# dkogan/libdogleg

Hardware: NVIDIA B200
Metric: dogleg_iterations_per_sec (higher is better)
Workload: dtype f64

## Files before the change

include/dogleg_gpu.h:

```cpp
#pragma once
#include <stddef.h>
#include "dogleg.h"
#ifdef __cplusplus
extern "C" {
#endif

int         dogleg_gpu_device_count(void);
int         dogleg_gpu_set_device(int device);
int         dogleg_gpu_get_device(void);
const char* dogleg_gpu_last_error(void);
const char* dogleg_gpu_version(void);

void        dogleg_gpu_set_permutation(const int* perm, int n, int postorder);

typedef void (dogleg_gpu_callback_sparse_t)(const double* d_p, double* d_x, double* d_Jt_values,
                                            void* stream, void* cookie);
typedef void (dogleg_gpu_callback_dense_t)(const double* d_p, double* d_x, double* d_J,
                                           void* stream, void* cookie);

double dogleg_gpu_optimize_sparse(double* p, unsigned int Nstate, unsigned int Nmeas, unsigned int NJnnz,
                                  const int* Jp, const int* Ji,
                                  dogleg_gpu_callback_sparse_t* f, void* cookie,
                                  const dogleg_parameters2_t* parameters,
                                  dogleg_solverContext_t** returnContext);
double dogleg_gpu_optimize_dense(double* p, unsigned int Nstate, unsigned int Nmeas,
                                 dogleg_gpu_callback_dense_t* f, void* cookie,
                                 const dogleg_parameters2_t* parameters,
                                 dogleg_solverContext_t** returnContext);

typedef void (dogleg_gpu_callback_dense_products_t)(const double* d_p, double* d_norm2x, double* d_Jtx,
                                                     double* d_JtJ, void* stream, void* cookie);
double dogleg_gpu_optimize_dense_products(double* p, unsigned int Nstate,
                                          dogleg_gpu_callback_dense_products_t* f, void* cookie,
                                          const dogleg_parameters2_t* parameters,
                                          dogleg_solverContext_t** returnContext);

int dogleg_gpu_solve(dogleg_solverContext_t* ctx, const double* B, double* X, int nrhs);
int dogleg_gpu_export_factor(dogleg_solverContext_t* ctx);

void dogleg_gpu_host_progress(size_t n_values_final, size_t n_x_final);

int  dogleg_gpu_nccl_get_unique_id(unsigned char id[128]);
int  dogleg_gpu_nccl_init(int rank, int world, const unsigned char id[128]);
void dogleg_gpu_nccl_finalize(void);
int  dogleg_gpu_nccl_world(void);

double dogleg_gpu_optimize_sparse_sharded(double* p, unsigned int Nstate,
                                          unsigned int Nmeas_total, const int* Jp_global, const int* Ji_global,
                                          unsigned int col_begin, unsigned int Nmeas_local,
                                          dogleg_callback_t* f_host, dogleg_gpu_callback_sparse_t* f_device,
                                          void* cookie, const dogleg_parameters2_t* parameters,
                                          dogleg_solverContext_t** returnContext);

double dogleg_gpu_optimize_dense_sharded(double* p, unsigned int Nstate, unsigned int Nmeas_total,
                                         unsigned int row_begin, unsigned int Nmeas_local,
                                         dogleg_callback_dense_t* f_host, dogleg_gpu_callback_dense_t* f_device,
                                         void* cookie, const dogleg_parameters2_t* parameters,
                                         dogleg_solverContext_t** returnContext);

void dogleg_gpu_context_layout(size_t out[6]);

void dogleg_gpu_get_stats(const dogleg_solverContext_t* ctx, double out[8]);
void dogleg_gpu_get_comm_stats(double out[2]);
void dogleg_gpu_get_phase_ms(double out[8]);

typedef void (dogleg_gpu_callback_dense_batched_t)(const double* d_p, double* d_x, double* d_J,
                                                   const int* d_active, int B,
                                                   void* stream, void* cookie);
int dogleg_gpu_optimize_dense_batched(double* p, unsigned int Nstate, unsigned int Nmeas,
                                      unsigned int B,
                                      dogleg_gpu_callback_dense_batched_t* f, void* cookie,
                                      const dogleg_parameters2_t* parameters,
                                      double* norm2x_out, int* iterations_out);

typedef void (dogleg_gpu_callback_dense_products_batched_t)(const double* d_p, double* d_norm2x, double* d_Jtx,
                                                             double* d_JtJ, const int* d_active, int B,
                                                             void* stream, void* cookie);
int dogleg_gpu_optimize_dense_products_batched(double* p, unsigned int Nstate, unsigned int B,
                                               dogleg_gpu_callback_dense_products_batched_t* f, void* cookie,
                                               const dogleg_parameters2_t* parameters,
                                               double* norm2x_out, int* iterations_out);

typedef struct dogleg_gpu_batch dogleg_gpu_batch_t;

int dogleg_gpu_optimize_dense_batched2(double* p, unsigned int Nstate, unsigned int Nmeas, unsigned int B,
                                       dogleg_gpu_callback_dense_batched_t* f, void* cookie,
                                       const dogleg_parameters2_t* parameters,
                                       double* norm2x_out, int* iterations_out, dogleg_gpu_batch_t** returnBatch);
int dogleg_gpu_optimize_dense_products_batched2(double* p, unsigned int Nstate, unsigned int B,
                                                dogleg_gpu_callback_dense_products_batched_t* f, void* cookie,
                                                const dogleg_parameters2_t* parameters,
                                                double* norm2x_out, int* iterations_out,
                                                dogleg_gpu_batch_t** returnBatch);

enum { DOGLEG_GPU_BATCH_UNFINISHED = 0,
       DOGLEG_GPU_BATCH_GRADIENT = 1,
       DOGLEG_GPU_BATCH_STEP = 2,
       DOGLEG_GPU_BATCH_TRUSTREGION = 3,
       DOGLEG_GPU_BATCH_MAX_ITERATIONS = 4 };


int  dogleg_gpu_batch_status(const dogleg_gpu_batch_t* batch, int* status_out, double* lambda_out);
int  dogleg_gpu_batch_solve(dogleg_gpu_batch_t* batch, const double* R, double* X, int nrhs);
int  dogleg_gpu_batch_solve_device(dogleg_gpu_batch_t* batch, const double* d_R, double* d_X, int nrhs, void* stream);
int  dogleg_gpu_batch_covariance(dogleg_gpu_batch_t* batch, double* out, int packed);
int  dogleg_gpu_batch_covariance_device(dogleg_gpu_batch_t* batch, double* d_out, int packed, void* stream);
void dogleg_gpu_batch_free(dogleg_gpu_batch_t** batch);

void dogleg_gpu_batched_stats(double out[8]);
void dogleg_gpu_release_batched_cache(void);

typedef struct dlb_symbolic dlb_symbolic_t;
dlb_symbolic_t* dlb_symbolic_create(int Nstate, int Nmeas, const int* Jp, const int* Ji,
                                    const int* perm_or_null, int postorder);
void            dlb_symbolic_free(dlb_symbolic_t* S);
void            dlb_symbolic_info(const dlb_symbolic_t* S, long long out[8]);
enum { DLB_SYM_PERM = 0, DLB_SYM_PARENT = 1, DLB_SYM_COLCOUNT = 2, DLB_SYM_SN_FIRST = 3,
       DLB_SYM_ROWS_PTR = 4, DLB_SYM_ROWS = 5, DLB_SYM_SN_PARENT = 6, DLB_SYM_CLS_OF_COL = 7,
       DLB_SYM_CLS_FRONT = 8, DLB_SYM_SN_LEVEL = 9, DLB_SYM_REL = 10, DLB_SYM_CHILD_PTR = 11,
       DLB_SYM_CHILD_LIST = 12, DLB_SYM_LEVEL_PTR = 13, DLB_SYM_LEVEL_SN = 14, DLB_SYM_CLS_PTR = 15,
       DLB_SYM_CLS_ROWS = 16, DLB_SYM_CLS_LOC = 17, DLB_SYM_MEM_PTR = 18, DLB_SYM_MEM_COL = 19 };
long long       dlb_symbolic_get(const dlb_symbolic_t* S, int what, int* out, long long cap);
long long       dlb_symbolic_front_off(const dlb_symbolic_t* S, long long* out, long long cap);

typedef struct dlb_gather_plan dlb_gather_plan_t;
dlb_gather_plan_t* dlb_gather_plan_create(const dlb_symbolic_t* S, int small_front_max, int heavy,
                                          int gsplit, int gchunk, int gtile);
void            dlb_gather_plan_free(dlb_gather_plan_t* G);
void            dlb_gather_plan_info(const dlb_gather_plan_t* G, long long out[8]);
enum { DLB_GP_DST = 0, DLB_GP_SRC_PTR = 1, DLB_GP_SRC_BASE = 2, DLB_GP_LD = 3, DLB_GP_H = 4, DLB_GP_W = 5,
       DLB_GP_SRC_LD = 6, DLB_GP_LEVEL_PTR = 7, DLB_GP_TMP_OFF = 8, DLB_GP_LEVEL_TMP = 9, DLB_GP_SG_FLAG = 10 };
long long       dlb_gather_plan_get(const dlb_gather_plan_t* G, int list, int what, long long* out, long long cap);

typedef struct dlb_task_plan dlb_task_plan_t;
dlb_task_plan_t* dlb_task_plan_create(const dlb_symbolic_t* S, const int* Jp, int col_begin, int ncols,
                                      int sm_count, int ranges_enabled);
void            dlb_task_plan_free(dlb_task_plan_t* T);
enum { DLB_TP_TASK_CLS = 0, DLB_TP_TASK_M0 = 1, DLB_TP_TASK_M1 = 2, DLB_TP_CLS_TASK_PTR = 3, DLB_TP_TASK_GOFF = 4,
       DLB_TP_TASK_GGOFF = 5, DLB_TP_MEM_COL = 6, DLB_TP_MEM_POS = 7, DLB_TP_BIG_TASKS = 8, DLB_TP_SMALL_TASKS = 9,
       DLB_TP_GJ_BIG_TASKS = 10, DLB_TP_RANGED = 11, DLB_TP_GP_COUNT = 12, DLB_TP_GP_FIRST = 13, DLB_TP_GINV_PTR = 14,
       DLB_TP_GINV_CLS = 15, DLB_TP_GINV_OFF = 16, DLB_TP_HEAVY = 17, DLB_TP_MEDIUM = 18,
       DLB_TP_SIZES = 19,
       DLB_TP_RANGE_TASKS = 20    };
long long       dlb_task_plan_get(const dlb_task_plan_t* T, int what, long long* out, long long cap);

typedef struct dlb_engine dlb_engine_t;

typedef struct
{
  double norm2_x, norm2_Jtx, maxabs_Jtx;
  double norm2_JJtx, k_cauchy, norm2_cauchy;
  double norm2_gn;
  double norm2_step, k_interp, Jtx_dot_step, maxabs_step, norm2_Jstep, discriminant;
  double step_type, trial_flags;
  long long minor;
} dlb_scalars_t;

enum { DLB_STEP_CAUCHY = 0, DLB_STEP_GAUSSNEWTON = 1, DLB_STEP_INTERPOLATED = 2 };

dlb_engine_t* dlb_engine_create(int solve_type, unsigned int Nstate, unsigned int Nmeas,
                                unsigned int NJnnz, int packed, int upper);
enum { DLB_ENGINE_NO_HOST_INPUTS = 1 };
dlb_engine_t* dlb_engine_create2(int solve_type, unsigned int Nstate, unsigned int Nmeas,
                                 unsigned int NJnnz, int packed, int upper, int flags);
dlb_engine_t* dlb_engine_create3(int solve_type, unsigned int Nstate, unsigned int Nmeas,
                                 unsigned int NJnnz, int packed, int upper, int flags,
                                 unsigned int Nmeas_total, unsigned int col_begin);
void          dlb_engine_comm_stats(const dlb_engine_t* e, double out[2]);
void          dlb_engine_destroy(dlb_engine_t* e);
void          dogleg_gpu_release_cache(void);
void          dogleg_gpu_assume_pattern_unchanged(int on);
int           dlb_engine_pattern_equals(const dlb_engine_t* e, const int* Jp, const int* Ji);

enum { DLB_BUF_P = 0, DLB_BUF_X = 1, DLB_BUF_JTX = 2, DLB_BUF_CAUCHY = 3, DLB_BUF_GN = 4,
       DLB_BUF_STEP = 5, DLB_BUF_JVALUES = 6, DLB_BUF_JP = 7, DLB_BUF_JI = 8,
       DLB_BUF_NORM2X = 9    };
void*         dlb_engine_host_buffer(dlb_engine_t* e, int slot, int which);
void*         dlb_engine_device_buffer(dlb_engine_t* e, int slot, int which);
void*         dlb_engine_stream(dlb_engine_t* e);

int  dlb_engine_set_pattern(dlb_engine_t* e, const int* Jp, const int* Ji,
                            const int* perm_or_null, int postorder);
const dlb_symbolic_t* dlb_engine_symbolic(const dlb_engine_t* e);

int  dlb_engine_evaluate(dlb_engine_t* e, int slot, int from_host, double norm2x_products);
void dlb_engine_begin_host_fill(dlb_engine_t* e, int slot);
int  dlb_engine_cauchy(dlb_engine_t* e, int slot);
int  dlb_engine_factorize(dlb_engine_t* e, int slot, double lambda);
int  dlb_engine_gauss_newton(dlb_engine_t* e, int slot);
int  dlb_engine_step(dlb_engine_t* e, int from, int to, int step_type, double delta);
int  dlb_engine_has_trial(const dlb_engine_t* e);
int  dlb_engine_has_fused_eval(const dlb_engine_t* e);
int  dlb_engine_trial(dlb_engine_t* e, int from, int to, double delta, double lambda);
void dlb_engine_set_lazy_p(dlb_engine_t* e, int on);
int  dlb_engine_download_p(dlb_engine_t* e, int slot);
int  dlb_engine_download(dlb_engine_t* e, int slot);
int  dlb_engine_upload_p(dlb_engine_t* e, int slot);
const dlb_scalars_t* dlb_engine_scalars(const dlb_engine_t* e);

int  dlb_engine_solve(dlb_engine_t* e, const double* B, double* X, int nrhs);
int  dlb_engine_debug_JtJ(dlb_engine_t* e, int slot, double lambda, double* JtJ_out);
int  dlb_engine_dense_factor_to_host(dlb_engine_t* e, double* out);

void dlb_engine_counters(const dlb_engine_t* e, double out[4]);
void dlb_engine_enable_timing(dlb_engine_t* e, int on);
void dlb_engine_phase_ms(const dlb_engine_t* e, double out[8]);

#ifdef __cplusplus
}
#endif
```

libdogleg_b200/csrc/dlb_capi_symbolic.cpp:

```cpp
#include "dlb_symbolic.h"
#include "dlb_gatherplan.h"
#include "dlb_taskplan.h"
#include "dogleg_internal.h"
#include <cstdlib>
#include <cstring>
#include <algorithm>

struct dlb_symbolic { DlbSymbolic S; };

extern "C" dlb_symbolic_t* dlb_symbolic_create(int Nstate, int Nmeas, const int* Jp, const int* Ji,
                                               const int* perm_or_null, int postorder)
{
  dlb_symbolic* h = new dlb_symbolic();
  if(!dlb_symbolic_analyze(h->S, Nstate, Nmeas, Jp, Ji, perm_or_null, postorder != 0))
  {
    delete h;
    dlb_set_error("malformed Jt pattern or permutation");
    return NULL;
  }
  return h;
}
extern "C" void dlb_symbolic_free(dlb_symbolic_t* h) { delete h; }

static const DlbSymbolic& sym(const dlb_symbolic_t* h) { return *reinterpret_cast<const DlbSymbolic*>(h); }

extern "C" void dlb_symbolic_info(const dlb_symbolic_t* h, long long out[8])
{
  const DlbSymbolic& S = sym(h);
  out[0] = S.ncls; out[1] = S.nsuper; out[2] = S.nlevels; out[3] = S.nnzL();
  out[4] = S.max_front_rows; out[5] = S.front_off.empty() ? 0 : S.front_off.back();
  out[6] = (long long)S.flops(); out[7] = (long long)S.rows.size();
}
extern "C" long long dlb_symbolic_get(const dlb_symbolic_t* h, int what, int* out, long long cap)
{
  const DlbSymbolic& S = sym(h);
  const std::vector<int>* v = NULL;
  switch(what)
  {
  case DLB_SYM_PERM: v = &S.perm; break;           case DLB_SYM_PARENT: v = &S.parent; break;
  case DLB_SYM_COLCOUNT: v = &S.colcount; break;   case DLB_SYM_SN_FIRST: v = &S.sn_first; break;
  case DLB_SYM_ROWS_PTR: v = &S.rows_ptr; break;   case DLB_SYM_ROWS: v = &S.rows; break;
  case DLB_SYM_SN_PARENT: v = &S.sn_parent; break; case DLB_SYM_CLS_OF_COL: v = &S.cls_of_col; break;
  case DLB_SYM_CLS_FRONT: v = &S.cls_front; break; case DLB_SYM_SN_LEVEL: v = &S.sn_level; break;
  case DLB_SYM_REL: v = &S.rel; break;             case DLB_SYM_CHILD_PTR: v = &S.child_ptr; break;
  case DLB_SYM_CHILD_LIST: v = &S.child_list; break; case DLB_SYM_LEVEL_PTR: v = &S.level_ptr; break;
  case DLB_SYM_LEVEL_SN: v = &S.level_sn; break;
  case DLB_SYM_CLS_PTR: v = &S.cls_ptr; break;     case DLB_SYM_CLS_ROWS: v = &S.cls_rows; break;
  case DLB_SYM_CLS_LOC: v = &S.cls_loc; break;     case DLB_SYM_MEM_PTR: v = &S.mem_ptr; break;
  case DLB_SYM_MEM_COL: v = &S.mem_col; break;
  default: return -1;
  }
  const long long n = (long long)v->size();
  if(out && cap > 0) std::memcpy(out, v->data(), sizeof(int) * (size_t)std::min(n, cap));
  return n;
}

extern "C" long long dlb_symbolic_front_off(const dlb_symbolic_t* h, long long* out, long long cap)
{
  const DlbSymbolic& S = sym(h);
  const long long n = (long long)S.front_off.size();
  for(long long i = 0; out && i < std::min(n, cap); i++) out[i] = (long long)S.front_off[i];
  return n;
}

struct dlb_gather_plan { DlbGatherPlan P; long long pool_fronts, solve_rows; int nlevels; };

extern "C" dlb_gather_plan_t* dlb_gather_plan_create(const dlb_symbolic_t* h, int small_front_max, int heavy,
                                                     int gsplit, int gchunk, int gtile)
{
  const DlbSymbolic& S = sym(h);
  DlbGatherParams GP;
  if(small_front_max > 0) GP.small_front_max = small_front_max;
  if(heavy >= 0) GP.heavy = heavy;
  if(gsplit > 0) GP.gsplit = gsplit;
  if(gchunk > 0) GP.gchunk = gchunk;
  if(gtile > 0) GP.gtile = gtile;
  dlb_gather_plan* g = new dlb_gather_plan();
  dlb_build_gather_plan(S, GP, g->P);
  g->pool_fronts = S.front_off.empty() ? 0 : (long long)S.front_off.back();
  g->solve_rows = (long long)S.rows.size();
  g->nlevels = S.nlevels;
  return g;
}
extern "C" void dlb_gather_plan_free(dlb_gather_plan_t* g) { delete g; }
extern "C" void dlb_gather_plan_info(const dlb_gather_plan_t* g, long long out[8])
{
  out[0] = g->pool_fronts; out[1] = g->P.pool_tmp; out[2] = g->P.pool_scratch;
  out[3] = g->solve_rows;  out[4] = g->P.solve_scratch;
  out[5] = (long long)g->P.fronts.dst.size(); out[6] = (long long)g->P.solve.dst.size(); out[7] = g->nlevels;
}
template<class T> static long long copy_wide(const std::vector<T>& v, long long* out, long long cap)
{
  const long long n = (long long)v.size();
  for(long long i = 0; out && i < std::min(n, cap); i++) out[i] = (long long)v[i];
  return n;
}
extern "C" long long dlb_gather_plan_get(const dlb_gather_plan_t* g, int list, int what, long long* out, long long cap)
{
  const DlbGatherList& G = list ? g->P.solve : g->P.fronts;
  switch(what)
  {
  case DLB_GP_DST:       return copy_wide(G.dst, out, cap);
  case DLB_GP_SRC_PTR:   return copy_wide(G.src_ptr, out, cap);
  case DLB_GP_SRC_BASE:  return copy_wide(G.gs_base, out, cap);
  case DLB_GP_LD:        return copy_wide(G.ld, out, cap);
  case DLB_GP_H:         return copy_wide(G.h, out, cap);
  case DLB_GP_W:         return copy_wide(G.w, out, cap);
  case DLB_GP_SRC_LD:    return copy_wide(G.gs_ld, out, cap);
  case DLB_GP_LEVEL_PTR: return copy_wide(list ? g->P.level_sg_ptr : g->P.level_gt_ptr, out, cap);
  case DLB_GP_TMP_OFF:   return copy_wide(g->P.heavy_tmp_off, out, cap);
  case DLB_GP_LEVEL_TMP: return copy_wide(g->P.level_tmp_size, out, cap);
  case DLB_GP_SG_FLAG:   return copy_wide(g->P.sg_flag, out, cap);
  default: return -1;
  }
}

struct dlb_task_plan { DlbTaskPlan T; };

extern "C" dlb_task_plan_t* dlb_task_plan_create(const dlb_symbolic_t* h, const int* Jp, int col_begin, int ncols,
                                                 int sm_count, int ranges_enabled)
{
  const DlbSymbolic& S = sym(h);
  if(!Jp || col_begin < 0 || ncols < 0 || col_begin + ncols > S.m) { dlb_set_error("task plan: bad column range"); return NULL; }
  dlb_task_plan* t = new dlb_task_plan();
  dlb_build_task_plan(S, Jp, col_begin, ncols, S.n, sm_count > 0 ? sm_count : 148, ranges_enabled != 0, t->T);
  return t;
}
extern "C" void dlb_task_plan_free(dlb_task_plan_t* t) { delete t; }
extern "C" long long dlb_task_plan_get(const dlb_task_plan_t* t, int what, long long* out, long long cap)
{
  const DlbTaskPlan& T = t->T;
  switch(what)
  {
  case DLB_TP_TASK_CLS:     return copy_wide(T.task_cls, out, cap);
  case DLB_TP_TASK_M0:      return copy_wide(T.task_m0, out, cap);
  case DLB_TP_TASK_M1:      return copy_wide(T.task_m1, out, cap);
  case DLB_TP_CLS_TASK_PTR: return copy_wide(T.cls_task_ptr, out, cap);
  case DLB_TP_TASK_GOFF:    return copy_wide(T.task_goff, out, cap);
  case DLB_TP_TASK_GGOFF:   return copy_wide(T.task_Goff, out, cap);
  case DLB_TP_MEM_COL:      return copy_wide(T.mem_col, out, cap);
  case DLB_TP_MEM_POS:      return copy_wide(T.mem_pos, out, cap);
  case DLB_TP_BIG_TASKS:    return copy_wide(T.big_tasks, out, cap);
  case DLB_TP_SMALL_TASKS:  return copy_wide(T.small_tasks, out, cap);
  case DLB_TP_GJ_BIG_TASKS: return copy_wide(T.gj_big_tasks, out, cap);
  case DLB_TP_RANGED:       return copy_wide(T.ranged, out, cap);
  case DLB_TP_GP_COUNT:     return copy_wide(T.gp_count, out, cap);
  case DLB_TP_GP_FIRST:     return copy_wide(T.gp_first, out, cap);
  case DLB_TP_GINV_PTR:     return copy_wide(T.ginv_ptr, out, cap);
  case DLB_TP_GINV_CLS:     return copy_wide(T.ginv_cls, out, cap);
  case DLB_TP_GINV_OFF:     return copy_wide(T.ginv_off, out, cap);
  case DLB_TP_HEAVY:        return copy_wide(T.heavy_state, out, cap);
  case DLB_TP_MEDIUM:       return copy_wide(T.medium_state, out, cap);
  case DLB_TP_SIZES:
  {
    const long long v[4] = {T.goff, T.Goff, (long long)T.range_kmax, (long long)T.heavy_threshold};
    for(long long i = 0; out && i < std::min<long long>(4, cap); i++) out[i] = v[i];
    return 4;
  }
  case DLB_TP_RANGE_TASKS:
  {
    const long long n = (long long)T.rtasks.size() * 17;
    for(size_t r = 0; out && r < T.rtasks.size() && (long long)(r + 1) * 17 <= cap; r++)
    {
      const DlbRangeTask& R = T.rtasks[r];
      long long* o = out + r * 17;
      o[0] = R.j0; o[1] = R.ncols; o[2] = R.P; o[3] = R.Ktot; o[4] = R.pos0;
      for(int i = 0; i < 4; i++) { o[5 + i] = R.cls[i]; o[9 + i] = R.koff[i]; o[13 + i] = R.goff[i]; }
    }
    return n;
  }
  default: return -1;
  }
}

extern "C" cholmod_factor* dlb_factor_descriptor_new(const dlb_symbolic_t* h, int n)
{
  cholmod_factor* L = (cholmod_factor*)std::calloc(1, sizeof(cholmod_factor));
  if(!L) return NULL;
  L->n = (size_t)n; L->minor = (size_t)n;
  L->is_ll = 1; L->is_super = 1; L->is_monotonic = 1;
  L->itype = CHOLMOD_INT; L->xtype = CHOLMOD_REAL; L->dtype = CHOLMOD_DOUBLE;
  if(!h) return L;
  const DlbSymbolic& S = sym(h);
  auto dup = [](const std::vector<int>& v) {
    int* p = (int*)std::malloc(sizeof(int) * std::max<size_t>(v.size(), 1));
    if(p && !v.empty()) std::memcpy(p, v.data(), sizeof(int) * v.size());
    return p;
  };
  L->Perm = dup(S.perm); L->IPerm = dup(S.iperm); L->ColCount = dup(S.colcount);
  L->nsuper = (size_t)S.nsuper; L->ssize = S.rows.size();
  L->super = dup(S.sn_first); L->pi = dup(S.rows_ptr); L->s = dup(S.rows);
  L->ordering = S.perm_given ? CHOLMOD_GIVEN : CHOLMOD_AMD;
  size_t xs = 0; int maxc = 0;
  std::vector<int> px(S.nsuper + 1, 0);
  for(int s = 0; s < S.nsuper; s++)
  {
    const int r = S.rows_ptr[s+1] - S.rows_ptr[s], c = S.sn_first[s+1] - S.sn_first[s];
    px[s] = (int)xs; xs += (size_t)r * c; maxc = std::max(maxc, c);
  }
  px[S.nsuper] = (int)xs;
  L->px = dup(px); L->xsize = xs; L->maxcsize = (size_t)maxc;
  return L;
}
extern "C" void dlb_factor_descriptor_free(cholmod_factor* L)
{
  if(!L) return;
  std::free(L->Perm); std::free(L->IPerm); std::free(L->ColCount);
  std::free(L->super); std::free(L->pi); std::free(L->px); std::free(L->s); std::free(L->x);
  std::free(L);
}
```

libdogleg_b200/csrc/dlb_device.h:

```cpp
#pragma once
#include <cuda_runtime.h>
#include <cstdint>
#include "dlb_taskplan.h"
#include "dlb_common.cuh"

struct __align__(16) DlbClsInfo { int k, m0, nm, r0; };
struct __align__(16) DlbLeaf { long long off; int c0, nc, r, rp, fcls0, ncls; };
struct __align__(16) DlbSmallTask { int k, m0, nm, r0; long long goff, Goff; };

struct DlbSparseDev
{
  int n, m, ncls, ntasks;
  const int* cls_ptr;
  const int* cls_rows;
  const int* cls_loc;
  const int* cls_front;
  const int* task_cls;
  const int* task_m0;
  const int* task_m1;
  const long long* task_goff;
  const long long* task_Goff;
  const int* mem_col;
  const unsigned int* mem_pos;
  const int* ginv_ptr;
  const int* ginv_cls;
  const long long* ginv_off;
  const int* cls_task_ptr;
  int nbig, nsmall;
  const int* big_tasks;
  const int* small_tasks;
  int nrange, range_kmax, ngj_big;
  const DlbRangeTask* rtasks;
  const int* gj_big_tasks;
  const int* gp_count;
  const DlbSmallTask* small_info;
  const DlbClsInfo* cls_info;
  int small_group;
  int nasm_small;
  const int* asm_small_tasks;
  int nfused;
  const DlbSmallTask* fused_info;
  int nheavy, heavy_threshold;
  const int* heavy_state;
  int nmedium;
  const int* medium_state;
};

struct DlbGather
{
  const long long* dst;
  const int* ld;
  const int* h;
  const int* w;
  const long long* src_ptr;
  const long long* gs_base;
  const int* gs_ld;
};

struct DlbFrontDev
{
  int n, nsuper;
  const int* sn_first;
  const int* rows_ptr;
  const int* rows;
  const int* rel;
  const int* sn_parent;
  const int* child_ptr;
  const int* child_list;
  const long long* front_off;
  const int* fcls_ptr;
  const int* fcls_list;
  const int* cls_task_ptr;
  const int* level_sn;
  const int* perm;
  const DlbLeaf* leaf;
  const unsigned int* leaf_pos; const unsigned int* leaf_kl; const unsigned int* leaf_loc;
  int leaf_ps, leaf_lw;
  int leaf_max_nc;
  long long ytot;
  const long long* heavy_tmp_off;
  double* heavy_tmp;
  DlbGather fg;
  DlbGather sg;
  const char* sg_flag;
};

struct DlbBigFront { long long off; int r, nc, col0, sn; long long inv_off; };

#define DLB_TRIAL_PART 8
#define DLB_TRIAL_PROF_MAX 62
enum { DLB_TRIAL_CAUCHY = 0, DLB_TRIAL_GN = 1, DLB_TRIAL_INTERP = 2 };
struct DlbPublished { DlbScalars sc; unsigned long long seq; };
struct DlbTrial
{
  int nlev; const int* level_ptr; const long long* level_gt; const long long* level_sg; const long long* level_tmp;
  int max_rows, max_cols, any_solve_gather;
  int small_tail;
  const double* Jtx; const double* p_from; const double* Gpart; double* cauchy; double* gn;
  double norm2_Jtx, norm2_cauchy, norm2_gn; int have_cauchy, have_gn;
  double* step; double* p_to; double* h_p_to;
  double* fronts; double* ywork; double* zperm;
  double* part; unsigned int* bar; long long* minor; long long* minor_next;
  DlbScalars* sc; DlbPublished* pub; unsigned long long seq;
  double delta, lambda;
  const int* eg_ptr; const unsigned int* eg_dst; const int* eg_sptr; const int* eg_src;
  unsigned long long* prof;
};
size_t dlb_trial_smem_bytes(int max_rows);
int  dlb_trial_threads(int max_rows);
int  dlb_trial_max_grid(int max_rows, int sm_count);
int  dlb_launch_trial(const DlbSparseDev& S, const DlbFrontDev& F, const DlbTrial& T, int grid, cudaStream_t st);

void dlb_launch_sparse_grad(const DlbSparseDev& S, const double* Jx, const double* x, double* gpart,
                            double* n2part, double* Jtx, double* part, unsigned int* counter,
                            DlbScalars* sc, int sm_count, cudaStream_t st);
int  dlb_sparse_n2part_size(const DlbSparseDev& S, int sm_count);
struct DlbPublished;
int  dlb_launch_sparse_eval_pass(const DlbSparseDev& S, const double* Jx, const double* x, double* Gpart, double* gpart,
                                 double* n2part, int sm_count, cudaStream_t st);
void dlb_launch_sparse_eval_reduce(const DlbSparseDev& S, const double* gpart, const double* n2part, int n2count, double* Jtx,
                                   double* part, unsigned int* counter, DlbScalars* sc, DlbPublished* pub, unsigned long long seq,
                                   int n2_behind_Jtx, int sm_count, cudaStream_t st);
void dlb_launch_sparse_jv(const DlbSparseDev& S, const double* Jx, const double* v, double* part,
                          unsigned int* counter, double* dst, int sm_count, cudaStream_t st);
void dlb_launch_sparse_jv_quad(const DlbSparseDev& S, const double* Jx, const double* Gpart, const double* v, double* part,
                               unsigned int* counter, double* dst, int sm_count, cudaStream_t st);
void dlb_launch_sparse_assemble(const DlbSparseDev& S, const double* Jx, double* Gpart, int all_small,
                                int sm_count, cudaStream_t st);

void dlb_launch_leaf_fronts(const DlbFrontDev& F, const DlbSparseDev& S, int q0, int q1, const double* Jx,
                            double* fronts, double lambda, long long* minor, int max_rows, int eliminate,
                            int sm_count, cudaStream_t st);
void dlb_launch_leaf_fronts_mma(const DlbFrontDev& F, const DlbSparseDev& S, int q0, int q1, const double* Jx,
                                double* fronts, double lambda, long long* minor, int max_rows, int max_pairs, int eliminate,
                                int sm_count, cudaStream_t st);
void dlb_launch_leaf_solve_fwd(const DlbFrontDev& F, int q0, int q1, const double* fronts, const double* rhs,
                               double* ywork, double* zperm, int nrhs, int sm_count, cudaStream_t st);
void dlb_launch_leaf_solve_bwd(const DlbFrontDev& F, int q0, int q1, const double* fronts, double* zperm,
                               int nrhs, int sm_count, cudaStream_t st);

void dlb_launch_front_level(const DlbFrontDev& F, const DlbSparseDev& S, int l0, int l1,
                            double* fronts, const double* Gpart, double lambda,
                            long long* minor, int max_rows, int skip_elimination, cudaStream_t st);
void dlb_bigfront_factor_batch(const DlbBigFront* d_descs, int nfronts, int max_r, int max_nc, double* fronts, double* inv,
                               int* cnt, long long* minor, cudaStream_t st, double* n_launch);
void dlb_launch_extend_gather(const DlbGather& G, long long t0, long long t1, double* pool, int accumulate, cudaStream_t st);
void dlb_launch_zero_bigfronts(const DlbBigFront* d_descs, int nfronts, int max_r, double* fronts, cudaStream_t st);
void dlb_launch_solve_fwd_level(const DlbFrontDev& F, int l0, int l1, const double* fronts,
                                const double* rhs , double* ywork,
                                double* zperm, int nrhs, int max_rows, int max_cols, cudaStream_t st);
void dlb_launch_solve_bwd_level(const DlbFrontDev& F, int l0, int l1, const double* fronts,
                                double* zperm, int nrhs, int max_rows, int max_cols, cudaStream_t st);
void dlb_launch_fronts_to_dense(const DlbFrontDev& F, const double* fronts, double* out, cudaStream_t st);

void dlb_launch_bigsolve_fwd(const DlbFrontDev& F, const DlbBigFront* d_descs, int nfronts, int max_r, int max_nc,
                             const double* fronts, const double* inv, const double* rhs, double* ywork, double* zperm, int nrhs,
                             cudaStream_t st);
long long dlb_bigsolve_partial_size(int r, int nc);
void dlb_launch_bigsolve_bwd(const DlbFrontDev& F, const DlbBigFront* d_descs, int nfronts, int max_r, int max_nc,
                             const double* fronts, const double* inv, double* zperm, double* partial, const long long* d_part_off,
                             int nrhs, cudaStream_t st);

void dlb_launch_dense_grad(const double* J, const double* x, int M, int N, double* Jtx,
                           double* work, double* part, unsigned int* counter, DlbScalars* sc,
                           int sm_count, cudaStream_t st);
void dlb_launch_dense_jv(const double* J, const double* v, int M, int N, double* work,
                         double* dst, int sm_count, cudaStream_t st);
size_t dlb_dense_syrk_work_size(int M, int N, int sm_count);
void dlb_launch_dense_syrk(const double* J, int M, int N, double* front, double* work,
                           int sm_count, cudaStream_t st);
void dlb_launch_products_to_front(const double* JtJ, int N, int packed, int upper, double* front, cudaStream_t st);
void dlb_launch_products_xAx(const double* JtJ, int N, int packed, int upper, const double* v,
                             double* dst, cudaStream_t st);
void dlb_launch_front_to_reference_layout(const double* front, int N, int packed, int upper, double* out, cudaStream_t st);
void dlb_launch_vec_stats_Jtx(const double* v, int N, double* part, unsigned int* counter, DlbScalars* sc,
                              int sm_count, cudaStream_t st);
void dlb_launch_vec_stats_Jtx_pub(const double* v, int N, double* part, unsigned int* counter, DlbScalars* sc,
                                  DlbPublished* pub, unsigned long long seq, int sm_count, cudaStream_t st);

void dlb_launch_cauchy(const double* Jtx, int N, double* cauchy, DlbScalars* sc, int sm_count, cudaStream_t st);
void dlb_launch_gn_finish(const double* zperm, const int* perm_or_null, int N, double* gn,
                          double* part, unsigned int* counter, DlbScalars* sc, int sm_count, cudaStream_t st);
void dlb_launch_step(int step_type, double delta, const double* p_from, const double* Jtx,
                     const double* cauchy, const double* gn, int N, double* step, double* p_to,
                     double* part, unsigned int* counter, DlbScalars* sc, int sm_count, cudaStream_t st);
```

libdogleg_b200/csrc/dlb_engine.cu:

```cuda
#include "dlb_common.cuh"
#include "dlb_device.h"
#include "dlb_symbolic.h"
#include "dlb_gatherplan.h"
#include "dlb_taskplan.h"
#include "dogleg_gpu.h"
#include <vector>
#include <string>
#include <cstring>
#include <cstdlib>
#include <climits>
#include <algorithm>
#include <type_traits>
#include <mutex>
#include <chrono>
#include <thread>

static_assert(sizeof(DlbScalars) == sizeof(dlb_scalars_t), "scalar block mirrors must agree");
#define DLB_SMALL_FRONT_MAX 158

static thread_local std::string g_last_error;
static int g_device = 0;
extern "C" const char* dogleg_gpu_last_error(void) { return g_last_error.c_str(); }
extern "C" const char* dogleg_gpu_version(void)    { return "libdogleg-b200 0.1 (sm_100a)"; }
extern "C" void dlb_set_error(const char* msg)     { g_last_error = msg ? msg : ""; }
// ... 244 lines not shown
  for(unsigned long spin = 0;; spin++)
  {
    if(*q == e->seq) break;
    if((spin & 0xfff) == 0xfff)
    {
      const cudaError_t rc = cudaStreamQuery(e->st);
      if(rc == cudaSuccess) { if(*q == e->seq) break; g_last_error = "the device finished without publishing its results"; return -1; }
      if(rc != cudaErrorNotReady) { g_last_error = std::string("device error: ") + cudaGetErrorString(rc); return -1; }
    }
  }
  __sync_synchronize();
  e->n_d2h += sizeof(DlbScalars);
  return 0;
}

extern "C" void dlb_trial_dbg_dump();
static std::mutex g_pool_mu;
static std::vector<dlb_engine*> g_pool;
static const size_t POOL_MAX = 2;
static bool cache_enabled()
{
  const char* env = getenv("DOGLEG_GPU_ENGINE_CACHE");
  return !(env && atoi(env) == 0);
}
static void engine_free(dlb_engine* e);
extern "C" void dogleg_gpu_release_batched_cache(void);
extern "C" void dogleg_gpu_release_cache(void)
{
  dogleg_gpu_release_batched_cache();
  std::vector<dlb_engine*> victims;
  { std::lock_guard<std::mutex> lk(g_pool_mu); victims.swap(g_pool); }
  for(dlb_engine* e : victims) engine_free(e);
}

static int allreduce_sum(dlb_engine* e, double* d_buf, size_t count)
{
  if(!e->sharded || g_nccl.world <= 1) return 0;
  if(!g_nccl.comm) { g_last_error = "sharded engine without dogleg_gpu_nccl_init()"; return -1; }
  const int rc = g_nccl.AllReduce(d_buf, d_buf, count,  8,  0, g_nccl.comm, e->st);
  if(rc != 0) { g_last_error = std::string("ncclAllReduce: ") + (g_nccl.GetErrorString ? g_nccl.GetErrorString(rc) : "failed"); return -1; }
  e->n_allreduce += 1; e->allreduce_bytes += 8.0 * count;
  return 0;
}
extern "C" void dlb_engine_comm_stats(const dlb_engine_t* e, double out[2]) { out[0] = e->n_allreduce; out[1] = e->allreduce_bytes; }

extern "C" dlb_engine_t* dlb_engine_create(int solve_type, unsigned int Nstate, unsigned int Nmeas,
                                           unsigned int NJnnz, int packed, int upper)
{
  return dlb_engine_create2(solve_type, Nstate, Nmeas, NJnnz, packed, upper, 0);
}

extern "C" dlb_engine_t* dlb_engine_create2(int solve_type, unsigned int Nstate, unsigned int Nmeas,
                                            unsigned int NJnnz, int packed, int upper, int flags)
{
  return dlb_engine_create3(solve_type, Nstate, Nmeas, NJnnz, packed, upper, flags, 0, 0);
}

static dlb_engine_t* engine_create_impl(int solve_type, unsigned int Nstate, unsigned int Nmeas,
                                        unsigned int NJnnz, int packed, int upper, int flags,
                                        unsigned int Nmeas_total, unsigned int col_begin);
extern "C" dlb_engine_t* dlb_engine_create3(int solve_type, unsigned int Nstate, unsigned int Nmeas,
                                            unsigned int NJnnz, int packed, int upper, int flags,
                                            unsigned int Nmeas_total, unsigned int col_begin)
{
  dlb_engine_t* e = engine_create_impl(solve_type, Nstate, Nmeas, NJnnz, packed, upper, flags, Nmeas_total, col_begin);
  if(!e && g_last_error.find("out of memory") != std::string::npos)
  {
    dogleg_gpu_release_cache();
    cudaGetLastError();
    e = engine_create_impl(solve_type, Nstate, Nmeas, NJnnz, packed, upper, flags, Nmeas_total, col_begin);
  }
  return e;
}
static dlb_engine_t* engine_create_impl(int solve_type, unsigned int Nstate, unsigned int Nmeas,
                                        unsigned int NJnnz, int packed, int upper, int flags,
                                        unsigned int Nmeas_total, unsigned int col_begin)
{
  const bool want_sharded = Nmeas_total > 0;
  if(want_sharded && (solve_type == DOGLEG_DENSE_PRODUCTS || (unsigned long long)col_begin + Nmeas > Nmeas_total))
  { g_last_error = "sharded engine: bad column range or solve type"; return NULL; }
  if(dogleg_gpu_device_count() <= 0)
  {
    g_last_error = "no CUDA device available: libdogleg-b200 has no CPU fallback";
    return NULL;
  }
  if(cudaSetDevice(g_device) != cudaSuccess) { g_last_error = "cudaSetDevice failed"; return NULL; }
  const bool want_host_inputs = !(flags & DLB_ENGINE_NO_HOST_INPUTS);
  if(cache_enabled())
  {
    std::lock_guard<std::mutex> lk(g_pool_mu);
    for(size_t i = 0; i < g_pool.size(); i++)
    {
      dlb_engine* c = g_pool[i];
      if(c->type == solve_type && c->N == (int)Nstate && c->M == (int)Nmeas && c->nnz == NJnnz &&
         c->packed == packed && c->upper == upper && c->device == g_device &&
         (c->host_inputs || !want_host_inputs) && (c->sharded || c->gather) == want_sharded &&
         (!want_sharded || (c->M_total == (int)Nmeas_total && c->col_begin == (int)col_begin)))
      {
        g_pool.erase(g_pool.begin() + i);
        c->factor_slot = -1; c->factor_lambda = 0; c->lazy_p = false;
        for(int sl = 0; sl < 2; sl++) { c->slot[sl].have_G = c->slot[sl].have_cauchy = c->slot[sl].have_gn = false; }
        c->n_launch = c->n_h2d = c->n_d2h = c->n_factor = 0;
        c->timing = false; memset(c->phase_ms, 0, sizeof(c->phase_ms));
        memset(c->h_sc, 0, sizeof(*c->h_sc));
        c->pattern_verified = false;
        c->n_allreduce = c->allreduce_bytes = 0;
        return c;
      }
    }
  }
  dlb_engine* e = new dlb_engine();
  e->host_inputs = want_host_inputs;
  { const char* jp = getenv("DOGLEG_GPU_JV_PASS"); e->jv_quad = !(jp && atoi(jp) != 0); }
  e->sharded = want_sharded; e->M_total = want_sharded ? (int)Nmeas_total : (int)Nmeas; e->col_begin = (int)col_begin;
  {
    const char* sm = getenv("DOGLEG_GPU_SHARD_MODE");
    const bool want_gather = sm ? !strcmp(sm, "gather") : Nstate >= 16384;
    if(want_sharded && solve_type == DOGLEG_SPARSE && want_gather) { e->gather = true; e->sharded = false; }
  }
  e->type = solve_type; e->N = (int)Nstate; e->M = (int)Nmeas; e->nnz = NJnnz;
  e->packed = packed; e->upper = upper; e->device = g_device;
  cudaDeviceProp prop;
  if(cudaGetDeviceProperties(&prop, g_device) == cudaSuccess) e->sm_count = prop.multiProcessorCount;
  const size_t N = e->N, M = e->M;
  if(solve_type == DOGLEG_SPARSE)              e->Jcount = NJnnz;
  else if(solve_type == DOGLEG_DENSE)          e->Jcount = M * N;
  else                                         e->Jcount = packed ? N * (N + 1) / 2 : N * N;

  auto fail = [&](const char* what) { g_last_error = what; engine_free(e); return (dlb_engine_t*)NULL; };
  if(cudaStreamCreateWithFlags(&e->st, cudaStreamNonBlocking) != cudaSuccess) return fail("cudaStreamCreate failed");
  cudaEventCreate(&e->ev0); cudaEventCreate(&e->ev1);
  if(cudaStreamCreateWithFlags(&e->st_copy, cudaStreamNonBlocking) != cudaSuccess) return fail("cudaStreamCreate failed");
  cudaEventCreateWithFlags(&e->ev_copy, cudaEventDisableTiming); cudaEventCreateWithFlags(&e->ev_idle, cudaEventDisableTiming);
  bool ok = true;
  auto hostalloc = [&](size_t count, auto** out) {
    typedef typename std::remove_reference<decltype(**out)>::type T;
    void* p = 0;
    const size_t bytes = std::max<size_t>(count, 1) * sizeof(T);
    if(cudaHostAlloc(&p, bytes, cudaHostAllocDefault) != cudaSuccess) { ok = false; p = 0; }
    else memset(p, 0, bytes);
    *out = static_cast<T*>(p);
  };
  auto devalloc = [&](size_t count, auto** out) {
    typedef typename std::remove_reference<decltype(**out)>::type T;
    void* p = 0;
    if(cudaMalloc(&p, std::max<size_t>(count, 1) * sizeof(T)) != cudaSuccess) { ok = false; p = 0; }
    *out = static_cast<T*>(p);
  };
  for(int s = 0; s < 2; s++)
  {
    Slot& L = e->slot[s];
    hostalloc(N, &L.h_p); hostalloc(N, &L.h_Jtx); hostalloc(N, &L.h_cauchy); hostalloc(N, &L.h_gn); hostalloc(N, &L.h_step);
    devalloc(N, &L.d_p);  devalloc(N + 1, &L.d_Jtx);  devalloc(N, &L.d_cauchy);  devalloc(N, &L.d_gn);  devalloc(N, &L.d_step);
    if(solve_type != DOGLEG_DENSE_PRODUCTS) { if(e->host_inputs) hostalloc(M, &L.h_x); if(!e->gather) devalloc(M, &L.d_x); }
    if(e->host_inputs) hostalloc(e->Jcount, &L.h_J);
    if(!e->gather) devalloc(e->Jcount + 2, &L.d_J);
    if(solve_type == DOGLEG_SPARSE && e->host_inputs) { hostalloc(M + 1, &L.h_Jp); hostalloc(NJnnz, &L.h_Ji); }
  }
  {
    void* hp = 0; void* dpub = 0;
    if(cudaHostAlloc(&hp, sizeof(DlbPublished), cudaHostAllocMapped) != cudaSuccess) ok = false;
    else
    {
      memset(hp, 0, sizeof(DlbPublished));
      e->h_pub = (DlbPublished*)hp; e->h_sc = (dlb_scalars_t*)&e->h_pub->sc;
      if(cudaHostGetDevicePointer(&dpub, hp, 0) != cudaSuccess) ok = false;
      e->d_pub = (DlbPublished*)dpub;
    }
  }
  devalloc(1, &e->d_sc);
  hostalloc(1, &e->h_minor); devalloc(2, &e->d_minor);
  devalloc(5 * (size_t)e->sm_count * 8 + 64, &e->d_part);
  devalloc(4, &e->d_counter);
  if(!ok) return fail("out of memory allocating operating-point buffers");
  cudaMemsetAsync(e->d_counter, 0, 4 * sizeof(unsigned int), e->st);
  cudaMemsetAsync(e->d_sc, 0, sizeof(DlbScalars), e->st);

  if(solve_type != DOGLEG_SPARSE)
  {
    std::vector<int> sn_first{0, e->N}, rows_ptr{0, e->N}, rows(N), rel(N, -1), sn_parent{-1},
                     child_ptr{0, 0}, child_list, fptr{0, 0}, flist, ctask{0}, level_sn{0}, perm(N);
    std::vector<long long> front_off{0, (long long)(N * N)};
    for(size_t i = 0; i < N; i++) { rows[i] = (int)i; perm[i] = (int)i; }
    DlbFrontDev& F = e->F;
    F.n = e->N; F.nsuper = 1; F.ytot = (long long)N;
    int rc = 0;
    rc |= dev_upload(e, sn_first, &F.sn_first);   rc |= dev_upload(e, rows_ptr, &F.rows_ptr);
    rc |= dev_upload(e, rows, &F.rows);           rc |= dev_upload(e, rel, &F.rel);
    rc |= dev_upload(e, sn_parent, &F.sn_parent); rc |= dev_upload(e, child_ptr, &F.child_ptr);
    rc |= dev_upload(e, child_list, &F.child_list); rc |= dev_upload(e, front_off, &F.front_off);
    rc |= dev_upload(e, fptr, &F.fcls_ptr);       rc |= dev_upload(e, flist, &F.fcls_list);
    rc |= dev_upload(e, ctask, &F.cls_task_ptr);  rc |= dev_upload(e, level_sn, &F.level_sn);
    rc |= dev_upload(e, perm, &F.perm);
    e->level_ptr = {0, 1};
    e->max_front_rows = e->N; e->max_front_cols = e->N;
    e->level_big.assign(1, {});
    if(e->N > DLB_SMALL_FRONT_MAX) { e->level_mid = {0}; e->level_big[0].push_back({0, e->N, e->N, 0, 0}); e->max_small_rows = 0; }
    else                           { e->level_mid = {1}; e->max_small_rows = e->N; }
    e->level_small_rows = {e->max_small_rows}; e->level_rows = {e->N}; e->level_cols = {e->N};
    rc |= upload_big_descs(e);
    const int nblk = std::max(1, std::min((e->M + 63) / 64, e->sm_count * 4));
    size_t work = (size_t)nblk * (N + 1) + 16;
    if(solve_type == DOGLEG_DENSE) work = std::max(work, dlb_dense_syrk_work_size(e->M, e->N, e->sm_count));
    rc |= dev_alloc(e, N * N + 128, &e->d_fronts);
    rc |= dev_alloc(e, work, &e->d_work);
    rc |= dev_alloc(e, (size_t)2048, &e->d_xAx);
    rc |= dev_alloc(e, N, &e->d_ywork);
    rc |= dev_alloc(e, N, &e->d_zperm);
    if(rc) return fail("out of memory allocating dense workspace");
    e->pattern_set = true;
  }
  if(cudaStreamSynchronize(e->st) != cudaSuccess) return fail("device initialisation failed");
  return e;
}

extern "C" void dlb_engine_destroy(dlb_engine_t* e)
{
  if(!e) return;
  if(cache_enabled() && e->st && e->pattern_set)
  {
    cudaSetDevice(e->device);
    if(cudaStreamSynchronize(e->st) != cudaSuccess || cudaGetLastError() != cudaSuccess) { engine_free(e); return; }
    dlb_engine* evicted = NULL;
    {
      std::lock_guard<std::mutex> lk(g_pool_mu);
      g_pool.push_back(e);
      if(g_pool.size() > POOL_MAX) { evicted = g_pool.front(); g_pool.erase(g_pool.begin()); }
    }
    if(evicted) engine_free(evicted);
    return;
  }
  engine_free(e);
}

static void engine_free(dlb_engine* e)
{
  if(!e) return;
  cudaSetDevice(e->device);
  if(e->st) cudaStreamSynchronize(e->st);
  for(int s = 0; s < 2; s++)
  {
    Slot& L = e->slot[s];
    void* hs[] = {L.h_p, L.h_x, L.h_Jtx, L.h_cauchy, L.h_gn, L.h_step, L.h_J, L.h_Jp, L.h_Ji};
    void* ds[] = {L.d_p, L.d_x, L.d_Jtx, L.d_cauchy, L.d_gn, L.d_step, L.d_J};
    for(void* p : hs) if(p) cudaFreeHost(p);
    for(void* p : ds) if(p) cudaFree(p);
  }
  if(e->h_pub) cudaFreeHost(e->h_pub);
  if(e->h_minor) cudaFreeHost(e->h_minor);
  void* ds[] = {e->d_sc, e->d_minor, e->d_part, e->d_counter, e->d_rhs};
  for(void* p : ds) if(p) cudaFree(p);
  for(void* p : e->dev_allocs) cudaFree(p);
  if(e->ev0) cudaEventDestroy(e->ev0);
  if(e->ev1) cudaEventDestroy(e->ev1);
  if(e->ev_copy) cudaEventDestroy(e->ev_copy);
  if(e->ev_idle) cudaEventDestroy(e->ev_idle);
  if(e->st_copy) cudaStreamDestroy(e->st_copy);
  if(e->st) cudaStreamDestroy(e->st);
  delete e->sym;
  delete e;
}

extern "C" void* dlb_engine_host_buffer(dlb_engine_t* e, int s, int which)
{
  Slot& L = e->slot[s & 1];
  switch(which)
  {
  case DLB_BUF_P: return L.h_p;       case DLB_BUF_X: return L.h_x;     case DLB_BUF_JTX: return L.h_Jtx;
  case DLB_BUF_CAUCHY: return L.h_cauchy; case DLB_BUF_GN: return L.h_gn; case DLB_BUF_STEP: return L.h_step;
  case DLB_BUF_JVALUES: return L.h_J; case DLB_BUF_JP: return L.h_Jp;   case DLB_BUF_JI: return L.h_Ji;
  }
  return NULL;
}
extern "C" void* dlb_engine_device_buffer(dlb_engine_t* e, int s, int which)
{
  Slot& L = e->slot[s & 1];
  switch(which)
  {
  case DLB_BUF_P: return L.d_p;       case DLB_BUF_JTX: return L.d_Jtx;
  case DLB_BUF_CAUCHY: return L.d_cauchy; case DLB_BUF_GN: return L.d_gn; case DLB_BUF_STEP: return L.d_step;
  case DLB_BUF_X:       return L.d_x ? L.d_x + (e->gather ? e->col_begin : 0) : NULL;
  case DLB_BUF_JVALUES: return L.d_J ? L.d_J + (e->gather ? e->slice_off : 0) : NULL;
  case DLB_BUF_NORM2X:  return e->type == DOGLEG_DENSE_PRODUCTS ? L.d_Jtx + e->N : NULL;
  }
  return NULL;
}
extern "C" int dlb_engine_pattern_equals(const dlb_engine_t* e, const int* Jp, const int* Ji)
{
  if(e->pat_full_p.empty()) return -1;
  const size_t np = e->pat_full_p.size(), ni = e->pat_full_i.size();
  if((size_t)(unsigned int)Jp[np - 1] != ni) return 0;
  return !memcmp(e->pat_full_p.data(), Jp, sizeof(int) * np) && !memcmp(e->pat_full_i.data(), Ji, sizeof(int) * ni) ? 1 : 0;
}
extern "C" void* dlb_engine_stream(dlb_engine_t* e) { return (void*)e->st; }
extern "C" const dlb_scalars_t* dlb_engine_scalars(const dlb_engine_t* e) { return e->h_sc; }
extern "C" const dlb_symbolic_t* dlb_engine_symbolic(const dlb_engine_t* e) { return (const dlb_symbolic_t*)e->sym; }
extern "C" void dlb_engine_counters(const dlb_engine_t* e, double out[4])
{ out[0] = e->n_launch; out[1] = e->n_h2d; out[2] = e->n_d2h; out[3] = e->n_factor; }
extern "C" void dlb_engine_enable_timing(dlb_engine_t* e, int on) { e->timing = on != 0; memset(e->phase_ms, 0, sizeof(e->phase_ms)); }
extern "C" void dlb_engine_phase_ms(const dlb_engine_t* e, double out[8]) { memcpy(out, e->phase_ms, sizeof(e->phase_ms)); }

static inline unsigned long long hash_mix(unsigned long long h, unsigned long long v)
{
  h ^= v + 0x9E3779B97F4A7C15ull + (h << 6) + (h >> 2);
  return h * 0xff51afd7ed558ccdull;
}
static unsigned long long hash_ints(const int* a, size_t n, unsigned long long seed)
{
  unsigned long long h0 = seed, h1 = seed ^ 0x1234567ull, h2 = seed ^ 0x89abcdefull, h3 = seed ^ 0x5555aaaaull;
  size_t i = 0;
  for(; i + 8 <= n; i += 8)
  {
    unsigned long long v[4];
    memcpy(v, a + i, 32);
    h0 = hash_mix(h0, v[0]); h1 = hash_mix(h1, v[1]); h2 = hash_mix(h2, v[2]); h3 = hash_mix(h3, v[3]);
  }
  for(; i < n; i++) h0 = hash_mix(h0, (unsigned long long)(unsigned int)a[i]);
  return hash_mix(hash_mix(h0, h1), hash_mix(h2, h3));
}
static unsigned long long pattern_hash(const int* Jp, size_t np, const int* Ji, size_t ni)
{
  const int NTH = ni > (1u << 22) ? 4 : 1;
  unsigned long long part[4] = {0, 0, 0, 0};
  std::vector<std::thread> th;
  for(int t = 1; t < NTH; t++)
    th.emplace_back([&, t]() { const size_t a = ni * t / NTH, b = ni * (t + 1) / NTH; part[t] = hash_ints(Ji + a, b - a, 0xabcdull + t); });
  part[0] = hash_ints(Ji, ni / NTH, 0xabcdull);
  for(auto& x : th) x.join();
  unsigned long long h = hash_ints(Jp, np, 0x77ull);
  for(int t = 0; t < NTH; t++) h = hash_mix(h, part[t]);
  return hash_mix(h, (unsigned long long)ni);
}
static thread_local int g_trust_pattern = -1;
extern "C" void dogleg_gpu_assume_pattern_unchanged(int on) { g_trust_pattern = on ? 1 : 0; }
static bool trust_pattern()
{
  if(g_trust_pattern >= 0) return g_trust_pattern != 0;
  const char* env = getenv("DOGLEG_GPU_TRUST_PATTERN");
  return env && atoi(env) != 0;
}

extern "C" int dlb_engine_set_pattern(dlb_engine_t* e, const int* Jp, const int* Ji,
                                      const int* perm_or_null, int postorder)
{
  if(e->type != DOGLEG_SPARSE) return 0;
  if(e->pattern_set && e->pattern_verified) return 0;
  cudaSetDevice(e->device);
  if(!Jp) { Jp = e->slot[0].h_Jp; Ji = e->slot[0].h_Ji; }
  if(!Jp || !Ji) { g_last_error = "set_pattern: no pattern given"; return -1; }
  const int Mtot = e->M_total, cb = e->col_begin;
  if((unsigned int)(Jp[cb + e->M] - Jp[cb]) > e->nnz) { g_last_error = "the pattern has more nonzeros than NJnnz"; return -1; }

  const char* env = getenv("DOGLEG_GPU_CHECK_PATTERN");
  const bool full_check = env && atoi(env) != 0;
  std::vector<int> sample;
  {
    auto take = [&](const int* a, size_t len) {
      const size_t stride = std::max<size_t>(1, len / 4096);
      sample.push_back((int)len);
      for(size_t i = 0; i < len; i += stride) sample.push_back(a[i]);
      for(size_t i = 0; i < std::min<size_t>(len, 64); i++) { sample.push_back(a[i]); sample.push_back(a[len - 1 - i]); }
    };
    take(Jp, (size_t)Mtot + 1);
    take(Ji, (size_t)(unsigned int)Jp[Mtot]);
  }
  std::vector<int> perm_req;
  if(perm_or_null) perm_req.assign(perm_or_null, perm_or_null + e->N);
  if(e->pattern_set)
  {
    bool same = sample == e->pat_sample && perm_req == e->perm_used && (perm_req.empty() || postorder == e->postorder_used);
    if(same && !trust_pattern()) same = pattern_hash(Jp, (size_t)Mtot + 1, Ji, (size_t)(unsigned int)Jp[Mtot]) == e->pat_hash;
    if(same && full_check)
      same = e->pat_full_p.size() == (size_t)Mtot + 1 && !memcmp(e->pat_full_p.data(), Jp, sizeof(int) * ((size_t)Mtot + 1)) &&
             !memcmp(e->pat_full_i.data(), Ji, sizeof(int) * e->pat_full_i.size());
    if(same) { e->pattern_verified = true; return 0; }
    CU(cudaStreamSynchronize(e->st));
    for(void* q : e->dev_allocs) cudaFree(q);
    e->dev_allocs.clear();
    delete e->sym; e->sym = 0;
    e->pattern_set = false;
    e->d_gpart = e->d_n2part = e->d_jvpart = e->d_fronts = e->d_ywork = e->d_zperm = 0;
    e->slot[0].d_G = e->slot[1].d_G = 0; e->slot[0].have_G = e->slot[1].have_G = false;
    e->fused_eval = e->fused_trial = false; e->d_trial_part = 0; e->d_bar = 0; e->d_prof = 0;
  }
  e->pat_sample.swap(sample);
  e->pat_hash = pattern_hash(Jp, (size_t)Mtot + 1, Ji, (size_t)(unsigned int)Jp[Mtot]);
  e->perm_used.swap(perm_req); e->postorder_used = postorder;
  if(full_check) { e->pat_full_p.assign(Jp, Jp + Mtot + 1); e->pat_full_i.assign(Ji, Ji + (unsigned int)Jp[Mtot]); }
  else { e->pat_full_p.clear(); e->pat_full_i.clear(); }
  e->sym = new DlbSymbolic();
  const bool verbose = getenv("DOGLEG_GPU_VERBOSE") && atoi(getenv("DOGLEG_GPU_VERBOSE")) != 0;
  const auto t_begin = std::chrono::steady_clock::now();
  if(!dlb_symbolic_analyze(*e->sym, e->N, Mtot, Jp, Ji, perm_or_null, postorder != 0))
  { g_last_error = "malformed Jt pattern (indices must be ascending and in range)"; return -1; }
  const DlbSymbolic& Y = *e->sym;
  const auto t_sym = std::chrono::steady_clock::now();
  if(Y.max_front_rows > 46340) { g_last_error = "a front has more than 46340 rows: not supported"; return -1; }

  const int cbk = e->gather ? 0 : cb, Mk = e->gather ? Mtot : e->M;
  if(e->gather)
  {
    const size_t nnz_full = (size_t)(unsigned int)Jp[Mtot];
    for(int sl = 0; sl < 2; sl++)
    {
      Slot& L = e->slot[sl];
      if(L.d_x) cudaFree(L.d_x);
      if(L.d_J) cudaFree(L.d_J);
      L.d_x = L.d_J = 0;
      CU(cudaMalloc(&L.d_x, sizeof(double) * std::max<size_t>(Mtot, 1)));
      CU(cudaMalloc(&L.d_J, sizeof(double) * (nnz_full + 2)));
    }
    e->slice_off = Jp[cb];
    const int world = g_nccl.comm ? g_nccl.world : 1, rank = g_nccl.comm ? g_nccl.rank : 0;
    std::vector<long long> mine{(long long)cb, (long long)e->M}, all(2 * (size_t)world, 0);
    if(world > 1)
    {
      long long* d_tab = 0;
      CU(cudaMalloc(&d_tab, sizeof(long long) * 2 * (size_t)(world + 1)));
      CU(cudaMemcpyAsync(d_tab, mine.data(), sizeof(long long) * 2, cudaMemcpyHostToDevice, e->st));
      if(g_nccl.AllGather(d_tab, d_tab + 2, 2,  4, g_nccl.comm, e->st) != 0)
      { cudaFree(d_tab); g_last_error = "ncclAllGather of the slice table failed"; return -1; }
      CU(cudaMemcpyAsync(all.data(), d_tab + 2, sizeof(long long) * 2 * world, cudaMemcpyDeviceToHost, e->st));
      CU(cudaStreamSynchronize(e->st));
      cudaFree(d_tab);
    }
    else all = mine;
    (void)rank;
    e->rank_cb.assign(world, 0); e->rank_m.assign(world, 0); e->rank_off.assign(world, 0); e->rank_nnz.assign(world, 0);
    for(int r = 0; r < world; r++)
    {
      e->rank_cb[r] = all[2*r]; e->rank_m[r] = all[2*r+1];
      if(e->rank_cb[r] < 0 || e->rank_cb[r] + e->rank_m[r] > Mtot) { g_last_error = "inconsistent column ranges across the ranks"; return -1; }
      e->rank_off[r] = Jp[e->rank_cb[r]];
      e->rank_nnz[r] = Jp[e->rank_cb[r] + e->rank_m[r]] - Jp[e->rank_cb[r]];
    }
  }
  {
    const char* fe = getenv("DOGLEG_GPU_FUSED");
    e->fused_eval = e->jv_quad && !(fe && atoi(fe) == 0);
    e->G_global = e->sharded && e->fused_eval;
  }
  DlbTaskPlan TP;
  {
    const char* renv = getenv("DOGLEG_GPU_RANGE");
    dlb_build_task_plan(Y, Jp, cbk, Mk, e->N, e->sm_count, !e->fused_eval && !(renv && atoi(renv) == 0), TP, e->G_global);
  }
  const std::vector<int>& task_cls = TP.task_cls; const std::vector<int>& task_m0 = TP.task_m0;
  const std::vector<int>& task_m1 = TP.task_m1;   const std::vector<int>& cls_task_ptr = TP.cls_task_ptr;
  const std::vector<long long>& task_goff = TP.task_goff; const std::vector<long long>& task_Goff = TP.task_Goff;
  const std::vector<int>& lmem_col = TP.mem_col;  const std::vector<unsigned int>& mem_pos = TP.mem_pos;
  const std::vector<int>& big_tasks = TP.big_tasks; const std::vector<int>& small_tasks = TP.small_tasks;
  const std::vector<DlbRangeTask>& rtasks = TP.rtasks; const std::vector<int>& gj_big_tasks = TP.gj_big_tasks;
  const std::vector<int>& gp_count = TP.gp_count;
  const std::vector<int>& ginv_ptr = TP.ginv_ptr; const std::vector<int>& ginv_cls = TP.ginv_cls;
  const std::vector<long long>& ginv_off = TP.ginv_off;
  const std::vector<int>& heavy_state = TP.heavy_state; const std::vector<int>& medium_state = TP.medium_state;
  const int ntasks = (int)task_cls.size(), range_kmax = TP.range_kmax, heavy_threshold = TP.heavy_threshold;
  const long long goff = TP.goff, Goff = TP.Goff;

  DlbSparseDev& S = e->S; DlbFrontDev& F = e->F;
  S.nheavy = (int)heavy_state.size(); S.heavy_threshold = heavy_threshold; S.nmedium = (int)medium_state.size();
  S.n = e->N; S.m = Mk; S.ncls = Y.ncls; S.ntasks = ntasks;
  S.nbig = (int)big_tasks.size(); S.nsmall = (int)small_tasks.size();
  S.nrange = (int)rtasks.size(); S.range_kmax = range_kmax; S.ngj_big = (int)gj_big_tasks.size();
  const std::vector<int>& mem_col_local = lmem_col;
  F.n = e->N; F.nsuper = Y.nsuper; F.ytot = (long long)Y.rows.size();
  int rc = 0;
  rc |= dev_upload(e, Y.cls_ptr, &S.cls_ptr);     rc |= dev_upload(e, Y.cls_rows, &S.cls_rows);
  rc |= dev_upload(e, Y.cls_loc, &S.cls_loc);     rc |= dev_upload(e, Y.cls_front, &S.cls_front);
  rc |= dev_upload(e, task_cls, &S.task_cls);     rc |= dev_upload(e, task_m0, &S.task_m0);
  rc |= dev_upload(e, task_m1, &S.task_m1);       rc |= dev_upload(e, task_goff, &S.task_goff);
  rc |= dev_upload(e, task_Goff, &S.task_Goff);   rc |= dev_upload(e, mem_col_local, &S.mem_col);
  rc |= dev_upload(e, mem_pos, &S.mem_pos);       rc |= dev_upload(e, ginv_ptr, &S.ginv_ptr);
  rc |= dev_upload(e, ginv_cls, &S.ginv_cls);     rc |= dev_upload(e, ginv_off, &S.ginv_off);
  rc |= dev_upload(e, heavy_state, &S.heavy_state); rc |= dev_upload(e, medium_state, &S.medium_state);
  rc |= dev_upload(e, big_tasks, &S.big_tasks);   rc |= dev_upload(e, small_tasks, &S.small_tasks);
  rc |= dev_upload(e, rtasks, &S.rtasks);         rc |= dev_upload(e, gj_big_tasks, &S.gj_big_tasks);
  rc |= dev_upload(e, gp_count, &S.gp_count);
  {
    std::vector<DlbSmallTask> info(small_tasks.size());
    int kmax = 1;
    for(size_t i = 0; i < small_tasks.size(); i++)
    {
      const int t = small_tasks[i], c = task_cls[t];
      info[i] = {Y.cls_ptr[c+1] - Y.cls_ptr[c], task_m0[t], task_m1[t] - task_m0[t], Y.cls_ptr[c], task_goff[t], task_Goff[t]};
      kmax = std::max(kmax, info[i].k);
    }
    S.small_group = kmax <= 8 ? 8 : (kmax <= 16 ? 16 : 32);
    rc |= dev_upload(e, info, &S.small_info);
  }
  rc |= dev_upload(e, Y.sn_first, &F.sn_first);   rc |= dev_upload(e, Y.rows_ptr, &F.rows_ptr);
  rc |= dev_upload(e, Y.rows, &F.rows);           rc |= dev_upload(e, Y.rel, &F.rel);
  rc |= dev_upload(e, Y.sn_parent, &F.sn_parent); rc |= dev_upload(e, Y.child_ptr, &F.child_ptr);
  rc |= dev_upload(e, Y.child_list, &F.child_list);
  { std::vector<long long> fo(Y.front_off.begin(), Y.front_off.end()); rc |= dev_upload(e, fo, &F.front_off); }
  rc |= dev_upload(e, Y.fcls_ptr, &F.fcls_ptr);   rc |= dev_upload(e, Y.fcls_list, &F.fcls_list);
  rc |= dev_upload(e, cls_task_ptr, &F.cls_task_ptr);
  S.cls_task_ptr = F.cls_task_ptr;
  {
    std::vector<int> level_sn(Y.level_sn);
    e->level_mid.assign(Y.nlevels, 0);
    e->level_big.assign(Y.nlevels, {});
    e->max_small_rows = 0;
    e->level_small_rows.assign(Y.nlevels, 0); e->level_rows.assign(Y.nlevels, 0); e->level_cols.assign(Y.nlevels, 0);
    e->nleaf = 0; e->leaf_max_rows = 0; e->leaf_max_pairs = 0;
    std::vector<char> cls_fused(Y.ncls, 0);
    if(!e->sharded && Y.nlevels > 0)
    {
      auto eligible = [&](int sn) {
        const int r = Y.rows_ptr[sn+1] - Y.rows_ptr[sn], nc = Y.sn_first[sn+1] - Y.sn_first[sn];
        if(r > 48 || nc > 8 || Y.child_ptr[sn+1] != Y.child_ptr[sn]) return false;
        if(Y.fcls_ptr[sn+1] - Y.fcls_ptr[sn] > 32) return false;
        int npair = 0, nvals = 0, nlocs = 0;
        for(int ci = Y.fcls_ptr[sn]; ci < Y.fcls_ptr[sn+1]; ci++)
        {
          const int c = Y.fcls_list[ci];
          if(cls_task_ptr[c+1] - cls_task_ptr[c] != 1) return false;
          const int t = cls_task_ptr[c];
          const int nm = task_m1[t] - task_m0[t], k = Y.cls_ptr[c+1] - Y.cls_ptr[c];
          if(k > 32) return false;
          npair += nm; nvals += nm * k; nlocs += k;
        }
        return npair <= 32 && nvals <= 256 && nlocs <= 128;
      };
      auto mid0 = std::stable_partition(level_sn.begin() + Y.level_ptr[0], level_sn.begin() + Y.level_ptr[1], eligible);
      e->nleaf = (int)(mid0 - (level_sn.begin() + Y.level_ptr[0]));
      const char* lm = getenv("DOGLEG_GPU_LEAF_MIN");
      if(e->nleaf < (lm ? atoi(lm) : 1024)) e->nleaf = 0;
      { const char* lm2 = getenv("DOGLEG_GPU_LEAF_MMA"); e->leaf_mma = !(lm2 && atoi(lm2) == 0); }
      for(int q = Y.level_ptr[0]; q < Y.level_ptr[0] + e->nleaf; q++)
      {
        const int sn = level_sn[q];
        e->leaf_max_rows = std::max(e->leaf_max_rows, Y.rows_ptr[sn+1] - Y.rows_ptr[sn]);
        if(Y.sn_first[sn+1] - Y.sn_first[sn] > 4) e->leaf_mma = false;
        int np = 0;
        for(int ci = Y.fcls_ptr[sn]; ci < Y.fcls_ptr[sn+1]; ci++) { const int t = cls_task_ptr[Y.fcls_list[ci]]; np += task_m1[t] - task_m0[t]; }
        e->leaf_max_pairs = std::max(e->leaf_max_pairs, np);
        for(int ci = Y.fcls_ptr[sn]; ci < Y.fcls_ptr[sn+1]; ci++) cls_fused[Y.fcls_list[ci]] = 1;
      }
    }
    {
      std::vector<DlbLeaf> leaf(e->nleaf);
      for(int i = 0; i < e->nleaf; i++)
      {
        const int sn = level_sn[Y.level_ptr[0] + i];
        leaf[i] = {(long long)Y.front_off[sn], Y.sn_first[sn], Y.sn_first[sn+1] - Y.sn_first[sn],
                   Y.rows_ptr[sn+1] - Y.rows_ptr[sn], Y.rows_ptr[sn], Y.fcls_ptr[sn], Y.fcls_ptr[sn+1] - Y.fcls_ptr[sn]};
      }
      rc |= dev_upload(e, leaf, &F.leaf);
      int ps = 1, lw = 1;
      for(int i = 0; i < e->nleaf; i++)
      {
        const int sn = level_sn[Y.level_ptr[0] + i];
        int np = 0, nl = 0;
        for(int ci = Y.fcls_ptr[sn]; ci < Y.fcls_ptr[sn+1]; ci++)
        { const int c = Y.fcls_list[ci], t = cls_task_ptr[c]; np += task_m1[t] - task_m0[t]; nl += Y.cls_ptr[c+1] - Y.cls_ptr[c]; }
        ps = std::max(ps, np); lw = std::max(lw, (nl + 3) / 4);
      }
      F.leaf_ps = ps; F.leaf_lw = lw; F.leaf_max_nc = 0;
      for(int i = 0; i < e->nleaf; i++)
      { const int sn = level_sn[Y.level_ptr[0] + i]; F.leaf_max_nc = std::max(F.leaf_max_nc, Y.sn_first[sn+1] - Y.sn_first[sn]); }
      std::vector<unsigned int> lpos((size_t)e->nleaf * ps, 0u), lkl((size_t)e->nleaf * ps, 0u), lloc((size_t)e->nleaf * lw, 0u);
      for(int i = 0; i < e->nleaf && e->leaf_mma; i++)
      {
        const int sn = level_sn[Y.level_ptr[0] + i];
        int np = 0, nl = 0;
        unsigned char* lb = (unsigned char*)(lloc.data() + (size_t)i * lw);
        for(int ci = Y.fcls_ptr[sn]; ci < Y.fcls_ptr[sn+1]; ci++)
        {
          const int c = Y.fcls_list[ci], t = cls_task_ptr[c], k = Y.cls_ptr[c+1] - Y.cls_ptr[c];
          for(int m = task_m0[t]; m < task_m1[t]; m++, np++)
          { lpos[(size_t)i * ps + np] = mem_pos[m]; lkl[(size_t)i * ps + np] = (unsigned)k | ((unsigned)nl << 8); }
          for(int l = 0; l < k; l++) lb[nl + l] = (unsigned char)Y.cls_loc[Y.cls_ptr[c] + l];
          nl += k;
        }
      }
      if(!e->leaf_mma) { lpos.clear(); lkl.clear(); lloc.clear(); }
      rc |= dev_upload(e, lpos, &F.leaf_pos); rc |= dev_upload(e, lkl, &F.leaf_kl); rc |= dev_upload(e, lloc, &F.leaf_loc);
      std::vector<DlbClsInfo> cinfo(Y.ncls);
      for(int c = 0; c < Y.ncls; c++)
      {
        const int t = cls_task_ptr[c];
        cinfo[c] = {Y.cls_ptr[c+1] - Y.cls_ptr[c], t < ntasks ? task_m0[t] : 0,
                    (t < ntasks && t < cls_task_ptr[c+1]) ? task_m1[t] - task_m0[t] : 0, Y.cls_ptr[c]};
      }
      rc |= dev_upload(e, cinfo, &S.cls_info);
    }
    {
      std::vector<int> asm_small;
      std::vector<DlbSmallTask> fused_info;
      for(int t : small_tasks)
      {
        const int c = task_cls[t];
        if(!cls_fused[c]) asm_small.push_back(t);
        else fused_info.push_back({Y.cls_ptr[c+1] - Y.cls_ptr[c], task_m0[t], task_m1[t] - task_m0[t], Y.cls_ptr[c], task_goff[t], task_Goff[t]});
      }
      S.nasm_small = (int)asm_small.size(); S.nfused = (int)fused_info.size();
      rc |= dev_upload(e, asm_small, &S.asm_small_tasks);
      rc |= dev_upload(e, fused_info, &S.fused_info);
    }
    for(int l = 0; l < Y.nlevels; l++)
    {
      auto rows_of = [&](int sn) { return Y.rows_ptr[sn+1] - Y.rows_ptr[sn]; };
      const int lbeg = Y.level_ptr[l] + (l == 0 ? e->nleaf : 0);
      for(int q = Y.level_ptr[l]; q < Y.level_ptr[l+1]; q++)
      {
        const int sn = level_sn[q];
        if(q < lbeg) continue;
        e->level_rows[l] = std::max(e->level_rows[l], rows_of(sn));
        e->level_cols[l] = std::max(e->level_cols[l], Y.sn_first[sn+1] - Y.sn_first[sn]);
        if(rows_of(sn) <= DLB_SMALL_FRONT_MAX) e->level_small_rows[l] = std::max(e->level_small_rows[l], rows_of(sn));
      }
      std::stable_partition(level_sn.begin() + lbeg, level_sn.begin() + Y.level_ptr[l+1],
                            [&](int sn) { return rows_of(sn) <= DLB_SMALL_FRONT_MAX; });
      int mid = lbeg;
      while(mid < Y.level_ptr[l+1] && rows_of(level_sn[mid]) <= DLB_SMALL_FRONT_MAX)
      { e->max_small_rows = std::max(e->max_small_rows, rows_of(level_sn[mid])); mid++; }
      e->level_mid[l] = mid;
      for(int q = mid; q < Y.level_ptr[l+1]; q++)
      {
        const int sn = level_sn[q];
        e->level_big[l].push_back({(long long)Y.front_off[sn], rows_of(sn), Y.sn_first[sn+1] - Y.sn_first[sn], Y.sn_first[sn], sn});
      }
    }
    rc |= dev_upload(e, level_sn, &F.level_sn);
    rc |= upload_big_descs(e);
  }
  rc |= dev_upload(e, Y.perm, &F.perm);
  long long pool_tmp = 0, pool_scratch = 0;
  long long solve_scratch = 0;
  {
// ... 97 lines not shown
        if(r2) { g_last_error = "out of device memory for the trial kernel's workspace"; return -1; }
        CU(cudaMemsetAsync(e->d_bar, 0, 4 * sizeof(unsigned int), e->st));
        e->fused_trial = true;
      }
    }
  }
  CU(cudaStreamSynchronize(e->st));
  e->pattern_set = true;
  e->pattern_verified = true;
  if(verbose)
  {
    const auto t_end = std::chrono::steady_clock::now();
    size_t fr = 0, tot = 0; cudaMemGetInfo(&fr, &tot);
    fprintf(stderr, "libdogleg-b200: pattern N=%d M=%d: %d classes, %d supernodes, %d levels, nnz(L)=%lld, fronts %.2f GB, "
            "max front %d; symbolic %.2f s, index build + upload %.2f s; device memory in use %.1f GB; fused evaluation %d, trial kernel %d (grid %d)\n",
            e->N, Mtot, Y.ncls, Y.nsuper, Y.nlevels, (long long)Y.nnzL(), 8e-9 * (double)Y.front_off[Y.nsuper], Y.max_front_rows,
            std::chrono::duration<double>(t_sym - t_begin).count(), std::chrono::duration<double>(t_end - t_sym).count(),
            1e-9 * (double)(tot - fr), (int)e->fused_eval, (int)e->fused_trial, e->trial_grid);
  }
  return 0;
}

extern "C" int dlb_engine_upload_p(dlb_engine_t* e, int s)
{
  cudaSetDevice(e->device);
  Slot& L = e->slot[s & 1];
  CU(cudaMemcpyAsync(L.d_p, L.h_p, sizeof(double) * e->N, cudaMemcpyHostToDevice, e->st));
  e->n_h2d += sizeof(double) * e->N;
  return 0;
}

static thread_local struct { dlb_engine* e; int slot; size_t wJ, wx; } g_fill = {0, 0, 0, 0};
#define DLB_FILL_MIN_BYTES (1u << 20)
extern "C" void dlb_engine_begin_host_fill(dlb_engine_t* e, int s)
{
  g_fill.e = 0;
  if(!e->host_inputs || e->type == DOGLEG_DENSE_PRODUCTS) return;
  cudaSetDevice(e->device);
  if(cudaEventRecord(e->ev_idle, e->st) != cudaSuccess || cudaStreamWaitEvent(e->st_copy, e->ev_idle, 0) != cudaSuccess) { cudaGetLastError(); return; }
  g_fill.e = e; g_fill.slot = s & 1; g_fill.wJ = 0; g_fill.wx = 0;
}
static void fill_copy_upto(dlb_engine* e, Slot& L, size_t nJ, size_t nx, bool all)
{
  nJ = std::min(nJ, e->Jcount); nx = std::min(nx, (size_t)e->M);
  if(nx > g_fill.wx && (all || (nx - g_fill.wx) * sizeof(double) >= DLB_FILL_MIN_BYTES))
  {
    cudaMemcpyAsync(L.d_x + (e->gather ? e->col_begin : 0) + g_fill.wx, L.h_x + g_fill.wx, sizeof(double) * (nx - g_fill.wx),
                    cudaMemcpyHostToDevice, e->st_copy);
    g_fill.wx = nx;
  }
  if(nJ > g_fill.wJ && (all || (nJ - g_fill.wJ) * sizeof(double) >= DLB_FILL_MIN_BYTES))
  {
    cudaMemcpyAsync(L.d_J + (e->gather ? e->slice_off : 0) + g_fill.wJ, L.h_J + g_fill.wJ, sizeof(double) * (nJ - g_fill.wJ),
                    cudaMemcpyHostToDevice, e->st_copy);
    g_fill.wJ = nJ;
  }
}
extern "C" void dogleg_gpu_host_progress(size_t n_values_final, size_t n_x_final)
{
  dlb_engine* e = g_fill.e;
  if(!e) return;
  fill_copy_upto(e, e->slot[g_fill.slot], n_values_final, n_x_final, false);
}

extern "C" int dlb_engine_evaluate(dlb_engine_t* e, int s, int from_host, double norm2x_products)
{
  cudaSetDevice(e->device);
  Slot& L = e->slot[s & 1];
  if(e->factor_slot == (s & 1)) e->factor_slot = -1;
  L.have_G = L.have_cauchy = L.have_gn = false;
  if(from_host && !e->host_inputs) { g_last_error = "evaluate(from_host): this engine was created without host mirrors"; return -1; }
  if(from_host)
  {
    PhaseTimer tm(e, 0);
    if(e->type == DOGLEG_DENSE_PRODUCTS)
    {
      CU(cudaMemcpyAsync(L.d_Jtx, L.h_Jtx, sizeof(double) * e->N, cudaMemcpyHostToDevice, e->st));
      CU(cudaMemcpyAsync(L.d_J, L.h_J, sizeof(double) * e->Jcount, cudaMemcpyHostToDevice, e->st));
      e->n_h2d += sizeof(double) * (e->N + e->Jcount);
    }
    else
    {
      size_t cnt = e->Jcount;
      if(e->type == DOGLEG_SPARSE)
      {
        cnt = (size_t)(unsigned int)L.h_Jp[e->M];
        if(cnt > (size_t)e->nnz) { g_fill.e = 0; g_last_error = "the callback wrote more nonzeros (Jt->p[Nmeas]) than NJnnz"; return -1; }
      }
      if(!(g_fill.e == e && g_fill.slot == (s & 1)))
      {
        g_fill.e = e; g_fill.slot = s & 1; g_fill.wJ = 0; g_fill.wx = 0;
        CU(cudaEventRecord(e->ev_idle, e->st));
        CU(cudaStreamWaitEvent(e->st_copy, e->ev_idle, 0));
      }
      if(g_fill.wJ > cnt) g_fill.wJ = cnt;
      {
        const size_t keepJ = e->Jcount; e->Jcount = cnt;
        fill_copy_upto(e, L, cnt, (size_t)e->M, true);
        e->Jcount = keepJ;
      }
      g_fill.e = 0;
      CU(cudaEventRecord(e->ev_copy, e->st_copy));
      CU(cudaStreamWaitEvent(e->st, e->ev_copy, 0));
      CU(cudaGetLastError());
      e->n_h2d += sizeof(double) * (e->M + cnt);
    }
  }
  if(e->gather && g_nccl.comm && g_nccl.world > 1)
  {
    PhaseTimer tm(e, 0);
    bool ok = g_nccl.GroupStart() == 0;
    for(int r = 0; ok && r < g_nccl.world; r++)
    {
      double* px = L.d_x + e->rank_cb[r]; double* pj = L.d_J + e->rank_off[r];
      if(e->rank_m[r] > 0)   ok = ok && g_nccl.Broadcast(px, px, (size_t)e->rank_m[r],  8, r, g_nccl.comm, e->st) == 0;
      if(e->rank_nnz[r] > 0) ok = ok && g_nccl.Broadcast(pj, pj, (size_t)e->rank_nnz[r], 8, r, g_nccl.comm, e->st) == 0;
      e->allreduce_bytes += 8.0 * (double)(e->rank_m[r] + e->rank_nnz[r]);
    }
    ok = (g_nccl.GroupEnd() == 0) && ok;
    if(!ok) { g_last_error = "ncclBroadcast of the Jacobian slices failed"; return -1; }
    e->n_allreduce += 1;
  }
  if(e->type == DOGLEG_SPARSE && e->fused_eval)
  {
    if(!e->pattern_set || !e->pattern_verified) { g_last_error = "dlb_engine_set_pattern() has not been called"; return -1; }
    int n2count = 0;
    {
      PhaseTimer tm(e, 1);
      n2count = dlb_launch_sparse_eval_pass(e->S, L.d_J, L.d_x, L.d_G, e->d_gpart, e->d_n2part, e->sm_count, e->st);
    }
    if(e->G_global && g_nccl.world > 1)
    {
      PhaseTimer tm(e, 3);
      dlb_launch_sparse_eval_reduce(e->S, e->d_gpart, e->d_n2part, n2count, L.d_Jtx, e->d_part, e->d_counter, e->d_sc,
                                    (DlbPublished*)0, 0ull, 1, e->sm_count, e->st);
      if(!g_nccl.comm) { g_last_error = "sharded engine without dogleg_gpu_nccl_init()"; return -1; }
      bool ok = g_nccl.GroupStart() == 0;
      ok = ok && g_nccl.AllReduce(L.d_G, L.d_G, (size_t)e->Goff_total,  8,  0, g_nccl.comm, e->st) == 0;
      ok = ok && g_nccl.AllReduce(L.d_Jtx, L.d_Jtx, (size_t)e->N + 1, 8, 0, g_nccl.comm, e->st) == 0;
      ok = (g_nccl.GroupEnd() == 0) && ok;
      if(!ok) { g_last_error = "ncclAllReduce of the class blocks / gradient failed"; return -1; }
      e->n_allreduce += 1; e->allreduce_bytes += 8.0 * (double)(e->Goff_total + e->N + 1);
      e->seq++;
      dlb_launch_vec_stats_Jtx_pub(L.d_Jtx, e->N, e->d_part, e->d_counter, e->d_sc, e->d_pub, e->seq, e->sm_count, e->st);
      e->n_launch += 1;
    }
    else
    {
      PhaseTimer tm(e, 3);
      e->seq++;
      dlb_launch_sparse_eval_reduce(e->S, e->d_gpart, e->d_n2part, n2count, L.d_Jtx, e->d_part, e->d_counter, e->d_sc, e->d_pub,
                                    e->seq, 0, e->sm_count, e->st);
    }
    e->n_launch += 1 + (e->S.nbig > 0) + (e->S.nasm_small > 0) + (e->S.nfused > 0);
    L.have_G = true;
    if(e->G_shared) e->slot[1 - (s & 1)].have_G = false;
    CU(cudaGetLastError());
  }
  else
  {
    PhaseTimer tm(e, 1);
    if(e->type == DOGLEG_SPARSE)
    {
      if(!e->pattern_set || !e->pattern_verified) { g_last_error = "dlb_engine_set_pattern() has not been called"; return -1; }
      dlb_launch_sparse_grad(e->S, L.d_J, L.d_x, e->d_gpart, e->d_n2part, L.d_Jtx, e->d_part, e->d_counter,
                             e->d_sc, e->sm_count, e->st);
      e->n_launch += 2;
    }
    else if(e->type == DOGLEG_DENSE)
    {
      dlb_launch_dense_grad(L.d_J, L.d_x, e->M, e->N, L.d_Jtx, e->d_work, e->d_part, e->d_counter,
                            e->d_sc, e->sm_count, e->st);
      e->n_launch += 2;
    }
    else
    {
      dlb_launch_vec_stats_Jtx(L.d_Jtx, e->N, e->d_part, e->d_counter, e->d_sc, e->sm_count, e->st);
      e->n_launch += 1;
      if(!from_host) CU(cudaMemcpyAsync(&e->d_sc->norm2_x, L.d_Jtx + e->N, sizeof(double), cudaMemcpyDeviceToDevice, e->st));
    }
    CU(cudaGetLastError());
    if(e->sharded && g_nccl.world > 1)
    {
      CU(cudaMemcpyAsync(L.d_Jtx + e->N, &e->d_sc->norm2_x, sizeof(double), cudaMemcpyDeviceToDevice, e->st));
      if(allreduce_sum(e, L.d_Jtx, (size_t)e->N + 1)) return -1;
      dlb_launch_vec_stats_Jtx(L.d_Jtx, e->N, e->d_part, e->d_counter, e->d_sc, e->sm_count, e->st);
      CU(cudaMemcpyAsync(&e->d_sc->norm2_x, L.d_Jtx + e->N, sizeof(double), cudaMemcpyDeviceToDevice, e->st));
      e->n_launch += 1;
    }
  }
  if(e->type == DOGLEG_SPARSE && e->fused_eval) { if(wait_published(e)) return -1; }
  else if(sync_scalars(e)) return -1;
  if(e->type == DOGLEG_DENSE_PRODUCTS && from_host) e->h_sc->norm2_x = norm2x_products;
  L.norm2_x = e->h_sc->norm2_x;
  L.norm2_Jtx = e->h_sc->norm2_Jtx;
  return 0;
}

static int ensure_G(dlb_engine* e, int s);
static int launch_norm2_Jv(dlb_engine* e, Slot& L, const double* d_v, double* d_dst)
{
  if(e->type == DOGLEG_SPARSE)
  {
    if(e->jv_quad && L.have_G)
      dlb_launch_sparse_jv_quad(e->S, L.d_J, L.d_G, d_v, e->d_part, e->d_counter, d_dst, e->sm_count, e->st);
    else
      dlb_launch_sparse_jv(e->S, L.d_J, d_v, e->d_part, e->d_counter, d_dst, e->sm_count, e->st);
    e->n_launch += 1;
  }
  else if(e->type == DOGLEG_DENSE)
  { dlb_launch_dense_jv(L.d_J, d_v, e->M, e->N, e->d_work, d_dst, e->sm_count, e->st); e->n_launch += 2; }
  else
  {
    if(e->packed && !e->upper)
    { g_last_error = "dense-products: v'JtJ v is only supported for unpacked or packed-upper JtJ (as in the reference)"; return -1; }
    dlb_launch_products_xAx(L.d_J, e->N, e->packed, e->upper, d_v, e->d_xAx, e->st);
    CU(cudaMemcpyAsync(d_dst, e->d_xAx, sizeof(double), cudaMemcpyDeviceToDevice, e->st));
    e->n_launch += 2;
  }
  CU(cudaGetLastError());
  if(!(e->G_global && L.have_G) && allreduce_sum(e, d_dst, 1)) return -1;
  return 0;
}

extern "C" int dlb_engine_cauchy(dlb_engine_t* e, int s)
{
  cudaSetDevice(e->device);
  Slot& L = e->slot[s & 1];
  if(ensure_G(e, s)) return -1;
  {
    PhaseTimer tm(e, 2);
    if(launch_norm2_Jv(e, L, L.d_Jtx, &e->d_sc->norm2_JJtx)) return -1;
    dlb_launch_cauchy(L.d_Jtx, e->N, L.d_cauchy, e->d_sc, e->sm_count, e->st);
    e->n_launch += 1;
    CU(cudaGetLastError());
  }
  if(sync_scalars(e)) return -1;
  L.have_cauchy = true; L.norm2_cauchy = e->h_sc->norm2_cauchy;
  return 0;
}

struct EvProf
{
  bool on; cudaStream_t st; std::vector<std::pair<std::string, cudaEvent_t>> ev;
  EvProf(cudaStream_t s) : st(s) { const char* p = getenv("DOGLEG_GPU_SOLVE_PROF"); on = p && atoi(p) != 0; if(on) mark("start"); }
  void mark(const std::string& name) { if(!on) return; cudaEvent_t x; cudaEventCreate(&x); cudaEventRecord(x, st); ev.push_back({name, x}); }
  void dump(const char* what)
  {
    if(!on) return;
    cudaStreamSynchronize(st);
    fprintf(stderr, "libdogleg-b200: %s (us):", what);
    for(size_t i = 1; i < ev.size(); i++) { float ms = 0; cudaEventElapsedTime(&ms, ev[i-1].second, ev[i].second); fprintf(stderr, " %s %.1f", ev[i].first.c_str(), 1e3 * ms); }
    float tot = 0; if(ev.size() > 1) cudaEventElapsedTime(&tot, ev.front().second, ev.back().second);
    fprintf(stderr, "  total %.1f\n", 1e3 * tot);
    for(auto& x : ev) cudaEventDestroy(x.second);
    ev.clear();
  }
};

static int run_factor_levels(dlb_engine* e, const double* Gpart, double lambda)
{
  const long long big = LLONG_MAX;
  e->minor_dirty = true;
  CU(cudaMemcpyAsync(e->d_minor, &big, sizeof(big), cudaMemcpyHostToDevice, e->st));
  const int nlev = (int)e->level_ptr.size() - 1;
  EvProf prof(e->st);
  for(int l = 0; l < nlev; l++)
  {
    const int nbigl = e->level_big_ptr[l+1] - e->level_big_ptr[l];
    if(nbigl > 0 && Gpart)
    {
      dlb_launch_zero_bigfronts(e->d_big_descs + e->level_big_ptr[l], nbigl, e->level_big_max_r[l], e->d_fronts, e->st);
      e->n_launch += 1;
    }
    if(!e->level_gt_ptr.empty() && e->level_gt_ptr[2*l+2] > e->level_gt_ptr[2*l])
    {
      if(e->level_tmp_size[l] > 0)
        CU(cudaMemsetAsync(e->F.heavy_tmp, 0, sizeof(double) * (size_t)e->level_tmp_size[l], e->st));
      dlb_launch_extend_gather(e->F.fg, e->level_gt_ptr[2*l], e->level_gt_ptr[2*l+1], e->d_fronts, 0, e->st);
      dlb_launch_extend_gather(e->F.fg, e->level_gt_ptr[2*l+1], e->level_gt_ptr[2*l+2], e->d_fronts, 1, e->st);
      e->n_launch += 2;
    }
    prof.mark("g" + std::to_string(l));
    const int lbeg = e->level_ptr[l] + (l == 0 && Gpart ? e->nleaf : 0);
    if(lbeg > e->level_ptr[l])
    {
      if(e->leaf_mma)
        dlb_launch_leaf_fronts_mma(e->F, e->S, e->level_ptr[l], lbeg, e->slot[e->asm_slot].d_J, e->d_fronts, lambda,
                                   e->d_minor, e->leaf_max_rows, e->leaf_max_pairs, 1, e->sm_count, e->st);
      else
        dlb_launch_leaf_fronts(e->F, e->S, e->level_ptr[l], lbeg, e->slot[e->asm_slot].d_J, e->d_fronts, lambda,
                               e->d_minor, e->leaf_max_rows, 1, e->sm_count, e->st);
      e->n_launch += 1;
    }
    if(e->level_mid[l] > lbeg)
    {
      dlb_launch_front_level(e->F, e->S, lbeg, e->level_mid[l], e->d_fronts, Gpart, lambda,
                             e->d_minor, e->level_small_rows[l], 0, e->st);
      e->n_launch += 1;
    }
    if(e->level_ptr[l+1] > e->level_mid[l])
    {
      dlb_launch_front_level(e->F, e->S, e->level_mid[l], e->level_ptr[l+1], e->d_fronts, Gpart, lambda,
                             e->d_minor, e->level_rows[l], 1, e->st);
      e->n_launch += 1;
      dlb_bigfront_factor_batch(e->d_big_descs + e->level_big_ptr[l], e->level_big_ptr[l+1] - e->level_big_ptr[l],
                                e->level_big_max_r[l], e->level_big_max_nc[l], e->d_fronts, e->d_biginv, e->d_big_cnt + e->level_big_ptr[l],
// ... 317 lines not shown
  return rc ? -1 : 0;
}

__global__ void k_pack_panels(DlbFrontDev F, const double* __restrict__ fronts, const int* __restrict__ px, double* __restrict__ out)
{
  const int s = blockIdx.x;
  const int nc = F.sn_first[s+1] - F.sn_first[s], r = F.rows_ptr[s+1] - F.rows_ptr[s];
  const double* A = fronts + F.front_off[s];
  double* o = out + px[s];
  for(int idx = threadIdx.x; idx < r * nc; idx += blockDim.x) o[idx] = A[idx];
}
extern "C" int dlb_engine_export_factor(dlb_engine_t* e, const int* px, long long xsize, double* x_host)
{
  cudaSetDevice(e->device);
  if(e->type != DOGLEG_SPARSE) { g_last_error = "export_factor: sparse engines only (dense factors: dlb_engine_dense_factor_to_host)"; return -1; }
  if(e->factor_slot < 0) { g_last_error = "export_factor: no factorization available"; return -1; }
  int* d_px = 0; double* d_out = 0;
  CU(cudaMalloc(&d_px, sizeof(int) * ((size_t)e->F.nsuper + 1)));
  if(cudaMalloc(&d_out, sizeof(double) * (size_t)std::max<long long>(xsize, 1)) != cudaSuccess)
  { cudaFree(d_px); cudaGetLastError(); g_last_error = "export_factor: out of device memory"; return -1; }
  CU(cudaMemcpyAsync(d_px, px, sizeof(int) * ((size_t)e->F.nsuper + 1), cudaMemcpyHostToDevice, e->st));
  k_pack_panels<<<e->F.nsuper, 256, 0, e->st>>>(e->F, e->d_fronts, d_px, d_out);
  CU(cudaGetLastError());
  CU(cudaMemcpyAsync(x_host, d_out, sizeof(double) * (size_t)xsize, cudaMemcpyDeviceToHost, e->st));
  CU(cudaStreamSynchronize(e->st));
  cudaFree(d_px); cudaFree(d_out);
  e->n_launch += 1; e->n_d2h += sizeof(double) * (double)xsize;
  return 0;
}

extern "C" int dlb_engine_step(dlb_engine_t* e, int from, int to, int step_type, double delta)
{
  cudaSetDevice(e->device);
  Slot& A = e->slot[from & 1]; Slot& B = e->slot[to & 1];
  if(ensure_G(e, from)) return -1;
  {
    PhaseTimer tm(e, 6);
    dlb_launch_step(step_type, delta, A.d_p, A.d_Jtx, A.d_cauchy, A.d_gn, e->N, B.d_step, B.d_p,
                    e->d_part, e->d_counter, e->d_sc, e->sm_count, e->st);
    e->n_launch += step_type == DLB_STEP_INTERPOLATED ? 2 : 1;
    if(launch_norm2_Jv(e, A, B.d_step, &e->d_sc->norm2_Jstep)) return -1;
  }
  if(!e->lazy_p)
  {
    PhaseTimer tm(e, 7);
    CU(cudaMemcpyAsync(B.h_p, B.d_p, sizeof(double) * e->N, cudaMemcpyDeviceToHost, e->st));
    e->n_d2h += sizeof(double) * e->N;
  }
  return sync_scalars(e);
}

extern "C" int dlb_engine_has_trial(const dlb_engine_t* e) { return e->fused_trial ? 1 : 0; }
extern "C" int dlb_engine_has_fused_eval(const dlb_engine_t* e) { return e->fused_eval ? 1 : 0; }
extern "C" int dlb_engine_trial(dlb_engine_t* e, int from, int to, double delta, double lambda)
{
  cudaSetDevice(e->device);
  if(!e->fused_trial) { g_last_error = "dlb_engine_trial: this engine has no fused trial kernel (dlb_engine_has_trial)"; return -1; }
  Slot& A = e->slot[from & 1]; Slot& B = e->slot[to & 1];
  if(!A.have_G) { g_last_error = "dlb_engine_trial: the starting point has not been evaluated"; return -1; }
  if(A.have_gn && (e->factor_slot != (from & 1))) A.have_gn = false;
  if(!A.have_gn) e->factor_slot = -1;
  if(e->minor_dirty)
  {
    static const long long big2[2] = {LLONG_MAX, LLONG_MAX};
    CU(cudaMemcpyAsync(e->d_minor, big2, sizeof(big2), cudaMemcpyHostToDevice, e->st));
    e->minor_dirty = false;
  }
  DlbTrial T;
  memset(&T, 0, sizeof(T));
  T.nlev = (int)e->level_ptr.size() - 1; T.level_ptr = e->d_level_ptr; T.level_gt = e->d_level_gt;
  T.level_sg = e->d_level_sg; T.level_tmp = e->d_level_tmp;
  T.max_rows = e->max_front_rows; T.max_cols = e->max_front_cols; T.any_solve_gather = e->any_solve_gather ? 1 : 0;
  T.small_tail = 2 * (size_t)e->N * sizeof(double) <= dlb_trial_smem_bytes(e->max_front_rows) ? 1 : 0;
  T.Jtx = A.d_Jtx; T.p_from = A.d_p; T.Gpart = A.d_G; T.cauchy = A.d_cauchy; T.gn = A.d_gn;
  T.norm2_Jtx = A.norm2_Jtx; T.norm2_cauchy = A.norm2_cauchy; T.norm2_gn = A.norm2_gn;
  T.have_cauchy = A.have_cauchy ? 1 : 0; T.have_gn = A.have_gn ? 1 : 0;
  T.step = B.d_step; T.p_to = B.d_p; T.h_p_to = e->lazy_p ? NULL : B.h_p;
  T.fronts = e->d_fronts; T.ywork = e->d_ywork; T.zperm = e->d_zperm;
  T.part = e->d_trial_part; T.bar = e->d_bar;
  T.minor = e->d_minor + (e->trial_parity & 1); T.minor_next = e->d_minor + ((e->trial_parity + 1) & 1);
  e->trial_parity++;
  T.sc = e->d_sc; T.pub = e->d_pub; T.seq = ++e->seq;
  T.delta = delta; T.lambda = lambda; T.prof = e->d_prof;
  T.eg_ptr = e->d_eg_ptr; T.eg_dst = e->d_eg_dst; T.eg_sptr = e->d_eg_sptr; T.eg_src = e->d_eg_src;
  {
    PhaseTimer tm(e, 4);
    if(dlb_launch_trial(e->S, e->F, T, e->trial_grid, e->st))
    { g_last_error = std::string("cooperative launch of the trial kernel failed: ") + cudaGetErrorString(cudaGetLastError()); return -1; }
    e->n_launch += 1;
  }
  if(wait_published(e)) return -1;
  if(e->d_prof)
  {
    unsigned long long h[DLB_TRIAL_PROF_MAX + 1];
    CU(cudaStreamSynchronize(e->st));
    CU(cudaMemcpy(h, e->d_prof, sizeof(h), cudaMemcpyDeviceToHost));
    const int n = (int)std::min<unsigned long long>(h[DLB_TRIAL_PROF_MAX], DLB_TRIAL_PROF_MAX);
    fprintf(stderr, "libdogleg-b200: trial kernel phases (us):");
    for(int i = 1; i < n; i++) fprintf(stderr, " %.1f", 1e-3 * (double)(h[i] - h[i-1]));
    fprintf(stderr, "  total %.1f\n", n > 0 ? 1e-3 * (double)(h[n-1] - h[0]) : 0.0);
    dlb_trial_dbg_dump();
  }
  if(!e->lazy_p) e->n_d2h += sizeof(double) * e->N;
  const dlb_scalars_t* sc = e->h_sc;
  if(!A.have_cauchy) { A.have_cauchy = true; A.norm2_cauchy = sc->norm2_cauchy; }
  if(sc->minor >= 0) { if(e->factor_slot == (from & 1)) e->factor_slot = -1; e->n_factor += 1; return 0; }
  if(sc->trial_flags != 0.0)
  {
    A.have_gn = true; A.norm2_gn = sc->norm2_gn;
    e->factor_slot = from & 1; e->factor_lambda = lambda; e->asm_slot = from & 1;
    e->n_factor += 1;
  }
  return 0;
}

extern "C" void dlb_engine_set_lazy_p(dlb_engine_t* e, int on) { e->lazy_p = on != 0; }
extern "C" int dlb_engine_download_p(dlb_engine_t* e, int s)
{
  cudaSetDevice(e->device);
  Slot& L = e->slot[s & 1];
  CU(cudaMemcpyAsync(L.h_p, L.d_p, sizeof(double) * e->N, cudaMemcpyDeviceToHost, e->st));
  CU(cudaStreamSynchronize(e->st));
  e->n_d2h += sizeof(double) * e->N;
  return 0;
}

extern "C" int dlb_engine_download(dlb_engine_t* e, int s)
{
  cudaSetDevice(e->device);
  Slot& L = e->slot[s & 1];
  const size_t nb = sizeof(double) * e->N;
  CU(cudaMemcpyAsync(L.h_p, L.d_p, nb, cudaMemcpyDeviceToHost, e->st));
  CU(cudaMemcpyAsync(L.h_Jtx, L.d_Jtx, nb, cudaMemcpyDeviceToHost, e->st));
  CU(cudaMemcpyAsync(L.h_cauchy, L.d_cauchy, nb, cudaMemcpyDeviceToHost, e->st));
  CU(cudaMemcpyAsync(L.h_gn, L.d_gn, nb, cudaMemcpyDeviceToHost, e->st));
  CU(cudaMemcpyAsync(L.h_step, L.d_step, nb, cudaMemcpyDeviceToHost, e->st));
  CU(cudaStreamSynchronize(e->st));
  e->n_d2h += 5 * nb;
  return 0;
}

extern "C" int dlb_engine_download_inputs(dlb_engine_t* e, int s)
{
  cudaSetDevice(e->device);
  Slot& L = e->slot[s & 1];
  if(!e->host_inputs) return 0;
  if(L.h_x) CU(cudaMemcpyAsync(L.h_x, L.d_x + (e->gather ? e->col_begin : 0), sizeof(double) * e->M, cudaMemcpyDeviceToHost, e->st));
  CU(cudaMemcpyAsync(L.h_J, L.d_J + (e->gather ? e->slice_off : 0), sizeof(double) * e->Jcount, cudaMemcpyDeviceToHost, e->st));
  CU(cudaStreamSynchronize(e->st));
  e->n_d2h += sizeof(double) * (e->M + e->Jcount);
  return 0;
}

extern "C" int dlb_engine_debug_JtJ(dlb_engine_t* e, int s, double lambda, double* JtJ_out)
{
  cudaSetDevice(e->device);
  Slot& L = e->slot[s & 1];
  const size_t NN = (size_t)e->N * e->N;
  double* d_out = 0;
  CU(cudaMalloc(&d_out, sizeof(double) * NN));
  CU(cudaMemsetAsync(d_out, 0, sizeof(double) * NN, e->st));
  if(e->type == DOGLEG_SPARSE)
  {
    if(assemble(e, L, true)) return -1;
    const int nlev = (int)e->level_ptr.size() - 1;
    for(int l = 0; l < nlev; l++)
      dlb_launch_front_level(e->F, e->S, e->level_ptr[l], e->level_ptr[l+1], e->d_fronts, L.d_G, -1.0,
                             e->d_minor, e->level_rows[l], 0, e->st);
  }
  else if(dense_fill_front(e, L)) return -1;
  dlb_launch_fronts_to_dense(e->F, e->d_fronts, d_out, e->st);
  CU(cudaGetLastError());
  CU(cudaMemcpyAsync(JtJ_out, d_out, sizeof(double) * NN, cudaMemcpyDeviceToHost, e->st));
  CU(cudaStreamSynchronize(e->st));
  cudaFree(d_out);
  for(int i = 0; i < e->N; i++) JtJ_out[(size_t)i * e->N + i] += lambda;
  e->factor_slot = -1;
  return 0;
}

extern "C" int dlb_engine_dense_factor_to_host(dlb_engine_t* e, double* out)
{
  cudaSetDevice(e->device);
  if(e->type == DOGLEG_SPARSE) { g_last_error = "dense_factor_to_host: sparse engine"; return -1; }
  if(e->factor_slot < 0) return 0;
  const int packed = e->type == DOGLEG_DENSE ? 1 : e->packed;
  const int upper  = e->type == DOGLEG_DENSE ? 1 : e->upper;
  const size_t cnt = packed ? (size_t)e->N * (e->N + 1) / 2 : (size_t)e->N * e->N;
  double* d_out = 0;
  CU(cudaMalloc(&d_out, sizeof(double) * cnt));
  if(!packed)
    CU(cudaMemcpyAsync(d_out, e->slot[e->factor_slot].d_J, sizeof(double) * cnt, cudaMemcpyDeviceToDevice, e->st));
  dlb_launch_front_to_reference_layout(e->d_fronts, e->N, packed, upper, d_out, e->st);
  CU(cudaMemcpyAsync(out, d_out, sizeof(double) * cnt, cudaMemcpyDeviceToHost, e->st));
  CU(cudaStreamSynchronize(e->st));
  cudaFree(d_out);
  e->n_launch += 1; e->n_d2h += sizeof(double) * cnt;
  return 0;
}
```

libdogleg_b200/csrc/dlb_sparse.cu:

```cuda
#include "dlb_common.cuh"
#include "dlb_device.h"
#include "dlb_devfn.cuh"

#define TASK_WARPS (DLB_NT / 32)

__device__ __forceinline__ void warp_range(int m0, int m1, int w, int& a, int& b)
{
  int per = (m1 - m0 + TASK_WARPS - 1) / TASK_WARPS;
  per = (per + 3) & ~3;
  a = min(m1, m0 + w * per);
  b = min(m1, a + per);
}

#define PIPE_BC 16
#define PIPE_NST 3
#define PIPE_LD 33
#define PIPE_WARP_DOUBLES (PIPE_NST * PIPE_BC * PIPE_LD + PIPE_NST * PIPE_BC + 32)
__device__ __forceinline__ void cp_async8(void* smem, const void* gmem)
{
  const unsigned d = (unsigned)__cvta_generic_to_shared(smem);
  asm volatile("cp.async.ca.shared.global [%0], [%1], 8;" :: "r"(d), "l"(gmem) : "memory");
}
__device__ __forceinline__ void cp_async_commit() { asm volatile("cp.async.commit_group;" ::: "memory"); }
template<int N> __device__ __forceinline__ void cp_async_wait() { asm volatile("cp.async.wait_group %0;" :: "n"(N) : "memory"); }
// ... 480 lines not shown
      if(a == 0) { total = fma(d0, d0, total); total = fma(d1, d1, total); }
    }
  }
  double out[5];
  if(grid_reduce5(total, 0.0, 0.0, 0.0, 0.0, part, counter, out))
    *dst = out[0] + (add0 ? *add0 : 0.0) + (add1 ? *add1 : 0.0);
}

__device__ __forceinline__ void dmma_m8n8k4(double& d0, double& d1, double a, double b)
{
  asm volatile("mma.sync.aligned.m8n8k4.row.col.f64.f64.f64.f64 {%0,%1}, {%2}, {%3}, {%0,%1};"
               : "+d"(d0), "+d"(d1) : "d"(a), "d"(b));
}

template<int NTILE, bool GRAD>
__device__ __forceinline__ void assemble_task_dmma(const DlbSparseDev& S, const double* __restrict__ Jx,
                                                   const double* __restrict__ x, double* dst, double* dstg, double& n2,
                                                   int k, int m0, int m1, int lane)
{
  const int g = lane >> 2, tt = lane & 3;
  constexpr int NPAIR = NTILE * (NTILE + 1) / 2;
  double acc[NPAIR][2];
#pragma unroll
  for(int i = 0; i < NPAIR; i++) { acc[i][0] = 0.0; acc[i][1] = 0.0; }
  bool on[NTILE];
  double gacc[NTILE];
#pragma unroll
  for(int ti = 0; ti < NTILE; ti++) { on[ti] = 8 * ti + g < k; gacc[ti] = 0.0; }

#pragma unroll 4
  for(int m = m0; m < m1; m += 4)
  {
    const int mm = m + tt;
    const bool valid = mm < m1;
    const unsigned int pos = valid ? S.mem_pos[mm] : 0u;
    double xv = 0.0;
    if(GRAD) { xv = valid ? x[S.mem_col[mm]] : 0.0; if(g == 0) n2 = fma(xv, xv, n2); }
    double v[NTILE];
#pragma unroll
    for(int ti = 0; ti < NTILE; ti++) v[ti] = (valid && on[ti]) ? ldg_stream(Jx + pos + 8 * ti + g) : 0.0;
    if(GRAD)
    {
#pragma unroll
      for(int ti = 0; ti < NTILE; ti++) gacc[ti] = fma(v[ti], xv, gacc[ti]);
    }
    int idx = 0;
#pragma unroll
    for(int ti = 0; ti < NTILE; ti++)
#pragma unroll
      for(int tj = 0; tj <= ti; tj++, idx++) dmma_m8n8k4(acc[idx][0], acc[idx][1], v[ti], v[tj]);
  }
  int idx = 0;
#pragma unroll
  for(int ti = 0; ti < NTILE; ti++)
#pragma unroll
    for(int tj = 0; tj <= ti; tj++, idx++)
    {
      const int a = 8 * ti + g, b0 = 8 * tj + 2 * tt;
      if(a < k)
      {
        const int row = a * (a + 1) / 2;
        if(b0 <= a)     dst[row + b0]     = acc[idx][0];
        if(b0 + 1 <= a) dst[row + b0 + 1] = acc[idx][1];
      }
    }
  if(GRAD)
  {
#pragma unroll
    for(int ti = 0; ti < NTILE; ti++)
    {
      double s0 = gacc[ti];
      s0 += __shfl_xor_sync(0xffffffffu, s0, 1);
      s0 += __shfl_xor_sync(0xffffffffu, s0, 2);
      if(tt == 0 && on[ti]) dstg[8 * ti + g] = s0;
    }
  }
}
template<bool GRAD>
__device__ __forceinline__ void assemble_task_dmma_k(const DlbSparseDev& S, const double* __restrict__ Jx,
                                                     const double* __restrict__ x, double* dst, double* dstg, double& n2,
                                                     int k, int m0, int m1, int lane)
{
  if(k <= 8)       assemble_task_dmma<1, GRAD>(S, Jx, x, dst, dstg, n2, k, m0, m1, lane);
  else if(k <= 16) assemble_task_dmma<2, GRAD>(S, Jx, x, dst, dstg, n2, k, m0, m1, lane);
  else if(k <= 24) assemble_task_dmma<3, GRAD>(S, Jx, x, dst, dstg, n2, k, m0, m1, lane);
  else             assemble_task_dmma<4, GRAD>(S, Jx, x, dst, dstg, n2, k, m0, m1, lane);
}

#define ASM_ACC 8
__device__ __forceinline__ void assemble_task_scalar(const DlbSparseDev& S, const double* __restrict__ Jx,
                                                     double* __restrict__ Gpart, int t, int lane, int w)
{
  const int c  = S.task_cls[t];
  const int m0 = S.task_m0[t], m1 = S.task_m1[t];
  const int k  = S.cls_ptr[c+1] - S.cls_ptr[c];
  const int npairs = k * (k + 1) / 2;
  const long long Goff = S.task_Goff[t];
  for(int q0 = 32 * ASM_ACC * w; q0 < npairs; q0 += 32 * ASM_ACC * TASK_WARPS)
  {
    int pa[ASM_ACC], pb[ASM_ACC];
    double acc[ASM_ACC];
#pragma unroll
    for(int u = 0; u < ASM_ACC; u++)
    {
      const int q = q0 + u * 32 + lane;
      int a = 0, b = 0;
      if(q < npairs)
      {
        a = (int)((sqrt(8.0 * (double)q + 1.0) - 1.0) * 0.5);
        while((a + 1) * (a + 2) / 2 <= q) a++;
        while(a * (a + 1) / 2 > q) a--;
        b = q - a * (a + 1) / 2;
      }
      pa[u] = a; pb[u] = b; acc[u] = 0.0;
    }
    for(int m = m0; m < m1; m++)
    {
      const double* col = Jx + S.mem_pos[m];
#pragma unroll
      for(int u = 0; u < ASM_ACC; u++) acc[u] = fma(col[pa[u]], col[pb[u]], acc[u]);
    }
#pragma unroll
    for(int u = 0; u < ASM_ACC; u++)
    {
      const int q = q0 + u * 32 + lane;
      if(q < npairs) Gpart[Goff + q] = acc[u];
    }
  }
}

__device__ __forceinline__ void grad_task_scalar(const DlbSparseDev& S, const double* __restrict__ Jx, const double* __restrict__ x,
                                                 double* __restrict__ gdst, int t, int lane, int w, double& n2)
{
  const int c  = S.task_cls[t];
  const int m0 = S.task_m0[t], m1 = S.task_m1[t];
  const int k  = S.cls_ptr[c+1] - S.cls_ptr[c];
  for(int a0 = 32 * w; a0 < k; a0 += 32 * TASK_WARPS)
  {
    const int a = a0 + lane;
    double acc = 0.0;
    for(int m = m0; m < m1; m++)
    {
      const double xv = x[S.mem_col[m]];
      if(a < k) acc = fma(ldg_stream(Jx + S.mem_pos[m] + a), xv, acc);
    }
    if(a < k) gdst[a] = acc;
  }
  if(w == 0) for(int m = m0 + lane; m < m1; m += 32) { const double xv = x[S.mem_col[m]]; n2 = fma(xv, xv, n2); }
}

#define ASM_PAIRS_MAX 528
template<bool GRAD>
__global__ void __launch_bounds__(DLB_NT, 3)
k_sparse_assemble(DlbSparseDev S, const double* __restrict__ Jx, const double* __restrict__ x,
                  double* __restrict__ Gpart, double* __restrict__ gpart, double* __restrict__ n2part)
{
  __shared__ double shG[TASK_WARPS][ASM_PAIRS_MAX];
  __shared__ double shg[GRAD ? TASK_WARPS : 1][32];
  __shared__ double sh[32];
  const int lane = threadIdx.x & 31, w = threadIdx.x >> 5;
  double n2 = 0.0;
  for(int bt = blockIdx.x; bt < S.nbig; bt += gridDim.x)
  {
    const int t = S.big_tasks[bt];
    const int c = S.task_cls[t];
    const int k = S.cls_ptr[c+1] - S.cls_ptr[c];
    if(k > 32)
    {
      assemble_task_scalar(S, Jx, Gpart, t, lane, w);
      if(GRAD) grad_task_scalar(S, Jx, x, gpart + S.task_goff[t], t, lane, w, n2);
      continue;
    }
    int m0, m1;
    warp_range(S.task_m0[t], S.task_m1[t], w, m0, m1);
    assemble_task_dmma_k<GRAD>(S, Jx, x, shG[w], shg[GRAD ? w : 0], n2, k, m0, m1, lane);
    __syncthreads();
    const int npairs = k * (k + 1) / 2;
    const long long Goff = S.task_Goff[t];
    for(int q = threadIdx.x; q < npairs; q += DLB_NT)
    {
      double s0 = 0.0;
#pragma unroll
      for(int u = 0; u < TASK_WARPS; u++) s0 += shG[u][q];
      Gpart[Goff + q] = s0;
    }
    if(GRAD && threadIdx.x < k)
    {
      double s0 = 0.0;
#pragma unroll
      for(int u = 0; u < TASK_WARPS; u++) s0 += shg[GRAD ? u : 0][threadIdx.x];
      gpart[S.task_goff[t] + threadIdx.x] = s0;
    }
    __syncthreads();
  }
  if(GRAD)
  {
    n2 = block_sum(n2, sh);
    if(threadIdx.x == 0) n2part[blockIdx.x] = n2;
  }
}

template<bool GRAD>
__global__ void __launch_bounds__(DLB_NT)
k_sparse_assemble_small(DlbSparseDev S, const int* __restrict__ tasks, int ntasks,
                        const double* __restrict__ Jx, const double* __restrict__ x,
                        double* __restrict__ Gpart, double* __restrict__ gpart, double* __restrict__ n2part)
{
  __shared__ double sh[32];
  const int lane = threadIdx.x & 31;
  const int wg = blockIdx.x * TASK_WARPS + (threadIdx.x >> 5), nw = gridDim.x * TASK_WARPS;
  double n2 = 0.0;
  for(int st = wg; st < ntasks; st += nw)
  {
    const int t = tasks[st];
    const int c = S.task_cls[t];
    const int k = S.cls_ptr[c+1] - S.cls_ptr[c];
    assemble_task_dmma_k<GRAD>(S, Jx, x, Gpart + S.task_Goff[t], GRAD ? gpart + S.task_goff[t] : (double*)0, n2,
                               k, S.task_m0[t], S.task_m1[t], lane);
  }
  if(GRAD)
  {
    n2 = block_sum(n2, sh);
    if(threadIdx.x == 0) n2part[blockIdx.x] = n2;
  }
}

static inline int grid_for_tasks(int ntasks, int sm_count)
{
  const int cap = sm_count * 8;
  return ntasks < 1 ? 1 : (ntasks > cap ? cap : ntasks);
}
static inline int grid_for_warp_tasks(int ntasks, int sm_count)
{
  const int cap = sm_count * 2;
  const int g = (ntasks + TASK_WARPS - 1) / TASK_WARPS;
  return g < 1 ? 1 : (g > cap ? cap : g);
}
static inline int grid_for_small(int nsmall, int sm_count)
{
  const int cap = sm_count * 8;
  const int g = (nsmall + TASK_WARPS - 1) / TASK_WARPS;
  return g < 1 ? 1 : (g > cap ? cap : g);
}
static inline int grid_for_groups(int nsmall, int G, int sm_count)
{
  const int cap = sm_count * 8;
  const int per_cta = 2 * (DLB_NT / G);
  const int g = (nsmall + per_cta - 1) / per_cta;
  return g < 1 ? 1 : (g > cap ? cap : g);
}
static inline int grid_for_range(int nrange, int sm_count)
{
  const int cap = sm_count * 3;
  const int g = (nrange + TASK_WARPS - 1) / TASK_WARPS;
  return g < 1 ? 1 : (g > cap ? cap : g);
}
int dlb_sparse_n2part_size(const DlbSparseDev& S, int sm_count)
{
  const int a = grid_for_range(S.nrange, sm_count) + grid_for_warp_tasks(S.ngj_big, sm_count) + grid_for_groups(S.nsmall, 32, sm_count);
  const int b = grid_for_tasks(S.nbig, sm_count) + grid_for_small(S.nasm_small, sm_count) + grid_for_groups(S.nfused, 32, sm_count);
  return a > b ? a : b;
}

template<int CHUNK, int NST>
static void launch_range_grad(const DlbSparseDev& S, const double* Jx, const double* x, double* gpart, double* n2part,
                              int g0, int nu, cudaStream_t st)
{
  const size_t smem = sizeof(double) * TASK_WARPS * (NST * (CHUNK / 8 + 4) + 128 + 4);
  static DlbPerDeviceOnce attr_once;
  if(attr_once.first())
  {
    cudaFuncSetAttribute(k_range_grad<1, CHUNK, NST>, cudaFuncAttributeMaxDynamicSharedMemorySize, (int)smem);
    cudaFuncSetAttribute(k_range_grad<2, CHUNK, NST>, cudaFuncAttributeMaxDynamicSharedMemorySize, (int)smem);
    cudaFuncSetAttribute(k_range_grad<3, CHUNK, NST>, cudaFuncAttributeMaxDynamicSharedMemorySize, (int)smem);
    cudaFuncSetAttribute(k_range_grad<4, CHUNK, NST>, cudaFuncAttributeMaxDynamicSharedMemorySize, (int)smem);
  }
  if(nu <= 1)      k_range_grad<1, CHUNK, NST><<<g0, DLB_NT, smem, st>>>(S, Jx, x, gpart, n2part);
  else if(nu == 2) k_range_grad<2, CHUNK, NST><<<g0, DLB_NT, smem, st>>>(S, Jx, x, gpart, n2part);
  else if(nu == 3) k_range_grad<3, CHUNK, NST><<<g0, DLB_NT, smem, st>>>(S, Jx, x, gpart, n2part);
  else             k_range_grad<4, CHUNK, NST><<<g0, DLB_NT, smem, st>>>(S, Jx, x, gpart, n2part);
}

void dlb_launch_sparse_grad(const DlbSparseDev& S, const double* Jx, const double* x, double* gpart,
                            double* n2part, double* Jtx, double* part, unsigned int* counter,
                            DlbScalars* sc, int sm_count, cudaStream_t st)
{
  int g1 = 0;
  if(S.nrange > 0)
  {
    const int g0 = grid_for_range(S.nrange, sm_count);
    const int nu = (S.range_kmax + 31) / 32;
    launch_range_grad<RANGE_CHUNK, RANGE_NST>(S, Jx, x, gpart, n2part, g0, nu, st);
    g1 += g0;
  }
  if(S.ngj_big > 0)
  {
    const int gb = grid_for_warp_tasks(S.ngj_big, sm_count);
    const size_t smem = sizeof(double) * TASK_WARPS * PIPE_WARP_DOUBLES;
    static DlbPerDeviceOnce attr_once;
    if(attr_once.first()) { cudaFuncSetAttribute(k_sparse_grad, cudaFuncAttributeMaxDynamicSharedMemorySize, (int)smem); }
    k_sparse_grad<<<gb, DLB_NT, smem, st>>>(S, Jx, x, gpart, n2part + g1);
    g1 += gb;
  }
  if(S.nsmall > 0)
  {
    const int G = S.small_group;
    const int g2 = grid_for_groups(S.nsmall, G, sm_count);
    if(G == 8)       k_sparse_grad_small<8><<<g2, DLB_NT, 0, st>>>(S, S.small_info, S.nsmall, Jx, x, gpart, n2part + g1);
    else if(G == 16) k_sparse_grad_small<16><<<g2, DLB_NT, 0, st>>>(S, S.small_info, S.nsmall, Jx, x, gpart, n2part + g1);
    else             k_sparse_grad_small<32><<<g2, DLB_NT, 0, st>>>(S, S.small_info, S.nsmall, Jx, x, gpart, n2part + g1);
    g1 += g2;
  }
  int g = (S.n + DLB_NT - 1) / DLB_NT; if(g < (S.nmedium + 7) / 8) g = (S.nmedium + 7) / 8; if(g < S.nheavy) g = S.nheavy;
  if(g > sm_count * 8) g = sm_count * 8; if(g < 1) g = 1;
  k_sparse_grad_reduce<<<g, DLB_NT, 0, st>>>(S, gpart, n2part, g1, Jtx, part, counter, sc, (DlbPublished*)0, 0ull, 0);
}

int dlb_launch_sparse_eval_pass(const DlbSparseDev& S, const double* Jx, const double* x, double* Gpart, double* gpart,
                                double* n2part, int sm_count, cudaStream_t st)
{
  int g1 = 0;
  if(S.nbig > 0)
  {
    const int gb = grid_for_tasks(S.nbig, sm_count);
    k_sparse_assemble<true><<<gb, DLB_NT, 0, st>>>(S, Jx, x, Gpart, gpart, n2part);
    g1 += gb;
  }
  if(S.nasm_small > 0)
  {
    const int gs = grid_for_small(S.nasm_small, sm_count);
    k_sparse_assemble_small<true><<<gs, DLB_NT, 0, st>>>(S, S.asm_small_tasks, S.nasm_small, Jx, x, Gpart, gpart, n2part + g1);
    g1 += gs;
  }
  if(S.nfused > 0)
  {
    const int G = S.small_group;
    const int g2 = grid_for_groups(S.nfused, G, sm_count);
    if(G == 8)       k_sparse_grad_small<8><<<g2, DLB_NT, 0, st>>>(S, S.fused_info, S.nfused, Jx, x, gpart, n2part + g1);
    else if(G == 16) k_sparse_grad_small<16><<<g2, DLB_NT, 0, st>>>(S, S.fused_info, S.nfused, Jx, x, gpart, n2part + g1);
    else             k_sparse_grad_small<32><<<g2, DLB_NT, 0, st>>>(S, S.fused_info, S.nfused, Jx, x, gpart, n2part + g1);
    g1 += g2;
  }
  return g1;
}
void dlb_launch_sparse_eval_reduce(const DlbSparseDev& S, const double* gpart, const double* n2part, int n2count, double* Jtx,
                                   double* part, unsigned int* counter, DlbScalars* sc, DlbPublished* pub, unsigned long long seq,
                                   int n2_behind_Jtx, int sm_count, cudaStream_t st)
{
  int g = (S.n + DLB_NT - 1) / DLB_NT; if(g < (S.nmedium + 7) / 8) g = (S.nmedium + 7) / 8; if(g < S.nheavy) g = S.nheavy;
  if(g > sm_count * 8) g = sm_count * 8; if(g < 1) g = 1;
  k_sparse_grad_reduce<<<g, DLB_NT, 0, st>>>(S, gpart, n2part, n2count, Jtx, part, counter, sc, pub, seq, n2_behind_Jtx);
}

void dlb_launch_sparse_jv(const DlbSparseDev& S, const double* Jx, const double* v, double* part,
                          unsigned int* counter, double* dst, int sm_count, cudaStream_t st)
{
  double* scratch = part + 5 * (size_t)sm_count * 8 + 8;
  const int kinds = (S.nrange > 0) + (S.ngj_big > 0) + (S.nsmall > 0);
  int done = 0;
  const double* adds[2] = {NULL, NULL};
  auto target = [&]() { return done == kinds - 1 ? dst : scratch + done; };
  if(S.nrange > 0)
  {
    const size_t smem = sizeof(double) * TASK_WARPS * RANGE_WARP_DOUBLES;
    static DlbPerDeviceOnce attr_once;
    if(attr_once.first())
    {
      cudaFuncSetAttribute(k_range_jv<1>, cudaFuncAttributeMaxDynamicSharedMemorySize, (int)smem);
      cudaFuncSetAttribute(k_range_jv<2>, cudaFuncAttributeMaxDynamicSharedMemorySize, (int)smem);
      cudaFuncSetAttribute(k_range_jv<3>, cudaFuncAttributeMaxDynamicSharedMemorySize, (int)smem);
      cudaFuncSetAttribute(k_range_jv<4>, cudaFuncAttributeMaxDynamicSharedMemorySize, (int)smem);
    }
    double* out = target();
    const int gr = grid_for_range(S.nrange, sm_count), nu = (S.range_kmax + 31) / 32;
    if(nu <= 1)      k_range_jv<1><<<gr, DLB_NT, smem, st>>>(S, Jx, v, part, counter, adds[0], adds[1], out);
    else if(nu == 2) k_range_jv<2><<<gr, DLB_NT, smem, st>>>(S, Jx, v, part, counter, adds[0], adds[1], out);
    else if(nu == 3) k_range_jv<3><<<gr, DLB_NT, smem, st>>>(S, Jx, v, part, counter, adds[0], adds[1], out);
    else             k_range_jv<4><<<gr, DLB_NT, smem, st>>>(S, Jx, v, part, counter, adds[0], adds[1], out);
    if(out != dst) adds[done] = out;
    done++;
  }
  if(S.ngj_big > 0)
  {
    const size_t smem = sizeof(double) * TASK_WARPS * PIPE_WARP_DOUBLES;
    static DlbPerDeviceOnce attr_once;
    if(attr_once.first()) { cudaFuncSetAttribute(k_sparse_jv, cudaFuncAttributeMaxDynamicSharedMemorySize, (int)smem); }
    double* out = target();
    k_sparse_jv<<<grid_for_warp_tasks(S.ngj_big, sm_count), DLB_NT, smem, st>>>(S, Jx, v, part, counter, adds[0], adds[1], out);
    if(out != dst) adds[done] = out;
    done++;
  }
  if(S.nsmall > 0)
  {
    const int G = S.small_group;
    const int g2 = grid_for_groups(S.nsmall, G, sm_count);
    double* out = target();
    if(G == 8)       k_sparse_jv_small<8><<<g2, DLB_NT, 0, st>>>(S, S.small_info, S.nsmall, Jx, v, part, counter, adds[0], adds[1], out);
    else if(G == 16) k_sparse_jv_small<16><<<g2, DLB_NT, 0, st>>>(S, S.small_info, S.nsmall, Jx, v, part, counter, adds[0], adds[1], out);
    else             k_sparse_jv_small<32><<<g2, DLB_NT, 0, st>>>(S, S.small_info, S.nsmall, Jx, v, part, counter, adds[0], adds[1], out);
    done++;
  }
  if(kinds == 0) cudaMemsetAsync(dst, 0, sizeof(double), st);
}

__global__ void __launch_bounds__(DLB_NT)
k_gpart_quadform(DlbSparseDev S, const int* __restrict__ listA, int nA, const int* __restrict__ listB, int nB,
                 const double* __restrict__ Gpart, const double* __restrict__ v,
                 double* part, unsigned int* counter, const double* add0, double* dst)
{
  const double total = quadform_partial(S, listA, nA, listB, nB, Gpart, v, blockIdx.x * TASK_WARPS + (threadIdx.x >> 5),
                                        gridDim.x * TASK_WARPS, threadIdx.x & 31);
  double out[5];
  if(grid_reduce5(total, 0.0, 0.0, 0.0, 0.0, part, counter, out)) *dst = out[0] + (add0 ? *add0 : 0.0);
}

void dlb_launch_sparse_jv_quad(const DlbSparseDev& S, const double* Jx, const double* Gpart, const double* v, double* part,
                               unsigned int* counter, double* dst, int sm_count, cudaStream_t st)
{
  double* scratch = part + 5 * (size_t)sm_count * 8 + 8;
  const double* add = NULL;
  if(S.nfused > 0)
  {
    const int G = S.small_group;
    const int g2 = grid_for_groups(S.nfused, G, sm_count);
    double* out = (S.nbig + S.nasm_small > 0) ? scratch : dst;
    if(G == 8)       k_sparse_jv_small<8><<<g2, DLB_NT, 0, st>>>(S, S.fused_info, S.nfused, Jx, v, part, counter, NULL, NULL, out);
    else if(G == 16) k_sparse_jv_small<16><<<g2, DLB_NT, 0, st>>>(S, S.fused_info, S.nfused, Jx, v, part, counter, NULL, NULL, out);
    else             k_sparse_jv_small<32><<<g2, DLB_NT, 0, st>>>(S, S.fused_info, S.nfused, Jx, v, part, counter, NULL, NULL, out);
    if(out != dst) add = out;
  }
  const int nt = S.nbig + S.nasm_small;
  if(nt > 0)
  {
    int g = (nt + TASK_WARPS - 1) / TASK_WARPS;
    if(g > sm_count * 8) g = sm_count * 8;
    k_gpart_quadform<<<g, DLB_NT, 0, st>>>(S, S.big_tasks, S.nbig, S.asm_small_tasks, S.nasm_small, Gpart, v, part, counter, add, dst);
  }
  else if(S.nfused == 0) cudaMemsetAsync(dst, 0, sizeof(double), st);
}

void dlb_launch_sparse_assemble(const DlbSparseDev& S, const double* Jx, double* Gpart, int all_small,
                                int sm_count, cudaStream_t st)
{
  if(S.nbig > 0)   k_sparse_assemble<false><<<grid_for_tasks(S.nbig, sm_count), DLB_NT, 0, st>>>(S, Jx, (const double*)0, Gpart, (double*)0, (double*)0);
  const int* tasks = all_small ? S.small_tasks : S.asm_small_tasks;
  const int nt = all_small ? S.nsmall : S.nasm_small;
  if(nt > 0) k_sparse_assemble_small<false><<<grid_for_small(nt, sm_count), DLB_NT, 0, st>>>(S, tasks, nt, Jx, (const double*)0, Gpart, (double*)0, (double*)0);
}
```

libdogleg_b200/csrc/dlb_taskplan.cpp:

```cpp
#include "dlb_taskplan.h"
#include <algorithm>
#include <climits>
#include <cstring>

void dlb_build_task_plan(const DlbSymbolic& Y, const int* Jp, int cbk, int Mk, int n_state, int sm_count,
                         bool ranges_enabled, DlbTaskPlan& T, bool one_task_per_class)
{
  T = DlbTaskPlan();
  const int target = sm_count * 8;
  const int chunk = one_task_per_class ? INT_MAX : std::max(512, (Mk + target - 1) / target);
  std::vector<int>& task_cls = T.task_cls; std::vector<int>& task_m0 = T.task_m0; std::vector<int>& task_m1 = T.task_m1;
  std::vector<int>& cls_task_ptr = T.cls_task_ptr; cls_task_ptr.assign(Y.ncls + 1, 0);
  std::vector<long long>& task_goff = T.task_goff; std::vector<long long>& task_Goff = T.task_Goff;
  long long& goff = T.goff; long long& Goff = T.Goff;
  std::vector<int>& lmem_col = T.mem_col; lmem_col.reserve(Mk);
  std::vector<unsigned int>& mem_pos = T.mem_pos; mem_pos.reserve(Mk);
  for(int c = 0; c < Y.ncls; c++)
  {
    const int* mb = Y.mem_col.data() + Y.mem_ptr[c];
    const int* me = Y.mem_col.data() + Y.mem_ptr[c+1];
    const int* lo = std::lower_bound(mb, me, cbk);
    const int* hi = std::lower_bound(mb, me, cbk + Mk);
    const int first = (int)lmem_col.size();
    for(const int* q = lo; q < hi; q++) { lmem_col.push_back(*q - cbk); mem_pos.push_back((unsigned int)(Jp[*q] - Jp[cbk])); }
    const int nmem = (int)lmem_col.size() - first;
    const int k = Y.cls_ptr[c+1] - Y.cls_ptr[c];
    const int nt = std::max(1, (nmem + chunk - 1) / chunk);
    const int per = (nmem + nt - 1) / nt;
    cls_task_ptr[c] = (int)task_cls.size();
    for(int t = 0; t < nt; t++)
    {
      const int m0 = first + t * per, m1 = std::min(first + nmem, m0 + per);
      if(m0 >= m1 && t > 0) break;
      task_cls.push_back(c); task_m0.push_back(m0); task_m1.push_back(std::max(m0, m1));
      task_goff.push_back(goff); task_Goff.push_back(Goff);
      goff += k; Goff += (long long)k * (k + 1) / 2;
    }
  }
  cls_task_ptr[Y.ncls] = (int)task_cls.size();
  const int ntasks = (int)task_cls.size();
  const int SMALL_MEMBERS = 32;
  std::vector<int>& big_tasks = T.big_tasks; std::vector<int>& small_tasks = T.small_tasks;
  for(int t = 0; t < ntasks; t++)
  {
    const int c = task_cls[t];
    const bool small = task_m1[t] - task_m0[t] <= SMALL_MEMBERS && Y.cls_ptr[c+1] - Y.cls_ptr[c] <= 32;
    (small ? small_tasks : big_tasks).push_back(t);
  }
  std::vector<DlbRangeTask>& rtasks = T.rtasks;
  std::vector<char>& ranged = T.ranged; ranged.assign(Y.ncls, 0);
  std::vector<int>& gp_count = T.gp_count; gp_count.assign(Y.ncls, 0);
  std::vector<long long>& gp_first = T.gp_first; gp_first.assign(Y.ncls, 0);
  int& range_kmax = T.range_kmax; range_kmax = 1;
  {
    const bool enabled = ranges_enabled;
    struct Run { int j0, n, P; bool ok; };
    std::vector<Run> runs;
    const int Ml = Mk;
    auto cls = [&](int j) { return Y.cls_of_col[cbk + j]; };
    auto klen = [&](int j) { return Jp[cbk + j + 1] - Jp[cbk + j]; };
    for(int j = 0; enabled && j < Ml; )
    {
      int bestP = 0, bestLen = 0;
      for(int P = 1; P <= 4 && j + P <= Ml; P++)
      {
        bool distinct = true;
        for(int a = 0; a < P; a++) for(int b = a + 1; b < P; b++) if(cls(j + a) == cls(j + b)) distinct = false;
        if(!distinct) continue;
        int len = P;
        while(j + len < Ml && cls(j + len) == cls(j + len - P)) len++;
        len -= len % P;
        if(len > bestLen) { bestLen = len; bestP = P; }
      }
      int Ktot = 0;
      for(int i = 0; i < bestP; i++) Ktot += klen(j + i);
      if(bestP > 0 && bestLen >= 64 * bestP && Ktot <= 128 && Ktot > 0) { runs.push_back({j, bestLen, bestP, true}); j += bestLen; }
      else j++;
    }
    std::vector<int> nlocal(Y.ncls, 0), inrun(Y.ncls, 0);
    for(int t = 0; t < ntasks; t++) nlocal[task_cls[t]] += task_m1[t] - task_m0[t];
    for(bool changed = true; changed; )
    {
      changed = false;
      std::fill(inrun.begin(), inrun.end(), 0);
      for(const Run& r : runs) if(r.ok) for(int i = 0; i < r.P; i++) inrun[cls(r.j0 + i)] += r.n / r.P;
      for(Run& r : runs)
        if(r.ok)
          for(int i = 0; i < r.P; i++)
            if(inrun[cls(r.j0 + i)] != nlocal[cls(r.j0 + i)]) { r.ok = false; changed = true; break; }
    }
    const int want = std::max(64, Ml / std::max(1, sm_count * 32));
    for(const Run& r : runs)
    {
      if(!r.ok) continue;
      const int per_periods = std::max(1, want / r.P);
      const int nper = r.n / r.P;
      const int nt = (nper + per_periods - 1) / per_periods, each = (nper + nt - 1) / nt;
      for(int t = 0; t < nt; t++)
      {
        const int q0 = t * each, q1 = std::min(nper, q0 + each);
        if(q0 >= q1) break;
        DlbRangeTask rt; memset(&rt, 0, sizeof(rt));
        rt.j0 = r.j0 + q0 * r.P; rt.ncols = (q1 - q0) * r.P; rt.P = r.P;
        rt.pos0 = (unsigned int)(Jp[cbk + rt.j0] - Jp[cbk]);
        int off = 0;
        for(int i = 0; i < r.P; i++) { rt.cls[i] = cls(r.j0 + i); rt.koff[i] = off; off += klen(r.j0 + i); ranged[rt.cls[i]] = 1; gp_count[rt.cls[i]]++; }
        rt.Ktot = off;
        range_kmax = std::max(range_kmax, off);
        rtasks.push_back(rt);
      }
    }
    for(int c = 0; c < Y.ncls; c++)
    {
      const int k = Y.cls_ptr[c+1] - Y.cls_ptr[c];
      if(ranged[c]) { gp_first[c] = goff; goff += (long long)k * gp_count[c]; gp_count[c] = 0; }
      else { gp_first[c] = task_goff[cls_task_ptr[c]]; gp_count[c] = cls_task_ptr[c+1] - cls_task_ptr[c]; }
    }
    for(DlbRangeTask& rt : rtasks)
      for(int i = 0; i < rt.P; i++)
      {
        const int c = rt.cls[i], k = Y.cls_ptr[c+1] - Y.cls_ptr[c];
        rt.goff[i] = gp_first[c] + (long long)k * gp_count[c]++;
      }
  }
  std::vector<int>& gj_big_tasks = T.gj_big_tasks;
  for(int t : big_tasks) if(!ranged[task_cls[t]]) gj_big_tasks.push_back(t);

  std::vector<int>& ginv_ptr = T.ginv_ptr; ginv_ptr.assign(n_state + 1, 0);
  for(int c = 0; c < Y.ncls; c++)
    for(int q = Y.cls_ptr[c]; q < Y.cls_ptr[c+1]; q++) ginv_ptr[Y.cls_rows[q] + 1]++;
  for(int i = 0; i < n_state; i++) ginv_ptr[i+1] += ginv_ptr[i];
  std::vector<int>& ginv_cls = T.ginv_cls; ginv_cls.assign(ginv_ptr[n_state], 0);
  std::vector<long long>& ginv_off = T.ginv_off; ginv_off.assign(ginv_ptr[n_state], 0);
  {
    std::vector<int> fill(ginv_ptr.begin(), ginv_ptr.end() - 1);
    for(int c = 0; c < Y.ncls; c++)
      for(int q = Y.cls_ptr[c]; q < Y.cls_ptr[c+1]; q++)
      {
        const int at = fill[Y.cls_rows[q]]++;
        ginv_cls[at] = gp_count[c] == 1 ? -1 : c;
        ginv_off[at] = gp_first[c] + (q - Y.cls_ptr[c]);
      }
  }

  const int heavy_threshold = T.heavy_threshold;
  std::vector<int>& heavy_state = T.heavy_state; std::vector<int>& medium_state = T.medium_state;
  for(int i = 0; i < n_state; i++)
  {
    const int cnt = ginv_ptr[i+1] - ginv_ptr[i];
    if(cnt >= heavy_threshold) heavy_state.push_back(i);
    else if(cnt >= DLB_LIGHT_MAX) medium_state.push_back(i);
  }
}
```

libdogleg_b200/csrc/dlb_taskplan.h:

```cpp
#pragma once
#include "dlb_symbolic.h"
#include <vector>

#define DLB_LIGHT_MAX 8

struct alignas(16) DlbRangeTask
{
  int j0, ncols, P, Ktot;
  unsigned int pos0; int pad[3];
  int cls[4], koff[4];
  long long goff[4];
};

struct DlbTaskPlan
{
  std::vector<int> task_cls, task_m0, task_m1;
  std::vector<int> cls_task_ptr;
  std::vector<long long> task_goff;
  std::vector<long long> task_Goff;
  std::vector<int> mem_col;
  std::vector<unsigned int> mem_pos;
  std::vector<int> big_tasks, small_tasks;
  std::vector<DlbRangeTask> rtasks;
  std::vector<char> ranged;
  int range_kmax = 1;
  std::vector<int> gj_big_tasks;
  std::vector<int> gp_count;
  std::vector<long long> gp_first;
  std::vector<int> ginv_ptr, ginv_cls;
  std::vector<long long> ginv_off;
  int heavy_threshold = 256;
  std::vector<int> heavy_state, medium_state;
  long long goff = 0, Goff = 0;
};

void dlb_build_task_plan(const DlbSymbolic& Y, const int* Jp, int cbk, int Mk, int n_state, int sm_count,
                         bool ranges_enabled, DlbTaskPlan& T, bool one_task_per_class = false);
```

libdogleg_b200/ffi.py:

```python
import ctypes as C
import os
import subprocess

HERE = os.path.dirname(os.path.abspath(__file__))
ROOT = os.path.dirname(HERE)

SOLVE_DENSE, SOLVE_SPARSE, SOLVE_DENSE_PRODUCTS = 0, 1, 2
DEBUG_VNLOG = 1 << 30
BUF_P, BUF_X, BUF_JTX, BUF_CAUCHY, BUF_GN, BUF_STEP, BUF_JVALUES, BUF_JP, BUF_JI, BUF_NORM2X = range(10)
STEP_CAUCHY, STEP_GAUSSNEWTON, STEP_INTERPOLATED = 0, 1, 2
BATCH_UNFINISHED, BATCH_GRADIENT, BATCH_STEP, BATCH_TRUSTREGION, BATCH_MAX_ITERATIONS = range(5)
SYM = dict(perm=0, parent=1, colcount=2, sn_first=3, rows_ptr=4, rows=5, sn_parent=6,
           cls_of_col=7, cls_front=8, sn_level=9, rel=10, child_ptr=11, child_list=12, level_ptr=13,
           level_sn=14, cls_ptr=15, cls_rows=16, cls_loc=17, mem_ptr=18, mem_col=19)
TP = dict(task_cls=0, task_m0=1, task_m1=2, cls_task_ptr=3, task_goff=4, task_Goff=5, mem_col=6, mem_pos=7,
          big_tasks=8, small_tasks=9, gj_big_tasks=10, ranged=11, gp_count=12, gp_first=13, ginv_ptr=14,
          ginv_cls=15, ginv_off=16, heavy=17, medium=18, sizes=19, range_tasks=20)
GP = dict(dst=0, src_ptr=1, src_base=2, ld=3, h=4, w=5, src_ld=6, level_ptr=7, tmp_off=8, level_tmp=9,
          sg_flag=10)


class Parameters(C.Structure):
    _fields_ = [("max_iterations", C.c_int), ("dogleg_debug", C.c_int),
                ("trustregion0", C.c_double),
                ("trustregion_decrease_factor", C.c_double), ("trustregion_decrease_threshold", C.c_double),
                ("trustregion_increase_factor", C.c_double), ("trustregion_increase_threshold", C.c_double),
                ("Jt_x_threshold", C.c_double), ("update_threshold", C.c_double),
                ("trustregion_threshold", C.c_double)]

    def set_flags(self, debug=False, packed=False, upper=False, vnlog=False):
        self.dogleg_debug = (1 if debug else 0) | (2 if packed else 0) | (4 if upper else 0) | \
                            (DEBUG_VNLOG if vnlog else 0)


class Scalars(C.Structure):
    _fields_ = [(n, C.c_double) for n in
                ("norm2_x", "norm2_Jtx", "maxabs_Jtx", "norm2_JJtx", "k_cauchy", "norm2_cauchy", "norm2_gn",
                 "norm2_step", "k_interp", "Jtx_dot_step", "maxabs_step", "norm2_Jstep", "discriminant",
                 "step_type", "trial_flags")] + [("minor", C.c_longlong)]


def lib_path():
    return os.path.join(HERE, "libdogleg.so")


def build(verbose=False):
    cmd = ["make", "-C", os.path.join(HERE, "csrc"), "-j8"]
    out = subprocess.run(cmd, capture_output=True, text=True)
    if out.returncode != 0:
        raise RuntimeError("building libdogleg.so failed:\n" + out.stdout[-4000:] + out.stderr[-4000:])
    if verbose:
        print(out.stdout[-2000:])
    return lib_path()


_lib = None


def load():
    global _lib
    if _lib is not None:
        return _lib
    path = lib_path()
    if not os.path.exists(path):
        raise RuntimeError(f"{path} is missing: run `python -c 'import __graft_entry__ as g; g.build()'`")
    L = C.CDLL(path, mode=C.RTLD_LOCAL)
    dp, ip, vp = C.POINTER(C.c_double), C.POINTER(C.c_int), C.c_void_p
    PP = C.POINTER(Parameters)
    L.dogleg_getDefaultParameters.argtypes = [PP]
    L.dogleg_getDefaultParameters.restype = None
    L.dogleg_optimize2.argtypes = [dp, C.c_uint, C.c_uint, C.c_uint, vp, vp, PP, C.POINTER(vp)]
    L.dogleg_optimize2.restype = C.c_double
    L.dogleg_optimize.argtypes = [dp, C.c_uint, C.c_uint, C.c_uint, vp, vp, C.POINTER(vp)]
    L.dogleg_optimize.restype = C.c_double
    L.dogleg_optimize_dense2.argtypes = [dp, C.c_uint, C.c_uint, vp, vp, PP, C.POINTER(vp)]
    L.dogleg_optimize_dense2.restype = C.c_double
    L.dogleg_optimize_dense.argtypes = [dp, C.c_uint, C.c_uint, vp, vp, C.POINTER(vp)]
    L.dogleg_optimize_dense.restype = C.c_double
    L.dogleg_optimize_dense_products.argtypes = [dp, C.c_uint, vp, vp, PP, C.POINTER(vp)]
    L.dogleg_optimize_dense_products.restype = C.c_double
    L.dogleg_freeContext.argtypes = [C.POINTER(vp)]
    L.dogleg_freeContext.restype = None
    L.dogleg_computeJtJfactorization.argtypes = [vp, vp]
    L.dogleg_computeJtJfactorization.restype = C.c_bool
    L.dogleg_setDebug.argtypes = [C.c_int]
    L.dogleg_setMaxIterations.argtypes = [C.c_int]
    L.dogleg_setInitialTrustregion.argtypes = [C.c_double]
    L.dogleg_setThresholds.argtypes = [C.c_double] * 3
    L.dogleg_setTrustregionUpdateParameters.argtypes = [C.c_double] * 4
    L.dogleg_gpu_device_count.restype = C.c_int
    L.dogleg_gpu_set_device.argtypes = [C.c_int]
    L.dogleg_gpu_last_error.restype = C.c_char_p
    L.dogleg_gpu_version.restype = C.c_char_p
    L.dogleg_gpu_set_permutation.argtypes = [ip, C.c_int, C.c_int]
    L.dogleg_gpu_set_permutation.restype = None
    L.dogleg_gpu_get_stats.argtypes = [vp, dp]
    L.dogleg_gpu_get_stats.restype = None
    L.dogleg_gpu_get_phase_ms.argtypes = [dp]
    L.dogleg_gpu_get_phase_ms.restype = None
    L.dogleg_gpu_optimize_sparse.argtypes = [dp, C.c_uint, C.c_uint, C.c_uint, ip, ip, vp, vp, PP, C.POINTER(vp)]
    L.dogleg_gpu_optimize_sparse.restype = C.c_double
    L.dogleg_gpu_optimize_dense.argtypes = [dp, C.c_uint, C.c_uint, vp, vp, PP, C.POINTER(vp)]
    L.dogleg_gpu_optimize_dense.restype = C.c_double
    L.dogleg_gpu_optimize_dense_batched.argtypes = [dp, C.c_uint, C.c_uint, C.c_uint, vp, vp, PP, dp, ip]
    L.dogleg_gpu_optimize_dense_batched.restype = C.c_int
    L.dogleg_gpu_optimize_dense_products.argtypes = [dp, C.c_uint, vp, vp, PP, C.POINTER(vp)]
    L.dogleg_gpu_optimize_dense_products.restype = C.c_double
    L.dogleg_gpu_optimize_dense_products_batched.argtypes = [dp, C.c_uint, C.c_uint, vp, vp, PP, dp, ip]
    L.dogleg_gpu_optimize_dense_products_batched.restype = C.c_int
    L.dogleg_gpu_optimize_dense_batched2.argtypes = [dp, C.c_uint, C.c_uint, C.c_uint, vp, vp, PP, dp, ip, C.POINTER(vp)]
    L.dogleg_gpu_optimize_dense_batched2.restype = C.c_int
    L.dogleg_gpu_optimize_dense_products_batched2.argtypes = [dp, C.c_uint, C.c_uint, vp, vp, PP, dp, ip, C.POINTER(vp)]
    L.dogleg_gpu_optimize_dense_products_batched2.restype = C.c_int
    L.dogleg_gpu_batch_status.argtypes = [vp, ip, dp]
    L.dogleg_gpu_batch_status.restype = C.c_int
    L.dogleg_gpu_batch_solve.argtypes = [vp, dp, dp, C.c_int]
    L.dogleg_gpu_batch_solve.restype = C.c_int
    L.dogleg_gpu_batch_solve_device.argtypes = [vp, vp, vp, C.c_int, vp]
    L.dogleg_gpu_batch_solve_device.restype = C.c_int
    L.dogleg_gpu_batch_covariance.argtypes = [vp, dp, C.c_int]
    L.dogleg_gpu_batch_covariance.restype = C.c_int
    L.dogleg_gpu_batch_covariance_device.argtypes = [vp, vp, C.c_int, vp]
    L.dogleg_gpu_batch_covariance_device.restype = C.c_int
    L.dogleg_gpu_batch_free.argtypes = [C.POINTER(vp)]
    L.dogleg_gpu_batch_free.restype = None
    L.dogleg_gpu_release_batched_cache.restype = None
    L.dogleg_gpu_batched_stats.argtypes = [dp]
    L.dogleg_gpu_batched_stats.restype = None
    L.dogleg_gpu_nccl_get_unique_id.argtypes = [vp]
    L.dogleg_gpu_nccl_init.argtypes = [C.c_int, C.c_int, vp]
    L.dogleg_gpu_nccl_finalize.restype = None
    L.dogleg_gpu_nccl_world.restype = C.c_int
    L.dogleg_gpu_optimize_sparse_sharded.argtypes = [dp, C.c_uint, C.c_uint, ip, ip, C.c_uint, C.c_uint, vp, vp, vp, PP,
                                                     C.POINTER(vp)]
    L.dogleg_gpu_optimize_sparse_sharded.restype = C.c_double
    L.dogleg_gpu_optimize_dense_sharded.argtypes = [dp, C.c_uint, C.c_uint, C.c_uint, C.c_uint, vp, vp, vp, PP, C.POINTER(vp)]
    L.dogleg_gpu_optimize_dense_sharded.restype = C.c_double
    L.dlb_engine_create3.argtypes = [C.c_int, C.c_uint, C.c_uint, C.c_uint, C.c_int, C.c_int, C.c_int, C.c_uint, C.c_uint]
    L.dlb_engine_create3.restype = vp
    L.dogleg_gpu_get_comm_stats.argtypes = [dp]
    L.dogleg_gpu_get_comm_stats.restype = None
    L.dlb_engine_comm_stats.argtypes = [vp, dp]
    L.dlb_engine_comm_stats.restype = None
    L.dlb_symbolic_create.argtypes = [C.c_int, C.c_int, ip, ip, ip, C.c_int]
    L.dlb_symbolic_create.restype = vp
    L.dlb_symbolic_free.argtypes = [vp]
    L.dlb_symbolic_free.restype = None
    L.dlb_symbolic_info.argtypes = [vp, C.POINTER(C.c_longlong)]
    L.dlb_symbolic_info.restype = None
    L.dlb_symbolic_get.argtypes = [vp, C.c_int, ip, C.c_longlong]
    L.dlb_symbolic_get.restype = C.c_longlong
    llp = C.POINTER(C.c_longlong)
    L.dlb_symbolic_front_off.argtypes = [vp, llp, C.c_longlong]
    L.dlb_symbolic_front_off.restype = C.c_longlong
    L.dlb_gather_plan_create.argtypes = [vp, C.c_int, C.c_int, C.c_int, C.c_int, C.c_int]
    L.dlb_gather_plan_create.restype = vp
    L.dlb_gather_plan_free.argtypes = [vp]
    L.dlb_gather_plan_free.restype = None
    L.dlb_gather_plan_info.argtypes = [vp, llp]
    L.dlb_gather_plan_info.restype = None
    L.dlb_gather_plan_get.argtypes = [vp, C.c_int, C.c_int, llp, C.c_longlong]
    L.dlb_gather_plan_get.restype = C.c_longlong
    L.dlb_task_plan_create.argtypes = [vp, ip, C.c_int, C.c_int, C.c_int, C.c_int]
    L.dlb_task_plan_create.restype = vp
    L.dlb_task_plan_free.argtypes = [vp]
    L.dlb_task_plan_free.restype = None
    L.dlb_task_plan_get.argtypes = [vp, C.c_int, llp, C.c_longlong]
    L.dlb_task_plan_get.restype = C.c_longlong
    L.dlb_engine_create.argtypes = [C.c_int, C.c_uint, C.c_uint, C.c_uint, C.c_int, C.c_int]
    L.dlb_engine_create.restype = vp
    L.dlb_engine_create2.argtypes = [C.c_int, C.c_uint, C.c_uint, C.c_uint, C.c_int, C.c_int, C.c_int]
    L.dlb_engine_create2.restype = vp
    L.dogleg_gpu_release_cache.restype = None
    L.dlb_engine_destroy.argtypes = [vp]
    L.dlb_engine_destroy.restype = None
    L.dlb_engine_host_buffer.argtypes = [vp, C.c_int, C.c_int]
    L.dlb_engine_host_buffer.restype = vp
    L.dlb_engine_device_buffer.argtypes = [vp, C.c_int, C.c_int]
    L.dlb_engine_device_buffer.restype = vp
    L.dlb_engine_stream.argtypes = [vp]
    L.dlb_engine_stream.restype = vp
    L.dlb_engine_set_pattern.argtypes = [vp, ip, ip, ip, C.c_int]
    L.dlb_engine_symbolic.argtypes = [vp]
    L.dlb_engine_symbolic.restype = vp
    L.dlb_engine_evaluate.argtypes = [vp, C.c_int, C.c_int, C.c_double]
    L.dlb_engine_cauchy.argtypes = [vp, C.c_int]
    L.dlb_engine_factorize.argtypes = [vp, C.c_int, C.c_double]
    L.dlb_engine_gauss_newton.argtypes = [vp, C.c_int]
    L.dlb_engine_step.argtypes = [vp, C.c_int, C.c_int, C.c_int, C.c_double]
    L.dlb_engine_has_trial.argtypes = [vp]
    L.dlb_engine_has_fused_eval.argtypes = [vp]
    L.dlb_engine_has_fused_eval.restype = C.c_int
    L.dlb_engine_trial.argtypes = [vp, C.c_int, C.c_int, C.c_double, C.c_double]
    L.dlb_engine_download.argtypes = [vp, C.c_int]
    L.dlb_engine_upload_p.argtypes = [vp, C.c_int]
    L.dlb_engine_scalars.argtypes = [vp]
    L.dlb_engine_scalars.restype = C.POINTER(Scalars)
    L.dlb_engine_solve.argtypes = [vp, dp, dp, C.c_int]
    L.dlb_engine_debug_JtJ.argtypes = [vp, C.c_int, C.c_double, dp]
    L.dlb_engine_dense_factor_to_host.argtypes = [vp, dp]
    L.dlb_engine_counters.argtypes = [vp, dp]
    L.dlb_engine_counters.restype = None
    L.dlb_engine_enable_timing.argtypes = [vp, C.c_int]
    L.dlb_engine_enable_timing.restype = None
    L.dlb_engine_phase_ms.argtypes = [vp, dp]
    L.dlb_engine_phase_ms.restype = None
    _lib = L
    return L


def default_parameters():
    P = Parameters()
    load().dogleg_getDefaultParameters(C.byref(P))
    return P
```

Baseline: 2344.

## Add eval-run kernel streaming contiguous J runs via bulk async copies

Adds a task-plan mode that groups consecutive columns sharing the same set of small classes into 'eval runs'. A new templated kernel streams each run's J values and x with TMA bulk copies through an mbarrier ring buffer and accumulates the class blocks and gradient using DMMA tensor-core tiles. It replaces the per-task indexed gathers in the fused-eval path. Remaining big tasks go to the existing assemble kernel, which now takes an explicit task list. The x buffer is padded for aligned bulk reads, and the change adds template instantiations, dynamic shared memory and an extra launch.

After: 2438 (median of 6 runs). +4.0%, better.

```diff
diff --git a/include/dogleg_gpu.h b/include/dogleg_gpu.h
--- a/include/dogleg_gpu.h
+++ b/include/dogleg_gpu.h
@@ -135,13 +135,18 @@
 typedef struct dlb_task_plan dlb_task_plan_t;
 dlb_task_plan_t* dlb_task_plan_create(const dlb_symbolic_t* S, const int* Jp, int col_begin, int ncols,
                                       int sm_count, int ranges_enabled);
+enum { DLB_TP_FLAG_RANGES = 1, DLB_TP_FLAG_EVAL_RUNS = 2, DLB_TP_FLAG_ONE_TASK = 4 };
+dlb_task_plan_t* dlb_task_plan_create2(const dlb_symbolic_t* S, const int* Jp, int col_begin, int ncols,
+                                       int sm_count, int flags);
 void            dlb_task_plan_free(dlb_task_plan_t* T);
 enum { DLB_TP_TASK_CLS = 0, DLB_TP_TASK_M0 = 1, DLB_TP_TASK_M1 = 2, DLB_TP_CLS_TASK_PTR = 3, DLB_TP_TASK_GOFF = 4,
        DLB_TP_TASK_GGOFF = 5, DLB_TP_MEM_COL = 6, DLB_TP_MEM_POS = 7, DLB_TP_BIG_TASKS = 8, DLB_TP_SMALL_TASKS = 9,
        DLB_TP_GJ_BIG_TASKS = 10, DLB_TP_RANGED = 11, DLB_TP_GP_COUNT = 12, DLB_TP_GP_FIRST = 13, DLB_TP_GINV_PTR = 14,
        DLB_TP_GINV_CLS = 15, DLB_TP_GINV_OFF = 16, DLB_TP_HEAVY = 17, DLB_TP_MEDIUM = 18,
        DLB_TP_SIZES = 19,
-       DLB_TP_RANGE_TASKS = 20    };
+       DLB_TP_RANGE_TASKS = 20,
+       DLB_TP_EVAL_RUNS = 21,
+       DLB_TP_EBIG_TASKS = 22     };
 long long       dlb_task_plan_get(const dlb_task_plan_t* T, int what, long long* out, long long cap);
 
 typedef struct dlb_engine dlb_engine_t;
@@ -200,6 +205,7 @@
 
 int  dlb_engine_solve(dlb_engine_t* e, const double* B, double* X, int nrhs);
 int  dlb_engine_debug_JtJ(dlb_engine_t* e, int slot, double lambda, double* JtJ_out);
+long long dlb_engine_debug_class_blocks(dlb_engine_t* e, int slot, double* out, long long cap);
 int  dlb_engine_dense_factor_to_host(dlb_engine_t* e, double* out);
 
 void dlb_engine_counters(const dlb_engine_t* e, double out[4]);
diff --git a/libdogleg_b200/csrc/dlb_capi_symbolic.cpp b/libdogleg_b200/csrc/dlb_capi_symbolic.cpp
--- a/libdogleg_b200/csrc/dlb_capi_symbolic.cpp
+++ b/libdogleg_b200/csrc/dlb_capi_symbolic.cpp
@@ -124,6 +124,16 @@
   if(!Jp || col_begin < 0 || ncols < 0 || col_begin + ncols > S.m) { dlb_set_error("task plan: bad column range"); return NULL; }
   dlb_task_plan* t = new dlb_task_plan();
   dlb_build_task_plan(S, Jp, col_begin, ncols, S.n, sm_count > 0 ? sm_count : 148, ranges_enabled != 0, t->T);
+  return t;
+}
+extern "C" dlb_task_plan_t* dlb_task_plan_create2(const dlb_symbolic_t* h, const int* Jp, int col_begin, int ncols,
+                                                  int sm_count, int flags)
+{
+  const DlbSymbolic& S = sym(h);
+  if(!Jp || col_begin < 0 || ncols < 0 || col_begin + ncols > S.m) { dlb_set_error("task plan: bad column range"); return NULL; }
+  dlb_task_plan* t = new dlb_task_plan();
+  dlb_build_task_plan(S, Jp, col_begin, ncols, S.n, sm_count > 0 ? sm_count : 148, (flags & DLB_TP_FLAG_RANGES) != 0, t->T,
+                      (flags & DLB_TP_FLAG_ONE_TASK) != 0, (flags & DLB_TP_FLAG_EVAL_RUNS) != 0);
   return t;
 }
 extern "C" void dlb_task_plan_free(dlb_task_plan_t* t) { delete t; }
@@ -169,6 +179,19 @@
     }
     return n;
   }
+  case DLB_TP_EVAL_RUNS:
+  {
+    const long long n = (long long)T.eruns.size() * 21;
+    for(size_t r = 0; out && r < T.eruns.size() && (long long)(r + 1) * 21 <= cap; r++)
+    {
+      const DlbEvalRun& R = T.eruns[r];
+      long long* o = out + r * 21;
+      o[0] = R.j0; o[1] = R.nper; o[2] = R.P; o[3] = R.Ktot; o[4] = R.pos0;
+      for(int i = 0; i < 4; i++) { o[5 + i] = R.k[i]; o[9 + i] = R.koff[i]; o[13 + i] = R.goff[i]; o[17 + i] = R.Goff[i]; }
+    }
+    return n;
+  }
+  case DLB_TP_EBIG_TASKS:   return copy_wide(T.ebig_tasks, out, cap);
   default: return -1;
   }
 }
diff --git a/libdogleg_b200/csrc/dlb_device.h b/libdogleg_b200/csrc/dlb_device.h
--- a/libdogleg_b200/csrc/dlb_device.h
+++ b/libdogleg_b200/csrc/dlb_device.h
@@ -40,6 +40,9 @@
   const int* asm_small_tasks;
   int nfused;
   const DlbSmallTask* fused_info;
+  int nerun, erun_P, erun_ntile, nebig;
+  const DlbEvalRun* eruns;
+  const int* ebig_tasks;
   int nheavy, heavy_threshold;
   const int* heavy_state;
   int nmedium;
diff --git a/libdogleg_b200/csrc/dlb_engine.cu b/libdogleg_b200/csrc/dlb_engine.cu
--- a/libdogleg_b200/csrc/dlb_engine.cu
+++ b/libdogleg_b200/csrc/dlb_engine.cu
@@ -420,7 +420,7 @@
     Slot& L = e->slot[s];
     hostalloc(N, &L.h_p); hostalloc(N, &L.h_Jtx); hostalloc(N, &L.h_cauchy); hostalloc(N, &L.h_gn); hostalloc(N, &L.h_step);
     devalloc(N, &L.d_p);  devalloc(N + 1, &L.d_Jtx);  devalloc(N, &L.d_cauchy);  devalloc(N, &L.d_gn);  devalloc(N, &L.d_step);
-    if(solve_type != DOGLEG_DENSE_PRODUCTS) { if(e->host_inputs) hostalloc(M, &L.h_x); if(!e->gather) devalloc(M, &L.d_x); }
+    if(solve_type != DOGLEG_DENSE_PRODUCTS) { if(e->host_inputs) hostalloc(M, &L.h_x); if(!e->gather) devalloc(M + 2, &L.d_x); }
     if(e->host_inputs) hostalloc(e->Jcount, &L.h_J);
     if(!e->gather) devalloc(e->Jcount + 2, &L.d_J);
     if(solve_type == DOGLEG_SPARSE && e->host_inputs) { hostalloc(M + 1, &L.h_Jp); hostalloc(NJnnz, &L.h_Ji); }
@@ -675,7 +675,7 @@
       if(L.d_x) cudaFree(L.d_x);
       if(L.d_J) cudaFree(L.d_J);
       L.d_x = L.d_J = 0;
-      CU(cudaMalloc(&L.d_x, sizeof(double) * std::max<size_t>(Mtot, 1)));
+      CU(cudaMalloc(&L.d_x, sizeof(double) * (Mtot + 2)));
       CU(cudaMalloc(&L.d_J, sizeof(double) * (nnz_full + 2)));
     }
     e->slice_off = Jp[cb];
@@ -711,7 +711,8 @@
   DlbTaskPlan TP;
   {
     const char* renv = getenv("DOGLEG_GPU_RANGE");
-    dlb_build_task_plan(Y, Jp, cbk, Mk, e->N, e->sm_count, !e->fused_eval && !(renv && atoi(renv) == 0), TP, e->G_global);
+    const bool runs = !(renv && atoi(renv) == 0);
+    dlb_build_task_plan(Y, Jp, cbk, Mk, e->N, e->sm_count, !e->fused_eval && runs, TP, e->G_global, e->fused_eval && runs);
   }
   const std::vector<int>& task_cls = TP.task_cls; const std::vector<int>& task_m0 = TP.task_m0;
   const std::vector<int>& task_m1 = TP.task_m1;   const std::vector<int>& cls_task_ptr = TP.cls_task_ptr;
@@ -745,6 +746,8 @@
   rc |= dev_upload(e, big_tasks, &S.big_tasks);   rc |= dev_upload(e, small_tasks, &S.small_tasks);
   rc |= dev_upload(e, rtasks, &S.rtasks);         rc |= dev_upload(e, gj_big_tasks, &S.gj_big_tasks);
   rc |= dev_upload(e, gp_count, &S.gp_count);
+  S.nerun = (int)TP.eruns.size(); S.erun_P = TP.erun_P; S.erun_ntile = TP.erun_ntile; S.nebig = (int)TP.ebig_tasks.size();
+  rc |= dev_upload(e, TP.eruns, &S.eruns);       rc |= dev_upload(e, TP.ebig_tasks, &S.ebig_tasks);
   {
     std::vector<DlbSmallTask> info(small_tasks.size());
     int kmax = 1;
@@ -1148,7 +1151,7 @@
       dlb_launch_sparse_eval_reduce(e->S, e->d_gpart, e->d_n2part, n2count, L.d_Jtx, e->d_part, e->d_counter, e->d_sc, e->d_pub,
                                     e->seq, 0, e->sm_count, e->st);
     }
-    e->n_launch += 1 + (e->S.nbig > 0) + (e->S.nasm_small > 0) + (e->S.nfused > 0);
+    e->n_launch += 1 + (e->S.nebig > 0) + (e->S.nasm_small > 0) + (e->S.nfused > 0) + (e->S.nerun > 0);
     L.have_G = true;
     if(e->G_shared) e->slot[1 - (s & 1)].have_G = false;
     CU(cudaGetLastError());
@@ -1772,6 +1775,19 @@
   return 0;
 }
 
+extern "C" long long dlb_engine_debug_class_blocks(dlb_engine_t* e, int s, double* out, long long cap)
+{
+  cudaSetDevice(e->device);
+  Slot& L = e->slot[s & 1];
+  if(e->type != DOGLEG_SPARSE || !L.d_G) return -1;
+  const long long n = e->Goff_total;
+  if(out && cap > 0)
+  {
+    CU(cudaMemcpyAsync(out, L.d_G, sizeof(double) * (size_t)std::min(n, cap), cudaMemcpyDeviceToHost, e->st));
+    CU(cudaStreamSynchronize(e->st));
+  }
+  return n;
+}
 extern "C" int dlb_engine_debug_JtJ(dlb_engine_t* e, int s, double lambda, double* JtJ_out)
 {
   cudaSetDevice(e->device);
diff --git a/libdogleg_b200/csrc/dlb_sparse.cu b/libdogleg_b200/csrc/dlb_sparse.cu
--- a/libdogleg_b200/csrc/dlb_sparse.cu
+++ b/libdogleg_b200/csrc/dlb_sparse.cu
@@ -656,17 +656,17 @@
 #define ASM_PAIRS_MAX 528
 template<bool GRAD>
 __global__ void __launch_bounds__(DLB_NT, 3)
-k_sparse_assemble(DlbSparseDev S, const double* __restrict__ Jx, const double* __restrict__ x,
-                  double* __restrict__ Gpart, double* __restrict__ gpart, double* __restrict__ n2part)
+k_sparse_assemble(DlbSparseDev S, const int* __restrict__ tasks, int ntasks, const double* __restrict__ Jx,
+                  const double* __restrict__ x, double* __restrict__ Gpart, double* __restrict__ gpart, double* __restrict__ n2part)
 {
   __shared__ double shG[TASK_WARPS][ASM_PAIRS_MAX];
   __shared__ double shg[GRAD ? TASK_WARPS : 1][32];
   __shared__ double sh[32];
   const int lane = threadIdx.x & 31, w = threadIdx.x >> 5;
   double n2 = 0.0;
-  for(int bt = blockIdx.x; bt < S.nbig; bt += gridDim.x)
-  {
-    const int t = S.big_tasks[bt];
+  for(int bt = blockIdx.x; bt < ntasks; bt += gridDim.x)
+  {
+    const int t = tasks[bt];
     const int c = S.task_cls[t];
     const int k = S.cls_ptr[c+1] - S.cls_ptr[c];
     if(k > 32)
@@ -729,6 +729,208 @@
   }
 }
 
+
+#define EVR_NST 3
+#define EVR_XST 36
+__host__ __device__ constexpr int evr_kmax(int P, int NTILE) { return 8 * P * NTILE < 128 ? 8 * P * NTILE : 128; }
+__host__ __device__ constexpr int evr_stage_j(int P, int NTILE)
+{ return 32 * evr_kmax(P, NTILE) * (3072 / (32 * evr_kmax(P, NTILE)) > 1 ? 3072 / (32 * evr_kmax(P, NTILE)) : 1); }
+__host__ __device__ constexpr size_t evr_smem(int P, int NTILE)
+{
+  return sizeof(double) * (size_t)TASK_WARPS * (EVR_NST * (evr_stage_j(P, NTILE) / 8 + 4 + EVR_XST) + 4 * NTILE * (8 * NTILE + 1) + 32 * P) +
+         sizeof(unsigned long long) * TASK_WARPS * EVR_NST;
+}
+__host__ __device__ constexpr int evr_min_blocks(int P, int NTILE)
+{ return P * NTILE * (NTILE + 1) <= 24 && 2 * (evr_smem(P, NTILE) + 1024 + 256) <= 228 * 1024 ? 2 : 1; }
+template<int P, int NTILE>
+struct EvrGeom
+{
+  static constexpr int STAGE_J = evr_stage_j(P, NTILE);
+  static constexpr int STAGE = STAGE_J / 8 + 4 + EVR_XST;
+  static constexpr int TRI = 8 * NTILE * (8 * NTILE + 1) / 2;
+  static constexpr int NPAIR = NTILE * (NTILE + 1) / 2;
+  static constexpr size_t SMEM = evr_smem(P, NTILE);
+};
+
+struct EvrCursor
+{
+  int r, q, b, cp, P, Ktot, j0; unsigned int pos0;
+  __device__ __forceinline__ void load(const DlbEvalRun* runs, int w, int stage_j)
+  {
+    const DlbEvalRun& R = runs[r];
+    P = R.P; Ktot = R.Ktot; j0 = R.j0; pos0 = R.pos0;
+    warp_range(0, R.nper, w, q, b);
+    cp = 4 * max(1, min(stage_j / (32 * Ktot), 8 / P));
+  }
+  __device__ __forceinline__ void seek(const DlbEvalRun* runs, int nruns, int w, int stage_j)
+  {
+    while(r < nruns && q >= b) { r += gridDim.x; if(r < nruns) load(runs, w, stage_j); }
+  }
+};
+__device__ __forceinline__ void evr_issue(const EvrCursor& c, const double* Jx, const double* x, double* stage, double* xstage,
+                                          unsigned long long* bar, int lane)
+{
+  if(lane != 0) return;
+  const int n = min(c.cp, c.b - c.q);
+  const unsigned long long b0 = ((unsigned long long)c.pos0 + (unsigned long long)c.q * c.Ktot) * 8ull;
+  const unsigned long long b1 = b0 + (unsigned long long)n * c.Ktot * 8ull;
+  const unsigned long long a0 = b0 & ~15ull, a1 = (b1 + 15ull) & ~15ull;
+  const unsigned long long x0 = (unsigned long long)(c.j0 + c.q * c.P) * 8ull, x1 = x0 + (unsigned long long)n * c.P * 8ull;
+  const unsigned long long xa0 = x0 & ~15ull, xa1 = (x1 + 15ull) & ~15ull;
+  mbar_expect_tx(bar, (unsigned)(a1 - a0 + xa1 - xa0));
+  bulk_g2s(stage, (const char*)Jx + a0, (unsigned)(a1 - a0), bar);
+  bulk_g2s(xstage, (const char*)x + xa0, (unsigned)(xa1 - xa0), bar);
+}
+
+template<int P, int NTILE>
+__global__ void __launch_bounds__(DLB_NT, evr_min_blocks(P, NTILE))
+k_eval_runs(const DlbEvalRun* __restrict__ runs, int nruns, const double* __restrict__ Jx, const double* __restrict__ x,
+            double* __restrict__ Gpart, double* __restrict__ gpart, double* __restrict__ n2part)
+{
+  using Geo = EvrGeom<P, NTILE>;
+  constexpr int STAGE = Geo::STAGE, XOFF = Geo::STAGE_J / 8 + 4, NPAIR = Geo::NPAIR, TRI = Geo::TRI;
+  __shared__ double sh[32];
+  extern __shared__ __align__(16) double sh_evr[];
+  const int lane = threadIdx.x & 31, w = threadIdx.x >> 5, g = lane >> 2, tt = lane & 3;
+  double* ring = sh_evr + (size_t)w * EVR_NST * STAGE;
+  double* shG = sh_evr + (size_t)TASK_WARPS * EVR_NST * STAGE;
+  double* shg = shG + (size_t)TASK_WARPS * TRI;
+  unsigned long long* bars = (unsigned long long*)(shg + (size_t)TASK_WARPS * 32 * P) + w * EVR_NST;
+  if(lane == 0) for(int st = 0; st < EVR_NST; st++) mbar_init(bars + st, 1);
+  asm volatile("fence.mbarrier_init.release.cluster;" ::: "memory");
+  __syncwarp();
+
+  EvrCursor cur;
+  cur.r = blockIdx.x; cur.q = cur.b = 0;
+  if(cur.r < nruns) cur.load(runs, w, Geo::STAGE_J);
+  cur.seek(runs, nruns, w, Geo::STAGE_J);
+  int ist = 0, cst = 0;
+  unsigned phase_bits = 0;
+  auto issue_next = [&]() {
+    if(cur.r >= nruns) return;
+    const int st = ist % EVR_NST;
+    evr_issue(cur, Jx, x, ring + st * STAGE, ring + st * STAGE + XOFF, bars + st, lane);
+    ist++;
+    cur.q += cur.cp;
+    cur.seek(runs, nruns, w, Geo::STAGE_J);
+  };
+  for(int c = 0; c < EVR_NST - 1; c++) issue_next();
+
+  double n2 = 0.0;
+  for(int r = blockIdx.x; r < nruns; r += gridDim.x)
+  {
+    const DlbEvalRun& R = runs[r];
+    const int Pr = R.P, Ktot = R.Ktot, j0 = R.j0;
+    const unsigned int pos0 = R.pos0;
+    int kk[P], ko[P], nt[P];
+#pragma unroll
+    for(int i = 0; i < P; i++) { kk[i] = i < Pr ? R.k[i] : 0; ko[i] = i < Pr ? R.koff[i] : 0; nt[i] = (kk[i] + 7) / 8; }
+    int a, b;
+    warp_range(0, R.nper, w, a, b);
+    const int cp = 4 * max(1, min(Geo::STAGE_J / (32 * Ktot), 8 / Pr));
+    double acc[P][NPAIR][2], gacc[P][NTILE];
+#pragma unroll
+    for(int i = 0; i < P; i++)
+    {
+#pragma unroll
+      for(int p = 0; p < NPAIR; p++) { acc[i][p][0] = 0.0; acc[i][p][1] = 0.0; }
+#pragma unroll
+      for(int ti = 0; ti < NTILE; ti++) gacc[i][ti] = 0.0;
+    }
+    for(int q0 = a; q0 < b; q0 += cp)
+    {
+      issue_next();
+      const int nq = min(cp, b - q0), st = cst % EVR_NST;
+      cst++;
+      mbar_wait(bars + st, (phase_bits >> st) & 1u);
+      phase_bits ^= 1u << st;
+      const double* tl = ring + st * STAGE + ((pos0 + (unsigned)q0 * Ktot) & 1u);
+      const double* xs = ring + st * STAGE + XOFF + ((j0 + q0 * Pr) & 1);
+      if(lane < nq * Pr) n2 = fma(xs[lane], xs[lane], n2);
+      for(int m = 0; m < nq; m += 4)
+      {
+        const int mm = m + tt;
+        const bool valid = mm < nq;
+#pragma unroll
+        for(int i = 0; i < P; i++)
+        {
+          if(i >= Pr) break;
+          const double xv = valid ? xs[mm * Pr + i] : 0.0;
+          const double* col = tl + mm * Ktot + ko[i] + g;
+          double v[NTILE];
+#pragma unroll
+          for(int ti = 0; ti < NTILE; ti++) v[ti] = (valid && 8 * ti + g < kk[i]) ? col[8 * ti] : 0.0;
+#pragma unroll
+          for(int ti = 0; ti < NTILE; ti++) gacc[i][ti] = fma(v[ti], xv, gacc[i][ti]);
+          int idx = 0;
+#pragma unroll
+          for(int ti = 0; ti < NTILE; ti++)
+#pragma unroll
+            for(int tj = 0; tj <= ti; tj++, idx++)
+              if(ti < nt[i]) dmma_m8n8k4(acc[i][idx][0], acc[i][idx][1], v[ti], v[tj]);
+        }
+      }
+      __syncwarp();
+    }
+#pragma unroll
+    for(int i = 0; i < P; i++)
+    {
+      if(i >= Pr) break;
+      double* dst = shG + (size_t)w * TRI;
+      int idx = 0;
+#pragma unroll
+      for(int ti = 0; ti < NTILE; ti++)
+#pragma unroll
+        for(int tj = 0; tj <= ti; tj++, idx++)
+        {
+          const int aa = 8 * ti + g, b0 = 8 * tj + 2 * tt;
+          if(aa < kk[i])
+          {
+            const int row = aa * (aa + 1) / 2;
+            if(b0 <= aa)     dst[row + b0]     = acc[i][idx][0];
+            if(b0 + 1 <= aa) dst[row + b0 + 1] = acc[i][idx][1];
+          }
+        }
+      if(i == 0)
+#pragma unroll
+        for(int i2 = 0; i2 < P; i2++)
+#pragma unroll
+          for(int ti = 0; ti < NTILE; ti++)
+          {
+            double s0 = gacc[i2][ti];
+            s0 += __shfl_xor_sync(0xffffffffu, s0, 1);
+            s0 += __shfl_xor_sync(0xffffffffu, s0, 2);
+            if(tt == 0 && 8 * ti + g < kk[i2]) shg[(size_t)w * 32 * P + 32 * i2 + 8 * ti + g] = s0;
+          }
+      __syncthreads();
+      const int npairs = kk[i] * (kk[i] + 1) / 2;
+      const long long Goff = R.Goff[i];
+      for(int q = threadIdx.x; q < npairs; q += DLB_NT)
+      {
+        double s0 = 0.0;
+#pragma unroll
+        for(int u = 0; u < TASK_WARPS; u++) s0 += shG[(size_t)u * TRI + q];
+        Gpart[Goff + q] = s0;
+      }
+      if(i == 0)
+        for(int t = threadIdx.x; t < 32 * Pr; t += DLB_NT)
+        {
+          const int i2 = t >> 5, e = t & 31;
+          if(e < R.k[i2])
+          {
+            double s0 = 0.0;
+#pragma unroll
+            for(int u = 0; u < TASK_WARPS; u++) s0 += shg[(size_t)u * 32 * P + t];
+            gpart[pick4(i2, R.goff[0], R.goff[1], R.goff[2], R.goff[3]) + e] = s0;
+          }
+        }
+      __syncthreads();
+    }
+  }
+  n2 = block_sum(n2, sh);
+  if(threadIdx.x == 0) n2part[blockIdx.x] = n2;
+}
+
 static inline int grid_for_tasks(int ntasks, int sm_count)
 {
   const int cap = sm_count * 8;
@@ -759,10 +961,26 @@
   const int g = (nrange + TASK_WARPS - 1) / TASK_WARPS;
   return g < 1 ? 1 : (g > cap ? cap : g);
 }
+static inline int grid_for_eval_runs(int nrun, int P, int ntile, int sm_count)
+{
+  const int cap = sm_count * evr_min_blocks(P, ntile);
+  const int per = (nrun + cap - 1) / cap;
+  return nrun < 1 ? 1 : (nrun + per - 1) / per;
+}
+template<int P, int NTILE>
+static void launch_eval_runs(const DlbSparseDev& S, const double* Jx, const double* x, double* Gpart, double* gpart,
+                             double* n2part, int grid, cudaStream_t st)
+{
+  static DlbPerDeviceOnce attr_once;
+  if(attr_once.first())
+    cudaFuncSetAttribute(k_eval_runs<P, NTILE>, cudaFuncAttributeMaxDynamicSharedMemorySize, (int)EvrGeom<P, NTILE>::SMEM);
+  k_eval_runs<P, NTILE><<<grid, DLB_NT, EvrGeom<P, NTILE>::SMEM, st>>>(S.eruns, S.nerun, Jx, x, Gpart, gpart, n2part);
+}
 int dlb_sparse_n2part_size(const DlbSparseDev& S, int sm_count)
 {
   const int a = grid_for_range(S.nrange, sm_count) + grid_for_warp_tasks(S.ngj_big, sm_count) + grid_for_groups(S.nsmall, 32, sm_count);
-  const int b = grid_for_tasks(S.nbig, sm_count) + grid_for_small(S.nasm_small, sm_count) + grid_for_groups(S.nfused, 32, sm_count);
+  const int b = grid_for_tasks(S.nbig, sm_count) + grid_for_small(S.nasm_small, sm_count) + grid_for_groups(S.nfused, 32, sm_count) +
+                (S.nerun > 0 ? grid_for_eval_runs(S.nerun, S.erun_P, S.erun_ntile < 1 ? 1 : S.erun_ntile, sm_count) : 0);
   return a > b ? a : b;
 }
 
@@ -824,10 +1042,10 @@
                                 double* n2part, int sm_count, cudaStream_t st)
 {
   int g1 = 0;
-  if(S.nbig > 0)
-  {
-    const int gb = grid_for_tasks(S.nbig, sm_count);
-    k_sparse_assemble<true><<<gb, DLB_NT, 0, st>>>(S, Jx, x, Gpart, gpart, n2part);
+  if(S.nebig > 0)
+  {
+    const int gb = grid_for_tasks(S.nebig, sm_count);
+    k_sparse_assemble<true><<<gb, DLB_NT, 0, st>>>(S, S.ebig_tasks, S.nebig, Jx, x, Gpart, gpart, n2part);
     g1 += gb;
   }
   if(S.nasm_small > 0)
@@ -844,6 +1062,32 @@
     else if(G == 16) k_sparse_grad_small<16><<<g2, DLB_NT, 0, st>>>(S, S.fused_info, S.nfused, Jx, x, gpart, n2part + g1);
     else             k_sparse_grad_small<32><<<g2, DLB_NT, 0, st>>>(S, S.fused_info, S.nfused, Jx, x, gpart, n2part + g1);
     g1 += g2;
+  }
+  if(S.nerun > 0)
+  {
+    const int nt = S.erun_ntile < 1 ? 1 : S.erun_ntile;
+    const int ge = grid_for_eval_runs(S.nerun, S.erun_P, nt, sm_count);
+    double* n2 = n2part + g1;
+    switch(4 * (S.erun_P - 1) + nt - 1)
+    {
+    case 0:  launch_eval_runs<1, 1>(S, Jx, x, Gpart, gpart, n2, ge, st); break;
+    case 1:  launch_eval_runs<1, 2>(S, Jx, x, Gpart, gpart, n2, ge, st); break;
+    case 2:  launch_eval_runs<1, 3>(S, Jx, x, Gpart, gpart, n2, ge, st); break;
+    case 3:  launch_eval_runs<1, 4>(S, Jx, x, Gpart, gpart, n2, ge, st); break;
+    case 4:  launch_eval_runs<2, 1>(S, Jx, x, Gpart, gpart, n2, ge, st); break;
+    case 5:  launch_eval_runs<2, 2>(S, Jx, x, Gpart, gpart, n2, ge, st); break;
+    case 6:  launch_eval_runs<2, 3>(S, Jx, x, Gpart, gpart, n2, ge, st); break;
+    case 7:  launch_eval_runs<2, 4>(S, Jx, x, Gpart, gpart, n2, ge, st); break;
+    case 8:  launch_eval_runs<3, 1>(S, Jx, x, Gpart, gpart, n2, ge, st); break;
+    case 9:  launch_eval_runs<3, 2>(S, Jx, x, Gpart, gpart, n2, ge, st); break;
+    case 10: launch_eval_runs<3, 3>(S, Jx, x, Gpart, gpart, n2, ge, st); break;
+    case 11: launch_eval_runs<3, 4>(S, Jx, x, Gpart, gpart, n2, ge, st); break;
+    case 12: launch_eval_runs<4, 1>(S, Jx, x, Gpart, gpart, n2, ge, st); break;
+    case 13: launch_eval_runs<4, 2>(S, Jx, x, Gpart, gpart, n2, ge, st); break;
+    case 14: launch_eval_runs<4, 3>(S, Jx, x, Gpart, gpart, n2, ge, st); break;
+    default: launch_eval_runs<4, 4>(S, Jx, x, Gpart, gpart, n2, ge, st); break;
+    }
+    g1 += ge;
   }
   return g1;
 }
@@ -946,7 +1190,8 @@
 void dlb_launch_sparse_assemble(const DlbSparseDev& S, const double* Jx, double* Gpart, int all_small,
                                 int sm_count, cudaStream_t st)
 {
-  if(S.nbig > 0)   k_sparse_assemble<false><<<grid_for_tasks(S.nbig, sm_count), DLB_NT, 0, st>>>(S, Jx, (const double*)0, Gpart, (double*)0, (double*)0);
+  if(S.nbig > 0)   k_sparse_assemble<false><<<grid_for_tasks(S.nbig, sm_count), DLB_NT, 0, st>>>(S, S.big_tasks, S.nbig, Jx, (const double*)0,
+                                                                                                 Gpart, (double*)0, (double*)0);
   const int* tasks = all_small ? S.small_tasks : S.asm_small_tasks;
   const int nt = all_small ? S.nsmall : S.nasm_small;
   if(nt > 0) k_sparse_assemble_small<false><<<grid_for_small(nt, sm_count), DLB_NT, 0, st>>>(S, tasks, nt, Jx, (const double*)0, Gpart, (double*)0, (double*)0);
diff --git a/libdogleg_b200/csrc/dlb_taskplan.cpp b/libdogleg_b200/csrc/dlb_taskplan.cpp
--- a/libdogleg_b200/csrc/dlb_taskplan.cpp
+++ b/libdogleg_b200/csrc/dlb_taskplan.cpp
@@ -4,7 +4,7 @@
 #include <cstring>
 
 void dlb_build_task_plan(const DlbSymbolic& Y, const int* Jp, int cbk, int Mk, int n_state, int sm_count,
-                         bool ranges_enabled, DlbTaskPlan& T, bool one_task_per_class)
+                         bool ranges_enabled, DlbTaskPlan& T, bool one_task_per_class, bool eval_runs)
 {
   T = DlbTaskPlan();
   const int target = sm_count * 8;
@@ -53,7 +53,7 @@
   std::vector<long long>& gp_first = T.gp_first; gp_first.assign(Y.ncls, 0);
   int& range_kmax = T.range_kmax; range_kmax = 1;
   {
-    const bool enabled = ranges_enabled;
+    const bool enabled = ranges_enabled || eval_runs;
     struct Run { int j0, n, P; bool ok; };
     std::vector<Run> runs;
     const int Ml = Mk;
@@ -79,6 +79,33 @@
     }
     std::vector<int> nlocal(Y.ncls, 0), inrun(Y.ncls, 0);
     for(int t = 0; t < ntasks; t++) nlocal[task_cls[t]] += task_m1[t] - task_m0[t];
+    std::vector<char> in_erun(Y.ncls, 0);
+    for(const Run& r : runs)
+    {
+      if(!eval_runs) break;
+      const int nper = r.n / r.P;
+      DlbEvalRun er; memset(&er, 0, sizeof(er));
+      er.j0 = r.j0; er.nper = nper; er.P = r.P;
+      er.pos0 = (unsigned int)(Jp[cbk + r.j0] - Jp[cbk]);
+      bool ok = true;
+      for(int i = 0; i < r.P && ok; i++)
+      {
+        const int c = cls(r.j0 + i), k = Y.cls_ptr[c+1] - Y.cls_ptr[c], t = cls_task_ptr[c];
+        ok = k <= 32 && cls_task_ptr[c+1] - t == 1 && nlocal[c] == nper && task_m1[t] - task_m0[t] > SMALL_MEMBERS;
+        er.k[i] = k; er.koff[i] = er.Ktot; er.Ktot += k;
+        er.goff[i] = task_goff[t]; er.Goff[i] = task_Goff[t];
+      }
+      if(!ok) continue;
+      for(int i = 0; i < r.P; i++)
+      {
+        in_erun[cls(r.j0 + i)] = 1;
+        T.erun_ntile = std::max(T.erun_ntile, (er.k[i] + 7) / 8);
+      }
+      T.erun_P = std::max(T.erun_P, r.P);
+      T.eruns.push_back(er);
+    }
+    for(int t : big_tasks) if(!in_erun[task_cls[t]]) T.ebig_tasks.push_back(t);
+    if(!ranges_enabled) runs.clear();
     for(bool changed = true; changed; )
     {
       changed = false;
diff --git a/libdogleg_b200/csrc/dlb_taskplan.h b/libdogleg_b200/csrc/dlb_taskplan.h
--- a/libdogleg_b200/csrc/dlb_taskplan.h
+++ b/libdogleg_b200/csrc/dlb_taskplan.h
@@ -10,6 +10,14 @@
   unsigned int pos0; int pad[3];
   int cls[4], koff[4];
   long long goff[4];
+};
+
+struct alignas(16) DlbEvalRun
+{
+  int j0, nper, P, Ktot;
+  unsigned int pos0; int pad[3];
+  int k[4], koff[4];
+  long long goff[4], Goff[4];
 };
 
 struct DlbTaskPlan
@@ -25,6 +33,9 @@
   std::vector<char> ranged;
   int range_kmax = 1;
   std::vector<int> gj_big_tasks;
+  std::vector<DlbEvalRun> eruns;
+  std::vector<int> ebig_tasks;
+  int erun_P = 0, erun_ntile = 0;
   std::vector<int> gp_count;
   std::vector<long long> gp_first;
   std::vector<int> ginv_ptr, ginv_cls;
@@ -35,4 +46,4 @@
 };
 
 void dlb_build_task_plan(const DlbSymbolic& Y, const int* Jp, int cbk, int Mk, int n_state, int sm_count,
-                         bool ranges_enabled, DlbTaskPlan& T, bool one_task_per_class = false);
+                         bool ranges_enabled, DlbTaskPlan& T, bool one_task_per_class = false, bool eval_runs = false);
diff --git a/libdogleg_b200/ffi.py b/libdogleg_b200/ffi.py
--- a/libdogleg_b200/ffi.py
+++ b/libdogleg_b200/ffi.py
@@ -15,7 +15,8 @@
            level_sn=14, cls_ptr=15, cls_rows=16, cls_loc=17, mem_ptr=18, mem_col=19)
 TP = dict(task_cls=0, task_m0=1, task_m1=2, cls_task_ptr=3, task_goff=4, task_Goff=5, mem_col=6, mem_pos=7,
           big_tasks=8, small_tasks=9, gj_big_tasks=10, ranged=11, gp_count=12, gp_first=13, ginv_ptr=14,
-          ginv_cls=15, ginv_off=16, heavy=17, medium=18, sizes=19, range_tasks=20)
+          ginv_cls=15, ginv_off=16, heavy=17, medium=18, sizes=19, range_tasks=20, eval_runs=21, ebig_tasks=22)
+TP_FLAG_RANGES, TP_FLAG_EVAL_RUNS, TP_FLAG_ONE_TASK = 1, 2, 4
 GP = dict(dst=0, src_ptr=1, src_base=2, ld=3, h=4, w=5, src_ld=6, level_ptr=7, tmp_off=8, level_tmp=9,
           sg_flag=10)
 
@@ -163,6 +164,8 @@
     L.dlb_gather_plan_get.restype = C.c_longlong
     L.dlb_task_plan_create.argtypes = [vp, ip, C.c_int, C.c_int, C.c_int, C.c_int]
     L.dlb_task_plan_create.restype = vp
+    L.dlb_task_plan_create2.argtypes = [vp, ip, C.c_int, C.c_int, C.c_int, C.c_int]
+    L.dlb_task_plan_create2.restype = vp
     L.dlb_task_plan_free.argtypes = [vp]
     L.dlb_task_plan_free.restype = None
     L.dlb_task_plan_get.argtypes = [vp, C.c_int, llp, C.c_longlong]
@@ -198,6 +201,8 @@
     L.dlb_engine_scalars.restype = C.POINTER(Scalars)
     L.dlb_engine_solve.argtypes = [vp, dp, dp, C.c_int]
     L.dlb_engine_debug_JtJ.argtypes = [vp, C.c_int, C.c_double, dp]
+    L.dlb_engine_debug_class_blocks.argtypes = [vp, C.c_int, dp, C.c_longlong]
+    L.dlb_engine_debug_class_blocks.restype = C.c_longlong
     L.dlb_engine_dense_factor_to_host.argtypes = [vp, dp]
     L.dlb_engine_counters.argtypes = [vp, dp]
     L.dlb_engine_counters.restype = None
diff --git a/profiles/micro/eval_pass.py b/profiles/micro/eval_pass.py
--- /dev/null
+++ b/profiles/micro/eval_pass.py
@@ -0,0 +1,113 @@
+import argparse
+import json
+import os
+import subprocess
+import sys
+
+ROOT = os.path.dirname(os.path.dirname(os.path.dirname(os.path.abspath(__file__))))
+sys.path.insert(0, ROOT)
+sys.path.insert(0, os.path.join(ROOT, "tests"))
+
+import numpy as np
+import torch
+
+from libdogleg_b200 import ffi
+from support import harness as H
+
+
+class DevBuf:
+
+    def __init__(self, ptr, n):
+        self.__cuda_array_interface__ = {"shape": (n,), "typestr": "<f8", "data": (ptr, False), "version": 3}
+
+
+def make_engine(prob, p, x, Jx, range_env):
+    os.environ["DOGLEG_GPU_RANGE"] = range_env
+    Jp, Ji = prob.pattern()
+    E = H.Engine(ffi.SOLVE_SPARSE, prob.N, prob.M, len(Ji))
+    E.load_sparse(0, p, x, Jp, Ji, Jx)
+    E.evaluate(0)
+    L = E.L
+    dJ = torch.as_tensor(DevBuf(L.dlb_engine_device_buffer(E.h, 0, ffi.BUF_JVALUES), len(Ji)), device="cuda")
+    stream = torch.cuda.ExternalStream(L.dlb_engine_stream(E.h))
+    return E, dJ, stream
+
+
+def run_passes(E, dJ, stream, src, n):
+    for _ in range(n):
+        with torch.cuda.stream(stream):
+            dJ.copy_(src)
+        E.check(E.L.dlb_engine_evaluate(E.h, 0, 0, 0.0))
+    torch.cuda.synchronize()
+
+
+def pass_times(prof, nth):
+    ev = sorted((e for e in prof.events() if e.device_type == torch.autograd.DeviceType.CUDA
+                 and not e.name.startswith("Memcpy") and "memcpy" not in e.name.lower()),
+                key=lambda e: e.time_range.start)
+    out, cur = [], 0.0
+    names = set()
+    for e in ev:
+        if "k_sparse_grad_reduce" in e.name:
+            out.append(cur)
+            cur = 0.0
+        else:
+            cur += e.time_range.end - e.time_range.start
+            names.add(e.name)
+    return out[-nth:], sorted(names)
+
+
+def main():
+    ap = argparse.ArgumentParser()
+    ap.add_argument("--rounds", type=int, default=5)
+    ap.add_argument("--passes", type=int, default=200)
+    ap.add_argument("--out", default=None, help="write the JSON result there (default: stdout only)")
+    a = ap.parse_args()
+    if not torch.cuda.is_available():
+        raise SystemExit("no CUDA device")
+    smi = subprocess.run(["nvidia-smi", "--query-gpu=name,power.limit,clocks.max.sm", "--format=csv,noheader"],
+                         capture_output=True, text=True).stdout.strip().splitlines()
+    os.environ["DOGLEG_GPU_ENGINE_CACHE"] = "0"
+    prob = H.Problem.mrcal(4, 200, 625)
+    p = prob.p0()
+    x, Jx = prob.evaluate(p)
+    nnz, M = len(Jx), prob.M
+    src = torch.from_numpy(Jx).cuda()
+    engines = {"class_tasks": make_engine(prob, p, x, Jx, "0"), "eval_runs": make_engine(prob, p, x, Jx, "1")}
+    Gsize = engines["eval_runs"][0].L.dlb_engine_debug_class_blocks(engines["eval_runs"][0].h, 0, None, 0)
+    jtx = {k: E.download(0)["Jtx"] for k, (E, _, _) in engines.items()}
+    assert np.array_equal(jtx["class_tasks"].view(np.int64), jtx["eval_runs"].view(np.int64))
+    for k, (E, dJ, st) in engines.items():
+        run_passes(E, dJ, st, src, 20)
+    rounds = {k: [] for k in engines}
+    kernels = {}
+    for r in range(a.rounds):
+        for k, (E, dJ, st) in engines.items():
+            with torch.profiler.profile(activities=[torch.profiler.ProfilerActivity.CUDA]) as prof:
+                run_passes(E, dJ, st, src, a.passes)
+            t, names = pass_times(prof, a.passes)
+            kernels[k] = names
+            rounds[k].append(float(np.median(t)))
+            print(f"round {r} {k}: median {np.median(t):.2f} us over {len(t)} passes (min {np.min(t):.2f}, max {np.max(t):.2f})",
+                  flush=True)
+    algo = 8.0 * (nnz + M) + 8.0 * Gsize
+    res = {"gpu": smi, "problem": "C2: mrcal(4, 200, 625), N=%d M=%d nnz=%d" % (prob.N, M, nnz),
+           "rounds": a.rounds, "passes_per_round": a.passes, "kernels": kernels,
+           "median_us_per_round": rounds,
+           "median_us": {k: float(np.median(v)) for k, v in rounds.items()},
+           "spread_us": {k: [float(np.min(v)), float(np.max(v))] for k, v in rounds.items()},
+           "bytes_algorithmic": algo,
+           "bytes_class_task_index": 8.0 * M,
+           "TBps_algorithmic": {k: algo / (np.median(v) * 1e-6) / 1e12 for k, v in rounds.items()}}
+    if a.out:
+        with open(a.out, "w") as f:
+            json.dump(res, f, indent=1)
+    else:
+        print(json.dumps(res))
+    print(json.dumps(res["median_us"]), json.dumps(res["spread_us"]), json.dumps(res["TBps_algorithmic"]))
+    for E, _, _ in engines.values():
+        E.close()
+
+
+if __name__ == "__main__":
+    main()
```
